# stelleg/caster-dta

Measured on AMD Instinct MI355X. Metric: graph-pairs/sec (Davis-shaped protein+drug), encoders fwd+bwd, higher is better.
Workload: dtype f32; 1 GPU; davis_b64; pairs_per_gpu=64, residues_per_gpu=19200, protein_edges_per_gpu=57484, atoms_per_gpu=2560, drug_edges_per_gpu=7986, encoder=CASTER-DTA(2,2), pass=fwdbwd, activation_storage=fp32, scope=encoders, torch_compile=False, tunable_gemms=False, two_lane_head=False, train_mode=True, csr_build_in_step=True, hip_graph=True, kernels=mfma

## Files before the change

caster-dta_amd/csrc/gvp_internal.h:

```cpp
#pragma once
#include <hip/hip_runtime.h>
#include <stdint.h>

#include "gvp_host.h"
#include "gvp_math.h"
#include "gvp_rng.h"

constexpr int POLICY_F32 = 0, POLICY_BF16 = 1, POLICY_GVPDEF = 2, POLICY_LINEAR = 3;

struct QuadOffsets {
  int emb, conv0, node0, layer_stride, head, total;
  int embT, convT0, nodeT0, layerT_stride, headT;
};

#ifndef CGVP_BWD_MAX_GRID
#define CGVP_BWD_MAX_GRID 240
#endif
constexpr int kBwdMaxGrid = CGVP_BWD_MAX_GRID;

#include <type_traits>

namespace gq { struct bf16s; struct f32_gvpdef; struct f32_linear; }
template <class T> struct Tag { using type = T; };
template <class ST> constexpr bool is_layer_kind = std::is_same_v<ST, gq::f32_gvpdef> || std::is_same_v<ST, gq::f32_linear>;
template <bool KINDS, class F>
int with_policy(int policy, F&& f) {
  if (policy == POLICY_F32) return f(Tag<float>{});
  if (policy == POLICY_BF16) return f(Tag<gq::bf16s>{});
  if constexpr (KINDS) {
    if (policy == POLICY_GVPDEF) return f(Tag<gq::f32_gvpdef>{});
    if (policy == POLICY_LINEAR) return f(Tag<gq::f32_linear>{});
  }
  return CGVP_ERR_UNSUPPORTED_DIMS;
}
template <class F>
int with_flag(bool b, F&& f) { return b ? f(std::true_type{}) : f(std::false_type{}); }

namespace quad {
int offsets(int nt_node, int nt_edge, int num_convs, QuadOffsets* o);
int prepare(const gvp::EncLayout& L, int num_convs, int packed_bf16, const float* params, float* image, hipStream_t st);
int node_embed(int nt_node, const float* img, const float* x_s, const float* x_v, const int64_t* ntypes,
               int64_t N, float* h, unsigned long long* rng_state, unsigned long long* rng_out, int policy, hipStream_t st);
int pass_begin(const gvp::EncLayout& L, int num_convs, int policy, const float* params, float* image, const float* x_s,
               const float* x_v, const int64_t* ntypes, int64_t N, float* h, unsigned long long* rng_state,
               unsigned long long* rng_out, const int64_t* edge_index, int64_t E, int32_t* counters, hipStream_t st);
int conv(int nt_edge, const float* img, const float* h, const float* e_s, const float* e_v,
         const int64_t* etypes, const int32_t* rowptr, const int32_t* eperm, const int32_t* esrc,
         const int32_t* edst, int64_t N, int64_t E, int mean, float* dh, int fuse, const float* img_node,
         const float* img_head, float* h_out, float* out, const float* mask0, const float* mask1, gvp::RngArgs rng,
         const float* e_in, float* e_out, int policy, hipStream_t st);
int node_update(const float* img_node, const float* img_head, const float* h, const float* dh, int64_t N,
                int with_head, float* h_out, float* out, const float* mask0, const float* mask1, gvp::RngArgs rng,
                int policy, hipStream_t st);

int node_update_bwd(const float* img_node, const float* imgT_node, const float* h, const float* dh,
                    const float* mask0, const float* mask1, gvp::RngArgs rng, const float* g_up0, const float* g_up1,
                    const float* g_up2, int64_t N, float* g_dh, float* g_h, float* zero_rows, float* slab, int* grid,
                    int policy, hipStream_t st);
int head_bwd(const float* img_head, const float* imgT_head, const float* h_out, const float* g_out, int64_t N,
             float* g_h_out, float* slab, int* grid, int policy, hipStream_t st);
int node_head_bwd(const float* img_head, const float* imgT_head, const float* h_out, const float* g_out, float* g_h_out,
                  float* head_slab, const float* img_node, const float* imgT_node, const float* h, const float* dh,
                  const float* mask0, const float* mask1, gvp::RngArgs rng, int64_t N, float* g_dh, float* g_h,
                  float* zero_rows, float* slab, int* grid, int policy, hipStream_t st);
int conv_bwd(int nt_edge, const float* img, const float* imgT, const float* h, const float* e_emb,
             const int32_t* rowptr, const int32_t* esrc, const int32_t* edst, int64_t N, int64_t E, int mean,
             const float* g_dh, float* g_src, float* g_dst, float* g_e, float* slab, int* grid, int policy, hipStream_t st,
             float* g_edge = nullptr, float* slot = nullptr);
int conv_bwd_max_waves();
int64_t src_index_work_ints(int64_t N, int64_t E);
int src_index(const int32_t* rowptr, const int32_t* esrc, int64_t N, int64_t E, int32_t* sptr, int32_t* spos,
              int32_t* work, hipStream_t st);
int src_sum(int width, const float* rows, const float* self, const int32_t* sptr, const int32_t* spos,
            const int32_t* rowptr, const float* slot, int64_t waves, int64_t N, float* out, hipStream_t st);
struct DetBufs { const int32_t* sptr; const int32_t* spos; float* rows; float* slot; };
int conv_bwd_entry(const cgvp_dims* dims, const cgvp_layout* layout, const float* image, int32_t layer,
                   const float* h, const float* e_emb, const int32_t* rowptr, const int32_t* esrc,
                   const int32_t* edst, int64_t N, int64_t E, int32_t aggr_mean, const float* g_dh, float* g_src,
                   int32_t g_src_zeroed, float* g_dst, float* g_e, float* grad_params, float* workspace,
                   cgvp_segment* segs, int32_t* nsegs, void* stream, const DetBufs* det);
bool deterministic_env();
int edge_embed_bwd(int nt_edge, const float* img, const float* imgT, const float* e_s, const float* e_v,
                   const int64_t* etypes, const int32_t* eperm, int64_t E, const float* const* g_e, int n_g,
                   float* g_e_s, float* g_e_v, float* slab, int* grid, int policy, hipStream_t st);
constexpr int kEdgeRow = 36;
int node_embed_bwd(int nt_node, const float* img, const float* imgT, const float* x_s, const float* x_v,
                   const int64_t* ntypes, int64_t N, const float* g_up0, const float* g_up1, const float* g_up2,
                   float* g_x_s, float* g_x_v, float* slab, int* grid, int policy, hipStream_t st);
constexpr int kGineBwdMaxGrid = 256;
constexpr int kGineBwdDefaultGrid = 16;
int gine_bwd(int cin, int chid, int cout, int nt, int net, int ed, const float* x, const int64_t* ntypes,
             const float* eattr, const int64_t* etypes, const int32_t* rowptr, const int32_t* eperm,
             const int32_t* esrc, const int32_t* edst, int64_t N, const cgvp_gine_w* w, float slope,
             const float* mask, gvp::RngArgs rng, const float* g_out, float* g_x, float* slab, int max_workgroups, int* rows,
             int* row_len, hipStream_t st, const float* agg_in = nullptr, const uint16_t* pos_in = nullptr,
             float* g_edge = nullptr, float* g_self = nullptr,
             float* g_eattr = nullptr, int eattr_accum = 0);
int gine_fwd(int cin, int chid, int cout, int nt, int net, int ed, const float* x, const int64_t* ntypes,
             const float* eattr, const int64_t* etypes, const int32_t* rowptr, const int32_t* eperm,
             const int32_t* esrc, const int32_t* edst, int64_t N, const cgvp_gine_w* w, float slope,
             const float* mask, gvp::RngArgs rng, float* out, float* agg_out, uint16_t* pos_out, hipStream_t st);
int reduce_slab(const float* slab, int rows, int stride, int col0, int len, float* dst, hipStream_t st);
int reduce_segments(const cgvp_segment* segs, int nsegs, float* grad_params, hipStream_t st, int overwrite = 0,
                    bool store_only = false);
struct BwdBlocks { int emb, conv_edge, conv_total, node, head; };
int bwd_block_sizes(int nt_node, int nt_edge, BwdBlocks* b);
void zero_words(void* p, size_t words, hipStream_t s);
int csr_build(const int64_t* edge_index, int64_t N, int64_t E, int32_t* rowptr, int32_t* eperm, int32_t* esrc,
              int32_t* edst, int32_t* work, int work_is_zero, int32_t* ids_scratch, unsigned long long* rng_state,
              unsigned long long* rng_out, hipStream_t stream);
}
```

caster-dta_amd/csrc/gvp_kernels.hip:

```cpp
#include <hip/hip_runtime.h>
#include <stdlib.h>
#include <stdint.h>

#include "gvp_internal.h"

using namespace gvp;

namespace {

constexpr int WAVE = 64;

inline int check_dims(const cgvp_dims* d) {
  if (!d) return CGVP_ERR_BAD_ARG;
  if (d->node_in_s != NODE_IN_S || d->node_in_v != NODE_IN_V || d->edge_in_s != EDGE_IN_S ||
      d->edge_in_v != EDGE_IN_V || d->hidden_s != NS || d->hidden_v != NV ||
      d->edge_hidden_s != ES || d->edge_hidden_v != EV || d->out_s != OUT)
    return CGVP_ERR_UNSUPPORTED_DIMS;
  if (d->storage != CGVP_F32 && d->storage != CGVP_BF16) return CGVP_ERR_UNSUPPORTED_DIMS;
  if (d->layer_kind < CGVP_LAYER_GATED || d->layer_kind > CGVP_LAYER_LINEAR) return CGVP_ERR_UNSUPPORTED_DIMS;
  if (d->layer_kind != CGVP_LAYER_GATED && d->storage != CGVP_F32) return CGVP_ERR_UNSUPPORTED_DIMS;
  return 0;
}
inline int check_dims_gated(const cgvp_dims* d) {
  if (int rc = check_dims(d)) return rc;
// ... 602 lines not shown
int cgvp_abi_version(void) { return CGVP_ABI_VERSION; }
const char* cgvp_build_info(void) { return "libcaster_gvp gfx950 (HIP, wave64), built " __DATE__ " " __TIME__; }

int cgvp_csr_from_coo(const int64_t* edge_index, int64_t N, int64_t E, int32_t* rowptr,
                      int32_t* eperm, int32_t* esrc, int32_t* edst, int32_t* work, int32_t work_is_zero,
                      int32_t* ids_scratch, void* stream) {
  return quad::csr_build(edge_index, N, E, rowptr, eperm, esrc, edst, work, work_is_zero, ids_scratch, nullptr, nullptr,
                         (hipStream_t)stream);
}
}

namespace quad {
void zero_words(void* p, size_t words, hipStream_t s) { ::zero_words(p, words, s); }

int csr_build(const int64_t* edge_index, int64_t N, int64_t E, int32_t* rowptr, int32_t* eperm, int32_t* esrc,
              int32_t* edst, int32_t* work, int work_is_zero, int32_t* ids_scratch, unsigned long long* rng_state,
              unsigned long long* rng_out, hipStream_t stream) {
  if (N < 0 || E < 0 || !rowptr || !work || (E > 0 && (!edge_index || !eperm || !esrc || !edst || !ids_scratch)))
    return CGVP_ERR_BAD_ARG;
  if (N >= (int64_t)1 << 31 || E >= (int64_t)1 << 31) return CGVP_ERR_BAD_ARG;
  if ((uintptr_t)work & 15) return CGVP_ERR_BAD_ARG;
  hipStream_t s = stream;
  const int64_t counters = (N + 1 + 63) / 64 * 64;
  if (work_is_zero == 0) {
    zero_words(work, (size_t)counters, s);
  }
  int32_t* tmp = ids_scratch;
  const int B = 256;
  if (E > 0 && work_is_zero != 2)
    launch<csr_count_kernel>(dim3((unsigned)((E + B - 1) / B)), dim3(B), 0, s, edge_index, N, E, work, rng_state, rng_out);
  else if (rng_state)
    launch<rng_next_kernel>(dim3(1), dim3(1), 0, s, rng_state, rng_out);
  if (N < SCAN_MULTI_MAX) {
    launch<csr_scan_multi_kernel>(dim3((unsigned)((N + 1 + SCAN_MULTI_CHUNK - 1) / SCAN_MULTI_CHUNK)),
                                  dim3(SCAN_MULTI_T), 0, s, work, (int32_t)N, (int32_t)counters, rowptr);
  } else {
    const int64_t tile = N < SCAN_LDS ? (N + 3) / 4 * 4 : SCAN_LDS;
    if (int rc = launch<csr_scan_kernel>(dim3(1), dim3(1024), (size_t)(tile + 1024 + 32) * sizeof(int32_t), s, work, N, rowptr)) return rc;
  }
  if (E > 0) launch<csr_fill_kernel>(dim3((unsigned)((E + B - 1) / B)), dim3(B), 0, s, edge_index, N, E, rowptr, work, tmp, edst);
  const int64_t span = E > counters ? E : counters;
  launch<csr_rank_kernel>(dim3((unsigned)((span + B - 1) / B)), dim3(B), 0, s, edge_index, N, E, counters, rowptr, tmp,
                          edst, eperm, esrc, work);
  return launch_status();
}

bool deterministic_env() {
  static const bool v = [] { const char* e = getenv("CGVP_DETERMINISTIC"); return e && e[0] == '1'; }();
  return v;
}

int64_t src_index_work_ints(int64_t N, int64_t E) { return (N + 1 + 63) / 64 * 64 + (E > 0 ? E : 1); }

int src_index(const int32_t* rowptr, const int32_t* esrc, int64_t N, int64_t E, int32_t* sptr, int32_t* spos,
              int32_t* work, hipStream_t s) {
  if (N < 0 || E < 0 || !rowptr || !sptr || !work || (E > 0 && (!esrc || !spos))) return CGVP_ERR_BAD_ARG;
  if (N >= (int64_t)1 << 31 || E >= (int64_t)1 << 31 || ((uintptr_t)work & 15)) return CGVP_ERR_BAD_ARG;
  const int64_t counters = (N + 1 + 63) / 64 * 64;
  int32_t* cnt = work;
  int32_t* tmp = work + counters;
  zero_words(cnt, (size_t)counters, s);
  const int B = 256;
  const unsigned eb = (unsigned)((E + B - 1) / B);
  if (E > 0) launch<src_count_kernel>(dim3(eb), dim3(B), 0, s, esrc, rowptr, N, cnt);
  if (N < SCAN_MULTI_MAX) {
    launch<csr_scan_multi_kernel>(dim3((unsigned)((N + 1 + SCAN_MULTI_CHUNK - 1) / SCAN_MULTI_CHUNK)),
                                  dim3(SCAN_MULTI_T), 0, s, cnt, (int32_t)N, (int32_t)counters, sptr);
  } else {
    const int64_t tile = N < SCAN_LDS ? (N + 3) / 4 * 4 : SCAN_LDS;
    if (int rc = launch<csr_scan_kernel>(dim3(1), dim3(1024), (size_t)(tile + 1024 + 32) * sizeof(int32_t), s, cnt, N, sptr)) return rc;
  }
  if (E > 0) {
    launch<src_fill_kernel>(dim3(eb), dim3(B), 0, s, esrc, rowptr, N, sptr, cnt, tmp);
    launch<src_rank_kernel>(dim3(eb), dim3(B), 0, s, esrc, rowptr, N, sptr, tmp, spos);
  }
  return launch_status();
}
}

extern "C" {

int cgvp_deterministic_forced(void) { return quad::deterministic_env() ? 1 : 0; }

int cgvp_csr_collate(const int32_t* st_rowptr, const int32_t* st_eperm, const int32_t* st_esrc,
                     const int32_t* st_edst, const int64_t* st_node_off, const int64_t* st_edge_off,
                     const int64_t* sel, const int64_t* b_node_off, const int64_t* b_edge_off, int64_t B,
                     int32_t table_mode, int32_t* rowptr, int32_t* eperm, int32_t* esrc, int32_t* edst, void* stream) {
  if (B < 0 || !rowptr) return CGVP_ERR_BAD_ARG;
  if (B == 0) return 0;
  if (!st_rowptr || !st_node_off || !st_edge_off || !sel || !b_node_off || !b_edge_off) return CGVP_ERR_BAD_ARG;
  CsrCollateArgs a{st_rowptr, st_eperm, st_esrc, st_edst, st_node_off, st_edge_off, sel, b_node_off, b_edge_off, B,
                   rowptr, eperm, esrc, edst, table_mode ? 1 : 0};
  launch<csr_collate_kernel>(dim3((unsigned)B), dim3(256), 0, (hipStream_t)stream, a);
  return launch_status();
}

int cgvp_lba_layout(const cgvp_dims* dims, int32_t num_ntypes, int32_t num_etypes, int32_t num_convs,
                    cgvp_layout* out) {
  if (int rc = check_dims(dims)) return rc;
  if (!out || num_ntypes < 0 || num_etypes < 0 || num_convs < 0) return CGVP_ERR_BAD_ARG;
  const EncLayout L = make_layout(num_ntypes, num_etypes, num_convs);
  out->nt_node = L.nt_node; out->nt_edge = L.nt_edge; out->node_gvp = L.node_gvp; out->node_ln = L.node_ln;
  out->edge_gvp = L.edge_gvp; out->edge_ln = L.edge_ln; out->conv0 = L.conv0;
  out->conv_stride = L.conv_stride; out->ln_out = L.ln_out; out->head = L.head; out->total = L.total;
  return 0;
}

int64_t cgvp_lba_image_floats(const cgvp_dims* dims, const cgvp_layout* layout) {
  if (int rc = check_dims(dims)) return rc;
  if (!layout) return CGVP_ERR_BAD_ARG;
  QuadOffsets o;
  if (int rc = quad::offsets(layout->nt_node, layout->nt_edge, num_convs_of(*layout), &o)) return rc;
  return o.total;
}

int cgvp_lba_prepare(const cgvp_dims* dims, const cgvp_layout* layout, const float* params, float* image,
                     void* stream) {
  if (int rc = check_dims(dims)) return rc;
  if (!layout || !params || !image) return CGVP_ERR_BAD_ARG;
  if (int rc = quad::prepare(cvt(*layout), num_convs_of(*layout), policy_of(dims) == POLICY_BF16 ? 1 : 0, params, image, (hipStream_t)stream)) return rc;
  return launch_status();
}

int cgvp_lba_pass_begin(const cgvp_dims* dims, const cgvp_layout* layout, const float* params, float* image,
                        const float* x_s, const float* x_v, const int64_t* ntypes, int64_t N, float* h,
                        uint64_t* rng_state, uint64_t* rng_out, const int64_t* edge_index, int64_t E,
                        int32_t* csr_counters, void* stream) {
  if (int rc = check_dims_gated(dims)) return rc;
  if (N < 0 || E < 0 || !layout || !params || !image || (layout->nt_node > 0 && N > 0 && !ntypes)) return CGVP_ERR_BAD_ARG;
  if ((rng_state != nullptr) != (rng_out != nullptr)) return CGVP_ERR_BAD_ARG;
  if (((uintptr_t)rng_state & 7) || ((uintptr_t)rng_out & 7) || ((uintptr_t)h & 15) || ((uintptr_t)image & 15)) return CGVP_ERR_BAD_ARG;
  if ((edge_index != nullptr) != (csr_counters != nullptr)) return CGVP_ERR_BAD_ARG;
  if (N > 0 && (!x_s || !x_v || !h)) return CGVP_ERR_BAD_ARG;
  if (N >= (int64_t)1 << 31 || E >= (int64_t)1 << 31) return CGVP_ERR_BAD_ARG;
  if (N == 0 && rng_state)
    if (int rc = cgvp_rng_next(rng_state, rng_out, stream)) return rc;
  if (int rc = quad::pass_begin(cvt(*layout), num_convs_of(*layout), policy_of(dims), params, image, x_s, x_v, ntypes, N, h,
                                reinterpret_cast<unsigned long long*>(rng_state), reinterpret_cast<unsigned long long*>(rng_out),
                                edge_index, E, csr_counters, (hipStream_t)stream)) return rc;
  return launch_status();
}


int cgvp_node_embed_fwd(const cgvp_dims* dims, const cgvp_layout* layout, const float* params,
                        const float* image, const float* x_s, const float* x_v, const int64_t* ntypes,
                        int64_t N, float* h, uint64_t* rng_state, uint64_t* rng_out, void* stream) {
  if (int rc = check_dims_gated(dims)) return rc;
  if (N < 0 || !layout || !params || (layout->nt_node > 0 && N > 0 && !ntypes)) return CGVP_ERR_BAD_ARG;
  if ((rng_state != nullptr) != (rng_out != nullptr) || (rng_state && !image)) return CGVP_ERR_BAD_ARG;
  if (((uintptr_t)rng_state & 7) || ((uintptr_t)rng_out & 7)) return CGVP_ERR_BAD_ARG;
  if (N == 0) return rng_state ? cgvp_rng_next(rng_state, rng_out, stream) : 0;
  if (!x_s || !x_v || !h) return CGVP_ERR_BAD_ARG;
  if (image) {
    if ((uintptr_t)h & 15) return CGVP_ERR_BAD_ARG;
    QuadOffsets o;
    if (int rc = quad::offsets(layout->nt_node, layout->nt_edge, num_convs_of(*layout), &o)) return rc;
    if (int rc = quad::node_embed(layout->nt_node, image + o.emb, x_s, x_v, ntypes, N, h,
                                  reinterpret_cast<unsigned long long*>(rng_state),
                                  reinterpret_cast<unsigned long long*>(rng_out), policy_of(dims), (hipStream_t)stream)) return rc;
    return launch_status();
  }
  if (policy_of(dims)) return CGVP_ERR_UNSUPPORTED_DIMS;
  NodeEmbedArgs a{params, cvt(*layout), x_s, x_v, ntypes, N, h};
  const dim3 grid((unsigned)((N + WAVE - 1) / WAVE));
  hipStream_t st = (hipStream_t)stream;
  switch (layout->nt_node) {
    case 0: launch<node_embed_kernel<0>>(grid, dim3(WAVE), 0, st, a); break;
    case 20: launch<node_embed_kernel<20>>(grid, dim3(WAVE), 0, st, a); break;
    case 21: launch<node_embed_kernel<21>>(grid, dim3(WAVE), 0, st, a); break;
    default: return CGVP_ERR_UNSUPPORTED_DIMS;
  }
  return launch_status();
}

int cgvp_conv_fwd(const cgvp_dims* dims, const cgvp_layout* layout, const float* params,
                  const float* image, int32_t layer,
                  const float* h, const float* e_s, const float* e_v, const int64_t* etypes,
                  const int32_t* rowptr, const int32_t* eperm, const int32_t* esrc,
                  const int32_t* edst, int64_t N, int64_t E, int32_t aggr_mean, const float* e_in,
                  float* e_out, float* dh, void* stream) {
  if (int rc = check_dims(dims)) return rc;
  if (N < 0 || E < 0 || !layout || !params) return CGVP_ERR_BAD_ARG;
  if (layer < 0 || layer >= num_convs_of(*layout)) return CGVP_ERR_BAD_ARG;
  if (N == 0) return 0;
  if (!h || !dh || !rowptr) return CGVP_ERR_BAD_ARG;
  if (!image && (e_in || e_out)) return CGVP_ERR_BAD_ARG;
  if (E > 0 && (!esrc || !edst)) return CGVP_ERR_BAD_ARG;
  if (E > 0 && !e_in && (!e_s || !e_v || !eperm || (layout->nt_edge > 0 && !etypes))) return CGVP_ERR_BAD_ARG;
  if (((uintptr_t)h & 15) || ((uintptr_t)e_s & 15) || ((uintptr_t)e_in & 15) || ((uintptr_t)e_out & 15)) return CGVP_ERR_BAD_ARG;
  if (image) {
    QuadOffsets o;
    if (int rc = quad::offsets(layout->nt_node, layout->nt_edge, num_convs_of(*layout), &o)) return rc;
    if (int rc = quad::conv(layout->nt_edge, image + o.conv0 + layer * o.layer_stride, h, e_s, e_v, etypes, rowptr,
                            eperm, esrc, edst, N, E, aggr_mean ? 1 : 0, dh, 0, nullptr, nullptr, nullptr, nullptr, nullptr,
                            nullptr, gvp::RngArgs{nullptr, 0.f, 0}, e_in, e_in ? nullptr : e_out, policy_of(dims),
                            (hipStream_t)stream)) return rc;
    return launch_status();
  }
  if (policy_of(dims)) return CGVP_ERR_UNSUPPORTED_DIMS;
  int64_t deg = (E + N - 1) / N;
  if (deg < 1) deg = 1;
  int npw = (int)(48 / deg);
  npw = npw < 1 ? 1 : (npw > WAVE ? WAVE : npw);
  ConvArgs a{params, cvt(*layout), layer, h, e_s, e_v, etypes, rowptr, eperm, esrc, edst, N, npw,
             aggr_mean ? 1 : 0, dh};
  const dim3 grid((unsigned)((N + npw - 1) / npw));
  hipStream_t st = (hipStream_t)stream;
  switch (layout->nt_edge) {
    case 0: launch<conv_fwd_kernel<0>>(grid, dim3(WAVE), 0, st, a); break;
    case 1: launch<conv_fwd_kernel<1>>(grid, dim3(WAVE), 0, st, a); break;
    default: return CGVP_ERR_UNSUPPORTED_DIMS;
  }
  return launch_status();
}

int cgvp_conv_layer_fwd(const cgvp_dims* dims, const cgvp_layout* layout, const float* image, int32_t layer,
                        const float* h, const float* e_s, const float* e_v, const int64_t* etypes,
                        const int32_t* rowptr, const int32_t* eperm, const int32_t* esrc, const int32_t* edst,
                        int64_t N, int64_t E, int32_t aggr_mean, const float* mask0, const float* mask1,
                        const cgvp_rng* rng, int32_t with_head, const float* e_in, float* e_out, float* dh,
                        float* h_out, float* out, void* stream) {
  if (int rc = check_dims_gated(dims)) return rc;
  if (int rc = check_rng(rng)) return rc;
  if (N < 0 || E < 0 || !layout || !image) return CGVP_ERR_BAD_ARG;
  if (layer < 0 || layer >= num_convs_of(*layout)) return CGVP_ERR_BAD_ARG;
  if (N == 0) return 0;
  if (!h || !rowptr || (with_head ? !out : !h_out)) return CGVP_ERR_BAD_ARG;
  if (E > 0 && (!esrc || !edst)) return CGVP_ERR_BAD_ARG;
  if (E > 0 && !e_in && (!e_s || !e_v || !eperm || (layout->nt_edge > 0 && !etypes))) return CGVP_ERR_BAD_ARG;
  const void* al[] = {h, e_s, dh, h_out, out, mask0, mask1, e_in, e_out};
  for (const void* q : al) if ((uintptr_t)q & 15) return CGVP_ERR_BAD_ARG;
  QuadOffsets o;
  if (int rc = quad::offsets(layout->nt_node, layout->nt_edge, num_convs_of(*layout), &o)) return rc;
  if (int rc = quad::conv(layout->nt_edge, image + o.conv0 + layer * o.layer_stride, h, e_s, e_v, etypes, rowptr, eperm,
                          esrc, edst, N, E, aggr_mean ? 1 : 0, dh, with_head ? 2 : 1,
                          image + o.node0 + layer * o.layer_stride, image + o.head, h_out, out, mask0, mask1,
                          rng_args(rng, 2 * layer), e_in, e_in ? nullptr : e_out, policy_of(dims), (hipStream_t)stream)) return rc;
  return launch_status();
}

int cgvp_node_update_fwd(const cgvp_dims* dims, const cgvp_layout* layout, const float* params,
                         const float* image, int32_t layer, const float* h, const float* dh, int64_t N,
                         int32_t with_head, float* h_out, float* out, void* stream) {
  if (int rc = check_dims(dims)) return rc;
  if (N < 0 || !layout || !params) return CGVP_ERR_BAD_ARG;
  if (layer < 0 || layer >= num_convs_of(*layout)) return CGVP_ERR_BAD_ARG;
  if (N == 0) return 0;
  if (!h || !dh || (with_head ? !out : !h_out)) return CGVP_ERR_BAD_ARG;
  if (((uintptr_t)h & 15) || ((uintptr_t)dh & 15)) return CGVP_ERR_BAD_ARG;
  if (image) {
    if (((uintptr_t)h_out & 15) || ((uintptr_t)out & 15)) return CGVP_ERR_BAD_ARG;
    QuadOffsets o;
    if (int rc = quad::offsets(layout->nt_node, layout->nt_edge, num_convs_of(*layout), &o)) return rc;
    if (int rc = quad::node_update(image + o.node0 + layer * o.layer_stride, image + o.head, h, dh, N,
                                   with_head ? 1 : 0, h_out, out, nullptr, nullptr, gvp::RngArgs{nullptr, 0.f, 0},
                                   policy_of(dims), (hipStream_t)stream)) return rc;
    return launch_status();
  }
  if (policy_of(dims)) return CGVP_ERR_UNSUPPORTED_DIMS;
  NodeUpdateArgs a{params, cvt(*layout), layer, h, dh, N, h_out, out};
  dim3 grid((unsigned)((N + WAVE - 1) / WAVE));
  if (with_head) launch<node_update_kernel<true>>(grid, dim3(WAVE), 0, (hipStream_t)stream, a);
  else launch<node_update_kernel<false>>(grid, dim3(WAVE), 0, (hipStream_t)stream, a);
  return launch_status();
}

int cgvp_node_update_fwd_train(const cgvp_dims* dims, const cgvp_layout* layout, const float* image,
                               int32_t layer, const float* h, const float* dh, const float* mask0,
                               const float* mask1, const cgvp_rng* rng, int64_t N, int32_t with_head, float* h_out,
                               float* out, void* stream) {
  if (int rc = check_dims(dims)) return rc;
  if (int rc = check_rng(rng)) return rc;
  if (N < 0 || !layout || !image) return CGVP_ERR_BAD_ARG;
  if (layer < 0 || layer >= num_convs_of(*layout)) return CGVP_ERR_BAD_ARG;
  if (N == 0) return 0;
  if (!h || !dh || (with_head ? !out : !h_out)) return CGVP_ERR_BAD_ARG;
  if (((uintptr_t)h & 15) || ((uintptr_t)dh & 15) || ((uintptr_t)h_out & 15) || ((uintptr_t)out & 15) ||
      ((uintptr_t)mask0 & 15) || ((uintptr_t)mask1 & 15)) return CGVP_ERR_BAD_ARG;
  QuadOffsets o;
  if (int rc = quad::offsets(layout->nt_node, layout->nt_edge, num_convs_of(*layout), &o)) return rc;
  if (int rc = quad::node_update(image + o.node0 + layer * o.layer_stride, image + o.head, h, dh, N,
                                 with_head ? 1 : 0, h_out, out, mask0, mask1, rng_args(rng, 2 * layer),
                                 policy_of(dims), (hipStream_t)stream)) return rc;
  return launch_status();
}

int64_t cgvp_bwd_workspace_floats(const cgvp_dims* dims, const cgvp_layout* layout) {
  if (int rc = check_dims(dims)) return rc;
  if (!layout) return CGVP_ERR_BAD_ARG;
  quad::BwdBlocks b;
  if (int rc = quad::bwd_block_sizes(layout->nt_node, layout->nt_edge, &b)) return rc;
  int mx = b.emb > b.conv_total ? b.emb : b.conv_total;
  mx = mx > b.node + b.head ? mx : b.node + b.head;
  mx = mx > 2 * b.conv_edge ? mx : 2 * b.conv_edge;
  return (int64_t)kBwdMaxGrid * mx;
}

int cgvp_node_update_bwd(const cgvp_dims* dims, const cgvp_layout* layout, const float* image, int32_t layer,
                         const float* h, const float* dh, const float* mask0, const float* mask1,
                         const cgvp_rng* rng, const float* h_out, const float* g_out, const float* g_up0, const float* g_up1,
                         const float* g_up2, int64_t N, int32_t with_head, float* g_dh, float* g_h,
                         float* zero_out, float* grad_params, float* workspace, cgvp_segment* segs, int32_t* nsegs,
                         void* stream) {
  if (int rc = check_dims(dims)) return rc;
  if (int rc = check_rng(rng)) return rc;
  if (N < 0 || !layout || !image || !grad_params || !workspace) return CGVP_ERR_BAD_ARG;
  const int nc = num_convs_of(*layout);
  if (layer < 0 || layer >= nc) return CGVP_ERR_BAD_ARG;
  if (N == 0) return 0;
  if (!h || !dh || !g_dh || (with_head && (!g_out || !h_out))) return CGVP_ERR_BAD_ARG;
  if (with_head && dims->layer_kind != CGVP_LAYER_GATED) return CGVP_ERR_UNSUPPORTED_DIMS;
  const void* al[] = {h, dh, mask0, mask1, h_out, g_out, g_up0, g_up1, g_up2, g_dh, g_h, zero_out};
  for (const void* q : al) if ((uintptr_t)q & 15) return CGVP_ERR_BAD_ARG;
  BwdLookup o;
  if (int rc = bwd_lookup(*layout, &o)) return rc;
  int grid = 0, hgrid = 0;
  hipStream_t st = (hipStream_t)stream;
  float* head_slab = workspace + (size_t)kBwdMaxGrid * o.blk.node;
  static const bool split_head = [] { const char* e = getenv("CGVP_SPLIT_HEAD_BWD"); return e && e[0] == '1'; }();
  if (with_head && !split_head) {
    if (int rc = quad::node_head_bwd(image + o.head, image + o.headT, h_out, g_out, g_dh, head_slab,
                                     image + o.node0 + layer * o.layer_stride, image + o.nodeT0 + layer * o.layerT_stride,
                                     h, dh, mask0, mask1, rng_args(rng, 2 * layer), N, g_dh, g_h, zero_out, workspace, &grid,
                                     policy_of(dims), st)) return rc;
    hgrid = grid;
  } else {
  if (with_head) {
    if (int rc = quad::head_bwd(image + o.head, image + o.headT, h_out, g_out, N, g_dh, head_slab, &hgrid, policy_of(dims), st)) return rc;
    g_up0 = g_dh; g_up1 = nullptr; g_up2 = nullptr;
  }
  if (int rc = quad::node_update_bwd(image + o.node0 + layer * o.layer_stride, image + o.nodeT0 + layer * o.layerT_stride,
                                     h, dh, mask0, mask1, rng_args(rng, 2 * layer), g_up0, g_up1, g_up2, N, g_dh, g_h, zero_out,
                                     workspace, &grid, policy_of(dims), st)) return rc;
  }
  const int node_len = conv_ff1() + LFf1::size(0) - conv_ln0();
  cgvp_segment sg[2] = {{workspace, grid, o.blk.node, 0, node_len, layout->conv0 + layer * layout->conv_stride + conv_ln0()},
                        {head_slab, hgrid, o.blk.head, 0, layout->total - layout->ln_out, layout->ln_out}};
  return emit_segments(sg, with_head ? 2 : 1, segs, nsegs, grad_params, st);
}

int cgvp_conv_bwd(const cgvp_dims* dims, const cgvp_layout* layout, const float* image, int32_t layer,
                  const float* h, const float* e_emb, const int32_t* rowptr, const int32_t* esrc,
                  const int32_t* edst, int64_t N, int64_t E, int32_t aggr_mean, const float* g_dh, float* g_src,
                  int32_t g_src_zeroed, float* g_dst, float* g_e, float* grad_params, float* workspace,
                  cgvp_segment* segs, int32_t* nsegs, void* stream) {
  if (quad::deterministic_env()) return CGVP_ERR_NONDETERMINISTIC;
  return quad::conv_bwd_entry(dims, layout, image, layer, h, e_emb, rowptr, esrc, edst, N, E, aggr_mean, g_dh, g_src,
                              g_src_zeroed, g_dst, g_e, grad_params, workspace, segs, nsegs, stream, nullptr);
}
}

int quad::conv_bwd_entry(const cgvp_dims* dims, const cgvp_layout* layout, const float* image, int32_t layer,
                         const float* h, const float* e_emb, const int32_t* rowptr, const int32_t* esrc,
                         const int32_t* edst, int64_t N, int64_t E, int32_t aggr_mean, const float* g_dh, float* g_src,
                         int32_t g_src_zeroed, float* g_dst, float* g_e, float* grad_params, float* workspace,
                         cgvp_segment* segs, int32_t* nsegs, void* stream, const quad::DetBufs* det) {
  if (int rc = check_dims(dims)) return rc;
  if (N < 0 || E < 0 || !layout || !image || !grad_params || !workspace) return CGVP_ERR_BAD_ARG;
  const int nc = num_convs_of(*layout);
  if (layer < 0 || layer >= nc) return CGVP_ERR_BAD_ARG;
  if (N == 0) return 0;
  if (!h || !g_dh || !g_src || !g_dst || !rowptr) return CGVP_ERR_BAD_ARG;
  if (E > 0 && (!e_emb || !g_e || !esrc || !edst)) return CGVP_ERR_BAD_ARG;
  const void* al[] = {h, e_emb, g_dh, g_src, g_dst, g_e};
  for (const void* q : al) if ((uintptr_t)q & 15) return CGVP_ERR_BAD_ARG;
  BwdLookup o;
  if (int rc = bwd_lookup(*layout, &o)) return rc;
  int grid = 0;
  hipStream_t st = (hipStream_t)stream;
  if (!g_src_zeroed && !det) {
    zero_words(g_src, (size_t)N * ROW, st);
  }
  if (int rc = quad::conv_bwd(layout->nt_edge, image + o.conv0 + layer * o.layer_stride,
                              image + o.convT0 + layer * o.layerT_stride, h, e_emb, rowptr, esrc, edst, N, E,
                              aggr_mean ? 1 : 0, g_dh, g_src, g_dst, g_e, workspace, &grid, policy_of(dims), st,
                              det ? det->rows : nullptr, det ? det->slot : nullptr)) return rc;
  if (det)
    if (int rc = quad::src_sum(ROW, det->rows, nullptr, det->sptr, det->spos, rowptr, det->slot, (int64_t)grid * 8, N, g_src, st))
      return rc;
  const cgvp_segment sg{workspace, grid, o.blk.conv_total, 0, conv_ln0(), layout->conv0 + layer * layout->conv_stride};
  return emit_segments(&sg, 1, segs, nsegs, grad_params, st, det ? 1 : 0, det != nullptr);
}

extern "C" {

int64_t cgvp_src_index_work_ints(int64_t num_nodes, int64_t num_edges) {
  if (num_nodes < 0 || num_edges < 0) return CGVP_ERR_BAD_ARG;
  return quad::src_index_work_ints(num_nodes, num_edges);
}

int cgvp_src_index(const int32_t* rowptr, const int32_t* esrc, int64_t num_nodes, int64_t num_edges, int32_t* sptr,
                   int32_t* spos, int32_t* work, void* stream) {
  return quad::src_index(rowptr, esrc, num_nodes, num_edges, sptr, spos, work, (hipStream_t)stream);
}

int64_t cgvp_conv_bwd_det_floats(int64_t num_nodes, int64_t num_edges) {
  if (num_nodes < 0 || num_edges < 0) return CGVP_ERR_BAD_ARG;
  return (num_edges > 0 ? num_edges : 1) * ROW + (int64_t)quad::conv_bwd_max_waves() * ROW;
}

int cgvp_conv_bwd_ex(const cgvp_dims* dims, const cgvp_layout* layout, const float* image, int32_t layer,
                     const float* h, const float* e_emb, const int32_t* rowptr, const int32_t* esrc,
                     const int32_t* edst, int64_t N, int64_t E, int32_t aggr_mean, const float* g_dh, float* g_src,
                     int32_t g_src_zeroed, float* g_dst, float* g_e, float* grad_params, float* workspace,
                     cgvp_segment* segs, int32_t* nsegs, const int32_t* sptr, const int32_t* spos, float* det_scratch,
                     int32_t flags, void* stream) {
  if (!((flags & CGVP_BWD_DETERMINISTIC) || quad::deterministic_env()))
    return quad::conv_bwd_entry(dims, layout, image, layer, h, e_emb, rowptr, esrc, edst, N, E, aggr_mean, g_dh, g_src,
                                g_src_zeroed, g_dst, g_e, grad_params, workspace, segs, nsegs, stream, nullptr);
  if (!sptr || !det_scratch || (E > 0 && !spos) || ((uintptr_t)det_scratch & 15)) return CGVP_ERR_BAD_ARG;
  const quad::DetBufs db{sptr, spos, det_scratch, det_scratch + (E > 0 ? E : 1) * ROW};
  return quad::conv_bwd_entry(dims, layout, image, layer, h, e_emb, rowptr, esrc, edst, N, E, aggr_mean, g_dh, g_src,
                              g_src_zeroed, g_dst, g_e, grad_params, workspace, segs, nsegs, stream, &db);
}

}

extern "C" {

int cgvp_edge_embed_bwd(const cgvp_dims* dims, const cgvp_layout* layout, const float* image, const float* e_s,
                        const float* e_v, const int64_t* etypes, const int32_t* eperm, int64_t E,
                        const float* const* g_e, int32_t num_g, float* g_e_s, float* g_e_v, float* grad_params,
                        float* workspace, cgvp_segment* segs, int32_t* nsegs, void* stream) {
  if (int rc = check_dims_gated(dims)) return rc;
  if (E < 0 || !layout || !image || !grad_params || !workspace || !g_e || num_g < 1) return CGVP_ERR_BAD_ARG;
  if ((g_e_s == nullptr) != (g_e_v == nullptr) || ((uintptr_t)g_e_s & 15)) return CGVP_ERR_BAD_ARG;
  if (segs && nsegs) *nsegs = 0;
  if (E == 0) return 0;
  if (!e_s || !e_v || !eperm || (layout->nt_edge > 0 && !etypes)) return CGVP_ERR_BAD_ARG;
  if ((uintptr_t)e_s & 15) return CGVP_ERR_BAD_ARG;
  for (int l = 0; l < num_g; ++l) if (!g_e[l] || ((uintptr_t)g_e[l] & 15)) return CGVP_ERR_BAD_ARG;
  BwdLookup o;
  if (int rc = bwd_lookup(*layout, &o)) return rc;
  int grid = 0;
  hipStream_t st = (hipStream_t)stream;
  if (g_e_s) {
    quad::zero_words(g_e_s, (size_t)E * EDGE_IN_S, st);
    quad::zero_words(g_e_v, (size_t)E * EDGE_IN_V * 3, st);
  }
  if (int rc = quad::edge_embed_bwd(layout->nt_edge, image + o.conv0, image + o.convT0, e_s, e_v, etypes, eperm, E, g_e,
                                    num_g, g_e_s, g_e_v, workspace, &grid, policy_of(dims), st)) return rc;
  const cgvp_segment sg{workspace, grid, o.blk.conv_edge, 0, layout->conv0 - layout->edge_gvp, layout->edge_gvp};
  return emit_segments(&sg, 1, segs, nsegs, grad_params, st);
}

int cgvp_node_embed_bwd(const cgvp_dims* dims, const cgvp_layout* layout, const float* image, const float* x_s,
                        const float* x_v, const int64_t* ntypes, int64_t N, const float* g_up0,
                        const float* g_up1, const float* g_up2, float* g_x_s, float* g_x_v, float* grad_params,
                        float* workspace, cgvp_segment* segs, int32_t* nsegs, void* stream) {
  if (int rc = check_dims_gated(dims)) return rc;
  if (N < 0 || !layout || !image || !grad_params || !workspace) return CGVP_ERR_BAD_ARG;
  if (N == 0) return 0;
  if (!x_s || !x_v || (layout->nt_node > 0 && !ntypes) || ((g_x_s == nullptr) != (g_x_v == nullptr))) return CGVP_ERR_BAD_ARG;
  const void* al[] = {g_up0, g_up1, g_up2};
  for (const void* q : al) if ((uintptr_t)q & 15) return CGVP_ERR_BAD_ARG;
  BwdLookup o;
  if (int rc = bwd_lookup(*layout, &o)) return rc;
  int grid = 0;
  hipStream_t st = (hipStream_t)stream;
  if (int rc = quad::node_embed_bwd(layout->nt_node, image + o.emb, image + o.embT, x_s, x_v, ntypes, N, g_up0, g_up1,
                                    g_up2, g_x_s, g_x_v, workspace, &grid, policy_of(dims), st)) return rc;
  const cgvp_segment sg{workspace, grid, o.blk.emb, 0, layout->edge_gvp - layout->node_gvp, layout->node_gvp};
  return emit_segments(&sg, 1, segs, nsegs, grad_params, st);
}

int cgvp_gine_conv_fwd(const float* x, const int64_t* ntypes, int32_t num_ntypes, const float* eattr,
                       const int64_t* etypes, int32_t num_etypes, int32_t edge_dim,
                       const int32_t* rowptr, const int32_t* eperm, const int32_t* esrc, const int32_t* edst,
                       int64_t N, int64_t E, int32_t cin, int32_t chid, int32_t cout, const cgvp_gine_w* w,
                       float act_slope, const float* mask, const cgvp_rng* rng, int32_t variant, float* out,
                       void* stream) {
  if (N < 0 || E < 0 || !w) return CGVP_ERR_BAD_ARG;
  if (int rc = check_rng(rng)) return rc;
  const gvp::RngArgs ra = rng_args(rng, 0);
  if (num_ntypes < 0 || num_etypes < 0 || edge_dim < 0 || cin <= num_ntypes) return CGVP_ERR_BAD_ARG;
  if (cin > WAVE || chid > WAVE || cout > WAVE || chid < 1 || cout < 1 || num_etypes + edge_dim > GINE_MAXKE)
    return CGVP_ERR_UNSUPPORTED_DIMS;
  if (N == 0) return 0;
  if (!x || !out || !rowptr || (num_ntypes > 0 && !ntypes)) return CGVP_ERR_BAD_ARG;
  if (E > 0 && (!eperm || !esrc || (edge_dim > 0 && !eattr) || (num_etypes > 0 && !etypes))) return CGVP_ERR_BAD_ARG;
  if (variant == 0 && edst && !((uintptr_t)out & 15) && !((uintptr_t)mask & 15)) {
    const int rc = quad::gine_fwd(cin, chid, cout, num_ntypes, num_etypes, edge_dim, x, ntypes, eattr, etypes, rowptr,
                                  eperm, esrc, edst, N, w, act_slope, mask, ra, out, nullptr, nullptr, (hipStream_t)stream);
    if (rc <= 0) return rc < 0 ? rc : launch_status();
  }
  GineArgs a{x, ntypes, num_ntypes, eattr, etypes, num_etypes, edge_dim, rowptr, eperm, esrc, N, cin,
             chid, cout, w->eps, w->we, w->be, w->w0, w->b0, w->w1, w->b1, act_slope, out, mask, ra};
  const size_t lds = (size_t)(chid * (cin + 1) + cout * (chid + 1) + 2 * GINE_APB * WAVE) * sizeof(float);
  launch<gine_conv_kernel>(dim3((unsigned)((N + GINE_APB - 1) / GINE_APB)),
                           dim3(WAVE * GINE_APB), lds, (hipStream_t)stream, a);
  return launch_status();
}

int cgvp_rng_next(uint64_t* state, uint64_t* out, void* stream) {
  if (!state || !out || ((uintptr_t)state & 7) || ((uintptr_t)out & 7)) return CGVP_ERR_BAD_ARG;
  launch<rng_next_kernel>(dim3(1), dim3(1), 0, (hipStream_t)stream,
                          reinterpret_cast<unsigned long long*>(state), reinterpret_cast<unsigned long long*>(out));
  return launch_status();
}

int cgvp_dropout_masks(const cgvp_rng* rng, int32_t num_masks, int64_t N, int32_t width, float* out, void* stream) {
  if (!rng || !rng->seed || !out || num_masks < 1 || N < 0 || width < 4 || (width & 3)) return CGVP_ERR_BAD_ARG;
  if (int rc = check_rng(rng)) return rc;
  if (N == 0) return 0;
  MaskArgs a{rng_args(rng, 0), num_masks, N, width, out};
  const int64_t total = (int64_t)num_masks * N * (width / 4);
  launch<dropout_masks_kernel>(dim3((unsigned)((total + 255) / 256 > 4096 ? 4096 : (total + 255) / 256)), dim3(256), 0,
                               (hipStream_t)stream, a);
  return launch_status();
}

int cgvp_bwd_reduce(const cgvp_segment* segs, int32_t nsegs, float* grad_params, int32_t overwrite, void* stream) {
  if (!segs || nsegs < 0 || nsegs > CGVP_MAX_SEGS || !grad_params) return CGVP_ERR_BAD_ARG;
  quad::reduce_segments(segs, nsegs, grad_params, (hipStream_t)stream, overwrite ? 1 : 0);
  return launch_status();
}

int64_t cgvp_gine_bwd_workspace_floats(void) { return (int64_t)quad::kGineBwdMaxGrid * gine_layer_floats(16, 64, 64, 14); }

int cgvp_gine_conv_bwd(const float* x, const int64_t* ntypes, int32_t num_ntypes, const float* eattr,
                       const int64_t* etypes, int32_t num_etypes, int32_t edge_dim, const int32_t* rowptr,
                       const int32_t* eperm, const int32_t* esrc, const int32_t* edst, int64_t N, int64_t E,
                       int32_t cin, int32_t chid, int32_t cout, const cgvp_gine_w* w, float act_slope,
                       const float* mask, const cgvp_rng* rng, const float* g_out, float* g_x, float* grad_layer,
                       float* workspace, int32_t max_workgroups, void* stream) {
  if (N < 0 || E < 0 || !w || !grad_layer || !workspace) return CGVP_ERR_BAD_ARG;
  if (int rc = check_rng(rng)) return rc;
  if (quad::deterministic_env() && g_x) return CGVP_ERR_NONDETERMINISTIC;
  if (N == 0) return 0;
  if (!x || !g_out || !rowptr || (num_ntypes > 0 && !ntypes)) return CGVP_ERR_BAD_ARG;
  if (E > 0 && (!eperm || !esrc || !edst || (edge_dim > 0 && !eattr) || (num_etypes > 0 && !etypes))) return CGVP_ERR_BAD_ARG;
  if (((uintptr_t)g_out & 15) || ((uintptr_t)mask & 15)) return CGVP_ERR_BAD_ARG;
  hipStream_t st = (hipStream_t)stream;
  if (g_x) {
    zero_words(g_x, (size_t)N * (cin - num_ntypes), st);
  }
  int rows = 0, row_len = 0;
  if (int rc = quad::gine_bwd(cin, chid, cout, num_ntypes, num_etypes, edge_dim, x, ntypes, eattr, etypes, rowptr, eperm,
                              esrc, edst, N, w, act_slope, mask, rng_args(rng, 0), g_out, g_x, workspace, max_workgroups, &rows, &row_len, st)) return rc;
  quad::reduce_slab(workspace, rows, row_len, 0, row_len, grad_layer, st);
  return launch_status();
}

}
```

caster-dta_amd/csrc/gvp_quad_bwd_kernels.hip:

```cpp
#include <hip/hip_runtime.h>
#include <stdint.h>
#include <stdlib.h>

#include <type_traits>

#include "gvp_internal.h"
#include "gvp_quad.h"

using namespace gq;

#ifdef CGVP_STAMPS
__device__ unsigned long long* g_stamp_buf_bwd = nullptr;
extern "C" int cgvp_debug_set_stamp_buffer_bwd(unsigned long long* buf) {
  return (int)hipMemcpyToSymbol(HIP_SYMBOL(g_stamp_buf_bwd), &buf, sizeof(buf));
}
#endif

namespace {

constexpr int WAVE = 64;
constexpr int TILE = 16;

#ifdef CGVP_STAMPS
#define STAMP(slot)                                                                          \
  do {                                                                                       \
    __builtin_amdgcn_sched_barrier(0);                                                       \
    unsigned long long t_;                                                                   \
    asm volatile("s_waitcnt vmcnt(0) lgkmcnt(0)\n\ts_memtime %0\n\ts_waitcnt lgkmcnt(0)" : "=s"(t_)::"memory"); \
    __builtin_amdgcn_sched_barrier(0);                                                       \
    if (g_stamp_buf_bwd && (threadIdx.x & 63) == 0)                                          \
      g_stamp_buf_bwd[((size_t)blockIdx.x * (blockDim.x >> 6) + (threadIdx.x >> 6)) * 16 + (slot)] = t_;    \
  } while (0)
struct WallStamp {
  int kind;
  __device__ __forceinline__ explicit WallStamp(int k) : kind(k) { put(0); }
  __device__ __forceinline__ ~WallStamp() { put(1); }
  __device__ __forceinline__ void put(int which) const {
    unsigned long long t_;
    asm volatile("s_waitcnt vmcnt(0) lgkmcnt(0)\n\ts_memrealtime %0\n\ts_waitcnt lgkmcnt(0)" : "=s"(t_)::"memory");
    const size_t wave = (size_t)blockIdx.x * (blockDim.x >> 6) + (threadIdx.x >> 6);
    if (g_stamp_buf_bwd && (threadIdx.x & 63) == 0 && wave < 4096)
      g_stamp_buf_bwd[4096 * 16 + ((size_t)kind * 4096 + wave) * 2 + which] = t_;
  }
};
#define WALL_STAMP(kind) WallStamp wall_stamp_(kind)
#else
#define STAMP(slot) do {} while (0)
#define WALL_STAMP(kind) do {} while (0)
#endif
constexpr int BW_WPB = 8, BW_TPB = WAVE * BW_WPB, BW_MAX_GRID = kBwdMaxGrid;
static_assert(BW_MAX_GRID <= 256, "at most one workgroup per CU");

__device__ __forceinline__ int opaque_lane(int lane) {
  asm volatile("" : "+v"(lane));
  return lane;
}

template <int BLK>
__device__ __forceinline__ void zero_block(float* gblk, int lane) {
  static_assert(BLK % 4 == 0, "blocks are whole float4s");
  for (int k = lane; k < BLK / 4; k += WAVE) reinterpret_cast<f4*>(gblk)[k] = f4{0.f, 0.f, 0.f, 0.f};
}
template <int BLK, int PW, int WPB_ = 8>
__device__ __forceinline__ void write_slab_row(float* slab, const float* blocks, int row = blockIdx.x) {
  __syncthreads();
  float* out = slab + (size_t)row * BLK;
  for (int k = threadIdx.x; k < BLK; k += WAVE * WPB_) {
    float t = 0.f;
#pragma unroll
    for (int ww = 0; ww < WPB_; ++ww) t += blocks[ww * PW + k];
    out[k] = t;
  }
}

template <int NFLOATS, int NTHR>
__device__ __forceinline__ void stage_slice(float* lds, const float* __restrict__ src, int tid) {
  static_assert(NFLOATS % 4 == 0, "image slices are whole float4s");
  constexpr int NF4 = NFLOATS / 4, IT = (NF4 + NTHR - 1) / NTHR;
  const f4* s = reinterpret_cast<const f4*>(src);
  f4* d = reinterpret_cast<f4*>(lds);
  f4 v[IT];
#pragma unroll
  for (int k = 0; k < IT; ++k) { const int idx = tid + k * NTHR; if (idx < NF4) v[k] = s[idx]; }
#pragma unroll
  for (int k = 0; k < IT; ++k) { const int idx = tid + k * NTHR; if (idx < NF4) d[idx] = v[k]; }
}

constexpr int cmax(int a, int b) { return a > b ? a : b; }
template <bool ONE> using AccFor = typename std::conditional<ONE, AccStoreOnce, AccPriv>::type;
constexpr int pad4(int x) { return (x + 3) / 4 * 4; }

template <class Acc, int S>
__device__ __forceinline__ void ln_param_grads(float* blk, bool first, int lane, bool active,
                                               const f4 (&dgamma)[S / 16], const f4 (&dbeta)[S / 16]) {
  const int i = lane & 15, g = lane >> 4;
#pragma unroll
  for (int t = 0; t < S / 16; ++t) {
    float tot[8];
    float* q[8];
    bool on[8];
#pragma unroll
    for (int r = 0; r < 4; ++r) {
      tot[r] = row_total(active ? dgamma[t][r] : 0.f);
      tot[4 + r] = row_total(active ? dbeta[t][r] : 0.f);
      q[r] = blk + 16 * t + 4 * g + r;
      q[4 + r] = blk + S + 16 * t + 4 * g + r;
      on[r] = on[4 + r] = i == 15;
    }
    add_where<Acc, 8>(q, on, tot);
  }
}

constexpr int NB_LN0 = 0, NB_LN1 = 2 * NS, NB_FF0 = 4 * NS, NB_FF1 = NB_FF0 + LFf0::size(0),
              NODE_BLK = NB_FF1 + LFf1::size(0);
constexpr int HB_LN = 0, HB_GVP = 2 * NS, HEAD_BLK = HB_GVP + LHead::size(0);
constexpr int NODE_GB = pad4(NODE_BLK), HEAD_GB = pad4(HEAD_BLK);

constexpr int MROW = NS + NV;
__device__ __forceinline__ void node_dropout(const float* mask, const gvp::RngArgs& rng, int which, int64_t n, int g,
                                             f4& ms, float& mv) {
  if (mask) {
    ms = *reinterpret_cast<const f4*>(mask + n * MROW + 4 * g);
    mv = mask[n * MROW + NS + g];
  } else if (rng.seed) {
    const unsigned long long seed = rng.seed[0], off = rng.seed[1];
    float fs[4];
    gvp::dropout_row20(seed, off, rng.stream + which, n, g, rng.p, fs, mv);
    ms = f4{fs[0], fs[1], fs[2], fs[3]};
  }
}
struct NodeBArgs {
  const float* img_node; const float* imgT_node;
  const float* h; const float* dh; const float* mask0; const float* mask1; gvp::RngArgs rng;
  const float* g_up0; const float* g_up1; const float* g_up2;
  int64_t N; float* g_dh; float* g_h; float* zero_rows; float* slab;
};
constexpr int node_bwd_lds_floats() { return BW_TPB + Image<0, 0>::ND_SIZE + Image<0, 0>::TN_SIZE + BW_WPB * (NODE_GB + TSCR_FLOATS); }
static_assert(node_bwd_lds_floats() * 4 <= 160 * 1024, "node backward LDS plan exceeds the CU");

template <typename ST, bool ONE = false>
__device__ __forceinline__ void node_bwd_body(const NodeBArgs& a, float* lds) {
  typedef Image<0, 0> IM;
  typedef AccFor<ONE> Acc;
  float* f_node = lds + BW_TPB;
  float* t_node = f_node + IM::ND_SIZE;
  float* blocks = t_node + IM::TN_SIZE;
  const int lane0 = threadIdx.x & 63, w = threadIdx.x >> 6;
  float* gblk = blocks + w * NODE_GB;
  float* tscr = blocks + BW_WPB * NODE_GB + w * TSCR_FLOATS;
  stage_slice<IM::ND_SIZE, BW_TPB>(f_node, a.img_node, threadIdx.x);
  stage_slice<IM::TN_SIZE, BW_TPB>(t_node, a.imgT_node, threadIdx.x);
  zero_block<NODE_GB>(gblk, lane0);
  STAMP(0);
  __syncthreads();
  STAMP(1);

  const f4 zero = {0.f, 0.f, 0.f, 0.f};
  const int zt[1] = {0};
  const bool first = false;
  const int64_t ntiles = (a.N + TILE - 1) / TILE;
  for (int64_t tile = (int64_t)w * gridDim.x + blockIdx.x; tile < ntiles; tile += (int64_t)gridDim.x * BW_WPB) {
    const int lane = opaque_lane(lane0), i = lane & 15, g = lane >> 4;
    const int64_t n = tile * TILE + i;
    const bool active = n < a.N;
    f4 x0[1] = {zero};
    float xv0[3][1] = {{0.f}, {0.f}, {0.f}};
    f4 m0s = {1.f, 1.f, 1.f, 1.f}, m1s = {1.f, 1.f, 1.f, 1.f};
    float m0v = 1.f, m1v = 1.f;
    f4 gs[1] = {zero};
    float gv[3][1] = {{0.f}, {0.f}, {0.f}};
    if (active) {
      const int64_t hr = n * ROW;
      node_dropout(a.mask0, a.rng, 0, n, g, m0s, m0v);
      node_dropout(a.mask1, a.rng, 1, n, g, m1s, m1v);
      x0[0] = Io<ST>::ld4(a.h, hr + 4 * g) + Io<ST>::ld4(a.dh, hr + 4 * g) * m0s;
#pragma unroll
      for (int p = 0; p < 3; ++p) xv0[p][0] = Io<ST>::ld(a.h, hr + NS + 3 * g + p) + Io<ST>::ld(a.dh, hr + NS + 3 * g + p) * m0v;
      const float* ups[3] = {a.g_up0, a.g_up1, a.g_up2};
#pragma unroll
      for (int u = 0; u < 3; ++u)
        if (ups[u]) {
          const float* r_ = ups[u] + n * ROW;
          gs[0] += *reinterpret_cast<const f4*>(r_ + 4 * g);
#pragma unroll
          for (int p = 0; p < 3; ++p) gv[p][0] += r_[NS + 3 * g + p];
        }
    }
    f4 y[1] = {x0[0]};
    float yv[3][1] = {{xv0[0][0]}, {xv0[1][0]}, {xv0[2][0]}};
    ln_quad<NS, NV>(f_node + IM::ND_LN0, lane, y, yv);
    f4 hs[1][4], s2[1][1];
    float hv[1][3][2], v2[1][3][1];
    float bs0[1][4], bv0[1][3][1], bs1[1][16], bv1[1][3][2];
    typename Ff0<ST>::Cache c0[1];
    typename Ff1<ST>::Cache c1[1];
#pragma unroll
    for (int r = 0; r < 4; ++r) bs0[0][r] = y[0][r];
#pragma unroll
    for (int p = 0; p < 3; ++p) bv0[0][p][0] = yv[p][0];
    Ff0<ST>::template forward<1, Io<ST>::BF>(f_node + IM::ND_FF0, lane, zt, bs0, bv0, hs, hv, c0);
#pragma unroll
    for (int t = 0; t < 4; ++t)
#pragma unroll
      for (int r = 0; r < 4; ++r) bs1[0][4 * t + r] = hs[0][t][r];
#pragma unroll
    for (int p = 0; p < 3; ++p) { bv1[0][p][0] = hv[0][p][0]; bv1[0][p][1] = hv[0][p][1]; }
    Ff1<ST>::template forward<1, Io<ST>::BF>(f_node + IM::ND_FF1, lane, zt, bs1, bv1, s2, v2, c1);
    f4 z[1] = {y[0] + s2[0][0] * m1s};
    float zv[3][1];
#pragma unroll
    for (int p = 0; p < 3; ++p) zv[p][0] = yv[p][0] + v2[0][p][0] * m1v;

    STAMP(2);
    STAMP(3);
    {
      f4 dga[1], dbe[1];
      ln_quad_bwd<NS, NV>(f_node + IM::ND_LN1, lane, z, zv, gs, gv, dga, dbe);
      ln_param_grads<Acc, NS>(gblk + NB_LN1, first, lane, active, dga, dbe);
    }
    float d_hs[16], d_hv[3][2];
    {
      f4 d_so[1] = {gs[0] * m1s};
      float d_vo[3][1] = {{gv[0][0] * m1v}, {gv[1][0] * m1v}, {gv[2][0] * m1v}};
      typename Ff1<ST>::Grads gr1;
      STAMP(4);
      Ff1<ST>::template backward<Io<ST>::BF>(t_node + IM::TN_FF1, lane, c1[0], d_so, d_vo, d_hs, d_hv, gr1);
      STAMP(5);
      Ff1<ST>::template weight_grads<Acc, Io<ST>::BF>(gblk + NB_FF1, first, lane, 0, active, bs1[0], bv1[0], c1[0], gr1, tscr);
    }
    {
      f4 d_so[4];
#pragma unroll
      for (int t = 0; t < 4; ++t) d_so[t] = f4{d_hs[4 * t], d_hs[4 * t + 1], d_hs[4 * t + 2], d_hs[4 * t + 3]};
      float d_ys[4], d_yv[3][1];
      typename Ff0<ST>::Grads gr0;
      STAMP(6);
      Ff0<ST>::template backward<Io<ST>::BF>(t_node + IM::TN_FF0, lane, c0[0], d_so, d_hv, d_ys, d_yv, gr0);
      STAMP(7);
      Ff0<ST>::template weight_grads<Acc, Io<ST>::BF>(gblk + NB_FF0, first, lane, 0, active, bs0[0], bv0[0], c0[0], gr0, tscr);
#pragma unroll
      for (int r = 0; r < 4; ++r) gs[0][r] += d_ys[r];
#pragma unroll
      for (int p = 0; p < 3; ++p) gv[p][0] += d_yv[p][0];
    }
    STAMP(8);
    {
      f4 dga[1], dbe[1];
      ln_quad_bwd<NS, NV>(f_node + IM::ND_LN0, lane, x0, xv0, gs, gv, dga, dbe);
      ln_param_grads<Acc, NS>(gblk + NB_LN0, first, lane, active, dga, dbe);
    }
    if (active) {
      if (a.g_h) {
        float* row = a.g_h + n * ROW;
        *reinterpret_cast<f4*>(row + 4 * g) = gs[0];
#pragma unroll
        for (int p = 0; p < 3; ++p) row[NS + 3 * g + p] = gv[p][0];
      }
      float* row = a.g_dh + n * ROW;
      *reinterpret_cast<f4*>(row + 4 * g) = gs[0] * m0s;
#pragma unroll
      for (int p = 0; p < 3; ++p) row[NS + 3 * g + p] = gv[p][0] * m0v;
      if (a.zero_rows) {
        float* z = a.zero_rows + n * ROW;
        *reinterpret_cast<f4*>(z + 4 * g) = zero;
#pragma unroll
        for (int p = 0; p < 3; ++p) z[NS + 3 * g + p] = 0.f;
      }
    }
  }
  STAMP(9);
  write_slab_row<NODE_GB, NODE_GB>(a.slab, blocks);
  STAMP(10);
}
template <typename ST, bool ONE = false>
__global__ __launch_bounds__(BW_TPB, 2) void node_bwd_kernel(NodeBArgs a) {
  WALL_STAMP(0);
  extern __shared__ __attribute__((aligned(16))) float lds[];
  node_bwd_body<ST, ONE>(a, lds);
}

struct HeadBArgs {
  const float* img_head; const float* imgT_head; const float* h_out; const float* g_out;
  int64_t N; float* g_h_out; float* slab;
};
constexpr int head_bwd_lds_floats() { return BW_TPB + Image<0, 0>::HD_SIZE + Image<0, 0>::TH_SIZE + BW_WPB * (HEAD_GB + TSCR_FLOATS); }

template <typename ST, bool ONE = false>
__device__ __forceinline__ void head_bwd_body(const HeadBArgs& a, float* lds) {
  typedef Image<0, 0> IM;
  typedef AccFor<ONE> Acc;
  float* f_head = lds + BW_TPB;
  float* t_head = f_head + IM::HD_SIZE;
  float* blocks = t_head + IM::TH_SIZE;
  const int lane = threadIdx.x & 63, w = threadIdx.x >> 6;
  float* gblk = blocks + w * HEAD_GB;
  float* tscr = blocks + BW_WPB * HEAD_GB + w * TSCR_FLOATS;
  stage_slice<IM::HD_SIZE, BW_TPB>(f_head, a.img_head, threadIdx.x);
  stage_slice<IM::TH_SIZE, BW_TPB>(t_head, a.imgT_head, threadIdx.x);
  zero_block<HEAD_GB>(gblk, lane);
  __syncthreads();

  const int i = lane & 15, g = lane >> 4;
  const f4 zero = {0.f, 0.f, 0.f, 0.f};
  const int zt[1] = {0};
  const bool first = false;
  const int64_t ntiles = (a.N + TILE - 1) / TILE;
  for (int64_t tile = (int64_t)w * gridDim.x + blockIdx.x; tile < ntiles; tile += (int64_t)gridDim.x * BW_WPB) {
    const int64_t n = tile * TILE + i;
    const bool active = n < a.N;
    f4 o1[1] = {zero};
    float ov1[3][1] = {{0.f}, {0.f}, {0.f}};
    f4 d_o[4] = {zero, zero, zero, zero};
    if (active) {
      const int64_t hr = n * ROW;
      o1[0] = Io<ST>::ld4(a.h_out, hr + 4 * g);
#pragma unroll
      for (int p = 0; p < 3; ++p) ov1[p][0] = Io<ST>::ld(a.h_out, hr + NS + 3 * g + p);
      const float* gr_ = a.g_out + n * OUT;
#pragma unroll
      for (int t = 0; t < 4; ++t) d_o[t] = *reinterpret_cast<const f4*>(gr_ + 16 * t + 4 * g);
    }
    f4 wsn[1] = {o1[0]};
    float wvn[3][1] = {{ov1[0][0]}, {ov1[1][0]}, {ov1[2][0]}};
    ln_quad<NS, NV>(f_head + IM::HD_LN, lane, wsn, wvn);
    float bsh[1][4], bvh[1][3][1], dummy[1][3][1];
#pragma unroll
    for (int r = 0; r < 4; ++r) bsh[0][r] = wsn[0][r];
#pragma unroll
    for (int p = 0; p < 3; ++p) bvh[0][p][0] = wvn[p][0];
    f4 o[1][4];
    QHead::Cache ch[1];
    QHead::template forward<1, Io<ST>::BF>(f_head + IM::HD_GVP, lane, zt, bsh, bvh, o, dummy, ch);
    float d_vo[3][1] = {{0.f}, {0.f}, {0.f}}, d_bs[4], d_bv[3][1];
    QHead::Grads grh;
    QHead::template backward<Io<ST>::BF>(t_head, lane, ch[0], d_o, d_vo, d_bs, d_bv, grh);
    QHead::template weight_grads<Acc, Io<ST>::BF>(gblk + HB_GVP, first, lane, 0, active, bsh[0], bvh[0], ch[0], grh, tscr);
    f4 dws[1] = {f4{d_bs[0], d_bs[1], d_bs[2], d_bs[3]}};
    float dwv[3][1] = {{d_bv[0][0]}, {d_bv[1][0]}, {d_bv[2][0]}};
    f4 dga[1], dbe[1];
    ln_quad_bwd<NS, NV>(f_head + IM::HD_LN, lane, o1, ov1, dws, dwv, dga, dbe);
    ln_param_grads<Acc, NS>(gblk + HB_LN, first, lane, active, dga, dbe);
    if (active) {
      float* row = a.g_h_out + n * ROW;
      *reinterpret_cast<f4*>(row + 4 * g) = dws[0];
#pragma unroll
      for (int p = 0; p < 3; ++p) row[NS + 3 * g + p] = dwv[p][0];
    }
  }
  write_slab_row<HEAD_GB, HEAD_GB>(a.slab, blocks);
}
template <typename ST>
__global__ __launch_bounds__(BW_TPB, 2) void head_bwd_kernel(HeadBArgs a) {
  WALL_STAMP(1);
  extern __shared__ __attribute__((aligned(16))) float lds[];
  head_bwd_body<ST>(a, lds);
}

template <typename ST, bool ONE = false>
__global__ __launch_bounds__(BW_TPB, 2) void node_head_bwd_kernel(HeadBArgs hd, NodeBArgs a) {
  WALL_STAMP(0);
  extern __shared__ __attribute__((aligned(16))) float lds[];
  head_bwd_body<ST, ONE>(hd, lds);
  __syncthreads();
  node_bwd_body<ST, ONE>(a, lds);
}

constexpr int EROW = quad::kEdgeRow;
template <int NTE>
struct ConvBlk {
  static constexpr int M0 = 0, M1 = M0 + LMsg0::size(0), M2 = M1 + LMsg::size(0), SIZE = pad4(M2 + LMsg::size(0));
};
#ifndef CGVP_CONV_BWD_WAVES
#define CGVP_CONV_BWD_WAVES 8
#endif
constexpr int CB_WPB = CGVP_CONV_BWD_WAVES, CB_TPB = WAVE * CB_WPB, CB_MAX_GRID = BW_MAX_GRID;
constexpr int CB_SCR = TSCR_FLOATS;
static_assert(CB_SCR >= (TILE / 2) * ROW + TILE, "g_src transpose fits the scratch");
template <int NTE>
struct ConvBImg {
  typedef Image<0, NTE> IM;
  static constexpr int F0 = IM::CV_M0, FSIZE = IM::CV_SIZE - IM::CV_M0;
  static constexpr int T0 = IM::TC_M0, TSIZE = IM::TC_SIZE - IM::TC_M0;
};
template <int NTE>
constexpr int conv_bwd_lds_floats() { return CB_TPB + ConvBImg<NTE>::FSIZE + ConvBImg<NTE>::TSIZE + CB_WPB * (ConvBlk<NTE>::SIZE + CB_SCR); }
static_assert(conv_bwd_lds_floats<1>() * 4 <= 160 * 1024 && conv_bwd_lds_floats<0>() * 4 <= 160 * 1024, "conv backward LDS plan exceeds the CU");

struct ConvBArgs {
  const float* img; const float* imgT;
  const float* h; const float* e_emb;
  const int32_t* rowptr; const int32_t* esrc; const int32_t* edst;
  int64_t N; int npw; int mean; const float* g_dh; float* g_src; float* g_dst; float* g_e; float* slab;
  float* g_edge; float* slot;
};

template <int NTE, typename ST>
__global__ __launch_bounds__(CB_TPB, CB_WPB / 4) void conv_bwd_kernel(ConvBArgs a) {
  WALL_STAMP(2);
  typedef Image<0, NTE> IM;
  typedef ConvBImg<NTE> BI;
  typedef ConvBlk<NTE> B;
  constexpr int PW = B::SIZE + CB_SCR;
  extern __shared__ __attribute__((aligned(16))) float lds[];
  float* img = lds + CB_TPB - BI::F0;
  float* imgT = lds + CB_TPB + BI::FSIZE - BI::T0;
  const int lane0 = threadIdx.x & 63, w = threadIdx.x >> 6;
  float* blocks = lds + CB_TPB + BI::FSIZE + BI::TSIZE;
  float* gblk = blocks + w * PW;
  float* scr = gblk + B::SIZE;
#ifdef CGVP_MFMA_TRANSPOSE
  float* const CB_TSCR = nullptr;
#else
  float* const CB_TSCR = scr;
#endif
  stage_slice<BI::FSIZE, CB_TPB>(lds + CB_TPB, a.img + BI::F0, threadIdx.x);
  stage_slice<BI::TSIZE, CB_TPB>(lds + CB_TPB + BI::FSIZE, a.imgT + BI::T0, threadIdx.x);
  for (int k = lane0; k < B::SIZE / 4; k += WAVE) reinterpret_cast<f4*>(gblk)[k] = f4{0.f, 0.f, 0.f, 0.f};
  STAMP(0);
  __syncthreads();
  STAMP(1);

  const f4 zero = {0.f, 0.f, 0.f, 0.f};
  const int zt[1] = {0};
  const int64_t ngroups = (a.N + a.npw - 1) / a.npw;
  const int64_t grp0 = (int64_t)blockIdx.x * CB_WPB + w;
  const bool first = false;
  float carry[7] = {0.f, 0.f, 0.f, 0.f, 0.f, 0.f, 0.f};
  int carry_dst = -1;
  for (int64_t grp = grp0; grp < ngroups; grp += (int64_t)gridDim.x * CB_WPB) {
    const int64_t n0 = grp * a.npw;
    const int nn = (int)((a.N - n0 < a.npw) ? (a.N - n0) : a.npw);
    const int32_t e0 = a.rowptr[n0], e1 = a.rowptr[n0 + nn];
    for (int k = lane0; k < nn * ROW; k += WAVE) {
      const int64_t nd = n0 + k / ROW;
      if (a.rowptr[nd + 1] == a.rowptr[nd]) a.g_dst[n0 * ROW + k] = 0.f;
    }
    for (int32_t base = e0; base < e1; base += TILE) {
      const int lane = opaque_lane(lane0), i = lane & 15, g = lane >> 4;
      const int32_t p = base + i;
      const bool active = p < e1;
      f4 es0 = zero, es1 = zero, sj = zero, si = zero, d_ms = zero;
      float ev[3] = {0.f, 0.f, 0.f}, vj[3] = {0.f, 0.f, 0.f}, vi[3] = {0.f, 0.f, 0.f}, d_mv[3] = {0.f, 0.f, 0.f};
      int32_t src = 0, dst = -1;
      if (active) {
        src = a.esrc[p];
        dst = a.edst[p];
        const int64_t er = (int64_t)p * EROW;
        es0 = Io<ST>::ld4(a.e_emb, er + 4 * g);
        es1 = Io<ST>::ld4(a.e_emb, er + 16 + 4 * g);
        if (g == 0) {
#pragma unroll
          for (int d = 0; d < 3; ++d) ev[d] = Io<ST>::ld(a.e_emb, er + ES + d);
        }
        const int64_t hj = (int64_t)src * ROW, hi = (int64_t)dst * ROW;
        const float* gd = a.g_dh + (int64_t)dst * ROW;
        sj = Io<ST>::ld4(a.h, hj + 4 * g);
        si = Io<ST>::ld4(a.h, hi + 4 * g);
        d_ms = *reinterpret_cast<const f4*>(gd + 4 * g);
#pragma unroll
        for (int d = 0; d < 3; ++d) { vj[d] = Io<ST>::ld(a.h, hj + NS + 3 * g + d); vi[d] = Io<ST>::ld(a.h, hi + NS + 3 * g + d); d_mv[d] = gd[NS + 3 * g + d]; }
        if (a.mean) {
          const int deg = a.rowptr[dst + 1] - a.rowptr[dst];
          const float sc = 1.0f / (float)(deg > 1 ? deg : 1);
          d_ms *= sc;
#pragma unroll
          for (int d = 0; d < 3; ++d) d_mv[d] *= sc;
        }
      }
      STAMP(2);
      float b0[1][16], bv0[1][3][3], b1[1][4], bv1[1][3][1], b2[1][4], bv2[1][3][1];
#pragma unroll
      for (int r = 0; r < 4; ++r) { b0[0][r] = sj[r]; b0[0][4 + r] = es0[r]; b0[0][8 + r] = es1[r]; b0[0][12 + r] = si[r]; }
#pragma unroll
      for (int d = 0; d < 3; ++d) { bv0[0][d][0] = vj[d]; bv0[0][d][1] = vi[d]; bv0[0][d][2] = ev[d]; }
      f4 s1[1][1], s2[1][1], s3[1][1];
      float v1[1][3][1], v2[1][3][1], v3[1][3][1];
      typename Msg0<ST>::Cache c0[1];
      typename Msg1<ST>::Cache c1[1];
      typename Msg2<ST>::Cache c2[1];
      Msg0<ST>::template forward<1, Io<ST>::BF>(img + IM::CV_M0, lane, zt, b0, bv0, s1, v1, c0);
#pragma unroll
      for (int r = 0; r < 4; ++r) b1[0][r] = s1[0][0][r];
#pragma unroll
      for (int d = 0; d < 3; ++d) bv1[0][d][0] = v1[0][d][0];
      Msg1<ST>::template forward<1, Io<ST>::BF>(img + IM::CV_M1, lane, zt, b1, bv1, s2, v2, c1);
#pragma unroll
      for (int r = 0; r < 4; ++r) b2[0][r] = s2[0][0][r];
#pragma unroll
      for (int d = 0; d < 3; ++d) bv2[0][d][0] = v2[0][d][0];
      Msg2<ST>::template forward<1, Io<ST>::BF>(img + IM::CV_M2, lane, zt, b2, bv2, s3, v3, c2);

      STAMP(3);
      constexpr bool kAllActive = true;
      float d_b[4], d_bv[3][1];
      {
        f4 d_so[1] = {d_ms};
        float d_vo[3][1] = {{d_mv[0]}, {d_mv[1]}, {d_mv[2]}};
        typename Msg2<ST>::Grads gr;
        Msg2<ST>::template backward<Io<ST>::BF>(imgT + IM::TC_M2, lane, c2[0], d_so, d_vo, d_b, d_bv, gr);
        STAMP(10);
        Msg2<ST>::template weight_grads<AccPriv, Io<ST>::BF>(gblk + B::M2, first, lane, 0, kAllActive, b2[0], bv2[0], c2[0], gr, CB_TSCR);
      }
      {
        f4 d_so[1] = {f4{d_b[0], d_b[1], d_b[2], d_b[3]}};
        float d_vo[3][1] = {{d_bv[0][0]}, {d_bv[1][0]}, {d_bv[2][0]}};
        typename Msg1<ST>::Grads gr;
        STAMP(11);
        Msg1<ST>::template backward<Io<ST>::BF>(imgT + IM::TC_M1, lane, c1[0], d_so, d_vo, d_b, d_bv, gr);
        STAMP(12);
        Msg1<ST>::template weight_grads<AccPriv, Io<ST>::BF>(gblk + B::M1, first, lane, 0, kAllActive, b1[0], bv1[0], c1[0], gr, CB_TSCR);
      }
      float d_b0[16], d_bv0[3][3];
      {
        f4 d_so[1] = {f4{d_b[0], d_b[1], d_b[2], d_b[3]}};
        float d_vo[3][1] = {{d_bv[0][0]}, {d_bv[1][0]}, {d_bv[2][0]}};
        typename Msg0<ST>::Grads gr;
        STAMP(13);
        Msg0<ST>::template backward<Io<ST>::BF>(imgT + IM::TC_M0, lane, c0[0], d_so, d_vo, d_b0, d_bv0, gr);
        STAMP(14);
        Msg0<ST>::template weight_grads<AccPriv, Io<ST>::BF>(gblk + B::M0, first, lane, 0, kAllActive, b0[0], bv0[0], c0[0], gr, CB_TSCR);
      }
      STAMP(4);
      if (active) {
        const int64_t gr_ = (int64_t)p * EROW;
        Io<ST>::st4(a.g_e, gr_ + 4 * g, f4{d_b0[4], d_b0[5], d_b0[6], d_b0[7]});
        Io<ST>::st4(a.g_e, gr_ + 16 + 4 * g, f4{d_b0[8], d_b0[9], d_b0[10], d_b0[11]});
        if (g == 0) {
#pragma unroll
          for (int d = 0; d < 3; ++d) Io<ST>::st(a.g_e, gr_ + ES + d, d_bv0[d][2]);
        }
      }
      STAMP(5);
      {
        float* trow = scr;
        int* tsrc = reinterpret_cast<int*>(scr + (TILE / 2) * ROW);
        if (g == 0) tsrc[i] = active ? src : -1;
        const int half = lane / ROW, col = lane - half * ROW;
#pragma unroll
        for (int hb = 0; hb < 2; ++hb) {
          if ((i >> 3) == hb) {
            float* tr = trow + (i & 7) * ROW;
            *reinterpret_cast<f4*>(tr + 4 * g) = f4{d_b0[0], d_b0[1], d_b0[2], d_b0[3]};
#pragma unroll
            for (int d = 0; d < 3; ++d) tr[NS + 3 * g + d] = d_bv0[d][0];
          }
          __builtin_amdgcn_fence(__ATOMIC_RELEASE, "workgroup");
          __builtin_amdgcn_wave_barrier();
          __builtin_amdgcn_fence(__ATOMIC_ACQUIRE, "workgroup");
          if (half < 2) {
#pragma unroll
            for (int k = 0; k < TILE / 4; ++k) {
              const int r = 2 * k + half;
              const int sr = tsrc[8 * hb + r];
              if (sr >= 0) atomicAdd(a.g_src + (int64_t)sr * ROW + col, trow[r * ROW + col]);
            }
          }
          __builtin_amdgcn_fence(__ATOMIC_RELEASE, "workgroup");
          __builtin_amdgcn_wave_barrier();
        }
      }
      STAMP(6);
      {
        float x[7] = {d_b0[12], d_b0[13], d_b0[14], d_b0[15], d_bv0[0][1], d_bv0[1][1], d_bv0[2][1]};
        if (i == 0 && active && dst == carry_dst) {
#pragma unroll
          for (int k = 0; k < 7; ++k) x[k] += carry[k];
        }
        seg_scan16<7>(dst, x);
        const int nxt = __builtin_amdgcn_update_dpp(-1, dst, 0x100 | 1, 0xf, 0xf, false);
        if (active && (i == TILE - 1 || nxt != dst)) {
          float* row = a.g_dst + (int64_t)dst * ROW;
          *reinterpret_cast<f4*>(row + 4 * g) = f4{x[0], x[1], x[2], x[3]};
#pragma unroll
          for (int d = 0; d < 3; ++d) row[NS + 3 * g + d] = x[4 + d];
        }
        carry_dst = __builtin_amdgcn_update_dpp(-1, dst, 0x100 | 15, 0xf, 0xf, false);
#pragma unroll
        for (int k = 0; k < 7; ++k)
          carry[k] = __builtin_bit_cast(float, __builtin_amdgcn_update_dpp(0, __builtin_bit_cast(int, x[k]), 0x100 | 15, 0xf, 0xf, false));
      }
    }
    STAMP(7);
  }
  STAMP(8);
  write_slab_row<B::SIZE, PW, CB_WPB>(a.slab, blocks);
  STAMP(9);
}

template <int TN, int WPB>
struct C2Shape {
  static constexpr int TPB = WAVE * WPB, GS_ROWS = TN * TILE;
  static constexpr int SCR = TN * TSCR_FLOATS + GS_ROWS * ROW + GS_ROWS;
  static_assert((TN * TSCR_FLOATS) % 4 == 0 && (GS_ROWS * ROW) % 4 == 0, "scratch regions stay 16-B aligned");
  template <int NTE>
  static constexpr int lds_floats() { return TPB + ConvBImg<NTE>::FSIZE + ConvBImg<NTE>::TSIZE + WPB * (ConvBlk<NTE>::SIZE + SCR); }
};
static_assert(C2Shape<2, 4>::lds_floats<1>() * 4 <= 160 * 1024 && C2Shape<1, 8>::lds_floats<1>() * 4 <= 160 * 1024, "conv backward v2 LDS plan exceeds the CU");

struct C2Rows {
  f4 es0, es1, sj, si, d_ms;
  float ev[3], vj[3], vi[3], d_mv[3];
};
template <typename ST>
__device__ __forceinline__ void c2_load_rows(const ConvBArgs& a, int32_t pc, int32_t src, int32_t dst, int g, C2Rows& r) {
  const int64_t er = (int64_t)pc * EROW;
  r.es0 = Io<ST>::ld4(a.e_emb, er + 4 * g);
  r.es1 = Io<ST>::ld4(a.e_emb, er + 16 + 4 * g);
#pragma unroll
  for (int d = 0; d < 3; ++d) r.ev[d] = Io<ST>::ld(a.e_emb, er + ES + d);
  const int64_t hj = (int64_t)src * ROW, hi = (int64_t)dst * ROW;
  const float* gd = a.g_dh + (int64_t)dst * ROW;
  r.sj = Io<ST>::ld4(a.h, hj + 4 * g);
  r.si = Io<ST>::ld4(a.h, hi + 4 * g);
  r.d_ms = *reinterpret_cast<const f4*>(gd + 4 * g);
#pragma unroll
  for (int d = 0; d < 3; ++d) {
    r.vj[d] = Io<ST>::ld(a.h, hj + NS + 3 * g + d);
    r.vi[d] = Io<ST>::ld(a.h, hi + NS + 3 * g + d);
    r.d_mv[d] = gd[NS + 3 * g + d];
  }
  if (a.mean) {
    const int deg = a.rowptr[dst + 1] - a.rowptr[dst];
    const float sc = 1.0f / (float)(deg > 1 ? deg : 1);
    r.d_ms *= sc;
#pragma unroll
    for (int d = 0; d < 3; ++d) r.d_mv[d] *= sc;
  }
}

template <int NTE, typename ST, int TN, int C2_WPB, bool STORE = false>
__global__ __launch_bounds__(WAVE * C2_WPB) __attribute__((amdgpu_waves_per_eu(C2_WPB / 4, C2_WPB / 4))) void conv_bwd2_kernel(ConvBArgs a) {
  WALL_STAMP(2);
  typedef Image<0, NTE> IM;
  typedef ConvBImg<NTE> BI;
  typedef ConvBlk<NTE> B;
  typedef C2Shape<TN, C2_WPB> SH;
  constexpr int C2_TPB = SH::TPB, C2_GS_ROWS = SH::GS_ROWS, C2_SCR = SH::SCR;
  constexpr int PW = B::SIZE + C2_SCR;
  constexpr bool BF = Io<ST>::BF;
  extern __shared__ __attribute__((aligned(16))) float lds[];
  float* img = lds + C2_TPB - BI::F0;
  float* imgT = lds + C2_TPB + BI::FSIZE - BI::T0;
  const int lane = threadIdx.x & 63, i = lane & 15, g = lane >> 4;
  const int w = __builtin_amdgcn_readfirstlane(threadIdx.x >> 6);
  float* blocks = lds + C2_TPB + BI::FSIZE + BI::TSIZE;
  float* gblk = blocks + w * PW;
  float* tscr = gblk + B::SIZE;
  float* trow = tscr + TN * TSCR_FLOATS;
  int* tsrc = reinterpret_cast<int*>(trow + C2_GS_ROWS * ROW);
  stage_slice<BI::FSIZE, C2_TPB>(lds + C2_TPB, a.img + BI::F0, threadIdx.x);
  stage_slice<BI::TSIZE, C2_TPB>(lds + C2_TPB + BI::FSIZE, a.imgT + BI::T0, threadIdx.x);
  for (int k = lane; k < B::SIZE / 4; k += WAVE) reinterpret_cast<f4*>(gblk)[k] = f4{0.f, 0.f, 0.f, 0.f};

  const f4 zero = {0.f, 0.f, 0.f, 0.f};
  const int64_t waves = (int64_t)gridDim.x * C2_WPB, wid = (int64_t)blockIdx.x * C2_WPB + w;
  {
    const int64_t npw = (a.N + waves - 1) / waves;
    const int64_t n0 = wid * npw;
    const int64_t nn = n0 >= a.N ? 0 : (a.N - n0 < npw ? a.N - n0 : npw);
    for (int64_t k = lane; k < nn * ROW; k += WAVE) {
      const int64_t nd = n0 + k / ROW;
      if (a.rowptr[nd + 1] == a.rowptr[nd]) a.g_dst[n0 * ROW + k] = 0.f;
    }
  }
  const int32_t E = a.rowptr[a.N];
  const int32_t iters = (E + TN * TILE - 1) / (TN * TILE);
  const int32_t ipw = (int32_t)((iters + waves - 1) / waves);
  const int64_t it0 = wid * ipw;
  const int32_t c_lo = (int32_t)(it0 < iters ? it0 : iters) * (TN * TILE);
  int32_t c_hi = (int32_t)(it0 + ipw < iters ? it0 + ipw : iters) * (TN * TILE);
  c_hi = c_hi < E ? c_hi : E;
  int32_t lead_dst = -1;
  if (c_lo > 0 && c_lo < c_hi) {
    const int32_t d0 = a.edst[c_lo], dm = a.edst[c_lo - 1];
    lead_dst = d0 == dm ? d0 : -1;
  }
  typename Msg0<ST>::WAcc w0;
  typename Msg1<ST>::WAcc w1;
  typename Msg2<ST>::WAcc w2;
  Msg0<ST>::wacc_zero(w0);
  Msg1<ST>::wacc_zero(w1);
  Msg2<ST>::wacc_zero(w2);
  float carry[7] = {0.f, 0.f, 0.f, 0.f, 0.f, 0.f, 0.f};
  int carry_dst = -1;
  const int32_t p_last = c_hi - 1;
  constexpr bool PREFETCH = C2_WPB == 4;
  int32_t csrc[TN], cdst[TN];
  C2Rows cur[TN];
  if (PREFETCH && c_lo < c_hi) {
#pragma unroll
    for (int j = 0; j < TN; ++j) {
      const int32_t p = c_lo + j * TILE + i, pc = p < p_last ? p : p_last;
      csrc[j] = a.esrc[pc];
      cdst[j] = a.edst[pc];
    }
#pragma unroll
    for (int j = 0; j < TN; ++j) {
      const int32_t p = c_lo + j * TILE + i, pc = p < p_last ? p : p_last;
      c2_load_rows<ST>(a, pc, csrc[j], cdst[j], g, cur[j]);
    }
  }
  STAMP(0);
  __syncthreads();
  STAMP(1);

  const int zt[TN] = {};
  for (int32_t base = c_lo; base < c_hi; base += TN * TILE) {
    STAMP(15);
    const int32_t nxt_base = base + TN * TILE;
    int32_t nsrc[TN], ndst[TN], npc[TN];
    if constexpr (PREFETCH) {
#pragma unroll
      for (int j = 0; j < TN; ++j) {
        const int32_t p = nxt_base + j * TILE + i;
        npc[j] = p < p_last ? p : p_last;
        nsrc[j] = a.esrc[npc[j]];
        ndst[j] = a.edst[npc[j]];
      }
    } else {
      int32_t pc[TN];
#pragma unroll
      for (int j = 0; j < TN; ++j) {
        const int32_t p = base + j * TILE + i;
        pc[j] = p < p_last ? p : p_last;
        csrc[j] = a.esrc[pc[j]];
        cdst[j] = a.edst[pc[j]];
      }
#pragma unroll
      for (int j = 0; j < TN; ++j) c2_load_rows<ST>(a, pc[j], csrc[j], cdst[j], g, cur[j]);
    }
    f4 es0[TN], es1[TN], sj[TN], si[TN], d_ms[TN];
    float ev[TN][3], vj[TN][3], vi[TN][3], d_mv[TN][3];
    int32_t src[TN], dst[TN];
    bool active[TN];
#pragma unroll
    for (int j = 0; j < TN; ++j) {
      active[j] = base + j * TILE + i < c_hi;
      src[j] = csrc[j];
      dst[j] = active[j] ? cdst[j] : -1;
      es0[j] = cur[j].es0; es1[j] = cur[j].es1; sj[j] = cur[j].sj; si[j] = cur[j].si;
      d_ms[j] = active[j] ? cur[j].d_ms : zero;
#pragma unroll
      for (int d = 0; d < 3; ++d) {
        ev[j][d] = g == 0 ? cur[j].ev[d] : 0.f;
        vj[j][d] = cur[j].vj[d];
        vi[j][d] = cur[j].vi[d];
        d_mv[j][d] = active[j] ? cur[j].d_mv[d] : 0.f;
      }
    }
    STAMP(2);
    float b0[TN][16], bv0[TN][3][3], b1[TN][4], bv1[TN][3][1], b2[TN][4], bv2[TN][3][1];
#pragma unroll
    for (int j = 0; j < TN; ++j) {
#pragma unroll
      for (int r = 0; r < 4; ++r) { b0[j][r] = sj[j][r]; b0[j][4 + r] = es0[j][r]; b0[j][8 + r] = es1[j][r]; b0[j][12 + r] = si[j][r]; }
#pragma unroll
      for (int d = 0; d < 3; ++d) { bv0[j][d][0] = vj[j][d]; bv0[j][d][1] = vi[j][d]; bv0[j][d][2] = ev[j][d]; }
    }
    f4 s1[TN][1], s2[TN][1], s3[TN][1];
    float v1[TN][3][1], v2[TN][3][1], v3[TN][3][1];
    typename Msg0<ST>::Cache c0[TN];
    typename Msg1<ST>::Cache c1[TN];
    typename Msg2<ST>::Cache c2[TN];
    Msg0<ST>::template forward<TN, BF>(img + IM::CV_M0, lane, zt, b0, bv0, s1, v1, c0);
#pragma unroll
    for (int j = 0; j < TN; ++j) {
#pragma unroll
      for (int r = 0; r < 4; ++r) b1[j][r] = s1[j][0][r];
#pragma unroll
      for (int d = 0; d < 3; ++d) bv1[j][d][0] = v1[j][d][0];
    }
    Msg1<ST>::template forward<TN, BF>(img + IM::CV_M1, lane, zt, b1, bv1, s2, v2, c1);
#pragma unroll
    for (int j = 0; j < TN; ++j) {
#pragma unroll
      for (int r = 0; r < 4; ++r) b2[j][r] = s2[j][0][r];
#pragma unroll
      for (int d = 0; d < 3; ++d) bv2[j][d][0] = v2[j][d][0];
    }
    Msg2<ST>::template forward<TN, BF>(img + IM::CV_M2, lane, zt, b2, bv2, s3, v3, c2);
    STAMP(3);
    float d_b[TN][4], d_bv[TN][3][1];
    {
      f4 d_so[TN][1];
      float d_vo[TN][3][1];
#pragma unroll
      for (int j = 0; j < TN; ++j) {
        d_so[j][0] = d_ms[j];
#pragma unroll
        for (int d = 0; d < 3; ++d) d_vo[j][d][0] = d_mv[j][d];
      }
      typename Msg2<ST>::Grads gr[TN];
      Msg2<ST>::template backward_tn<TN, BF>(imgT + IM::TC_M2, lane, c2, d_so, d_vo, d_b, d_bv, gr);
      STAMP(10);
      if constexpr (!PREFETCH) {
        float b2r[TN][4], bv2r[TN][3][1];
#pragma unroll
        for (int j = 0; j < TN; ++j) Msg1<ST>::outputs_from_cache(c1[j], b2r[j], bv2r[j]);
        Msg2<ST>::template wacc_accumulate<TN, BF>(w2, lane, zt, b2r, bv2r, c2, gr, tscr);
      } else {
        Msg2<ST>::template wacc_accumulate<TN, BF>(w2, lane, zt, b2, bv2, c2, gr, tscr);
      }
    }
    {
      f4 d_so[TN][1];
      float d_vo[TN][3][1];
#pragma unroll
      for (int j = 0; j < TN; ++j) {
        d_so[j][0] = f4{d_b[j][0], d_b[j][1], d_b[j][2], d_b[j][3]};
#pragma unroll
        for (int d = 0; d < 3; ++d) d_vo[j][d][0] = d_bv[j][d][0];
      }
      typename Msg1<ST>::Grads gr[TN];
      STAMP(11);
      Msg1<ST>::template backward_tn<TN, BF>(imgT + IM::TC_M1, lane, c1, d_so, d_vo, d_b, d_bv, gr);
      STAMP(12);
      if constexpr (!PREFETCH) {
        float b1r[TN][4], bv1r[TN][3][1];
#pragma unroll
        for (int j = 0; j < TN; ++j) Msg0<ST>::outputs_from_cache(c0[j], b1r[j], bv1r[j]);
        Msg1<ST>::template wacc_accumulate<TN, BF>(w1, lane, zt, b1r, bv1r, c1, gr, tscr);
      } else {
        Msg1<ST>::template wacc_accumulate<TN, BF>(w1, lane, zt, b1, bv1, c1, gr, tscr);
      }
    }
    float d_b0[TN][16], d_bv0[TN][3][3];
    {
      f4 d_so[TN][1];
      float d_vo[TN][3][1];
#pragma unroll
      for (int j = 0; j < TN; ++j) {
        d_so[j][0] = f4{d_b[j][0], d_b[j][1], d_b[j][2], d_b[j][3]};
#pragma unroll
        for (int d = 0; d < 3; ++d) d_vo[j][d][0] = d_bv[j][d][0];
      }
      typename Msg0<ST>::Grads gr[TN];
      STAMP(13);
      Msg0<ST>::template backward_tn<TN, BF>(imgT + IM::TC_M0, lane, c0, d_so, d_vo, d_b0, d_bv0, gr);
      STAMP(14);
      if constexpr (PREFETCH) {
#pragma unroll
        for (int j = 0; j < TN; ++j) c2_load_rows<ST>(a, npc[j], nsrc[j], ndst[j], g, cur[j]);
      }
      Msg0<ST>::template wacc_accumulate<TN, BF>(w0, lane, zt, b0, bv0, c0, gr, tscr);
    }
    int32_t next_first = -1;
    if (nxt_base < c_hi) next_first = PREFETCH ? __builtin_amdgcn_readfirstlane(ndst[0]) : a.edst[nxt_base];
    STAMP(4);
#pragma unroll
    for (int j = 0; j < TN; ++j)
      if (active[j]) {
        const int64_t gr_ = (int64_t)(base + j * TILE + i) * EROW;
        Io<ST>::st4(a.g_e, gr_ + 4 * g, f4{d_b0[j][4], d_b0[j][5], d_b0[j][6], d_b0[j][7]});
        Io<ST>::st4(a.g_e, gr_ + 16 + 4 * g, f4{d_b0[j][8], d_b0[j][9], d_b0[j][10], d_b0[j][11]});
        if (g == 0) {
#pragma unroll
          for (int d = 0; d < 3; ++d) Io<ST>::st(a.g_e, gr_ + ES + d, d_bv0[j][d][2]);
        }
      }
    STAMP(5);
    bool self[TN];
    if constexpr (STORE) {
#pragma unroll
      for (int j = 0; j < TN; ++j) {
        self[j] = active[j] && src[j] == dst[j];
        if (active[j]) {
          float* row = a.g_edge + (int64_t)(base + j * TILE + i) * ROW;
          const bool z = self[j];
          *reinterpret_cast<f4*>(row + 4 * g) = z ? zero : f4{d_b0[j][0], d_b0[j][1], d_b0[j][2], d_b0[j][3]};
#pragma unroll
          for (int d = 0; d < 3; ++d) row[NS + 3 * g + d] = z ? 0.f : d_bv0[j][d][0];
        }
      }
    } else {
#pragma unroll
      for (int j = 0; j < TN; ++j) {
        self[j] = active[j] && src[j] == dst[j];
        float* tr = trow + (j * TILE + i) * ROW;
        *reinterpret_cast<f4*>(tr + 4 * g) = f4{d_b0[j][0], d_b0[j][1], d_b0[j][2], d_b0[j][3]};
#pragma unroll
        for (int d = 0; d < 3; ++d) tr[NS + 3 * g + d] = d_bv0[j][d][0];
        if (g == 0) tsrc[j * TILE + i] = (active[j] && !self[j]) ? src[j] : -1;
      }
      __builtin_amdgcn_wave_barrier();
      {
        const int half = lane / ROW, col = lane - half * ROW;
        const int hr = half & 1;
        int sr[C2_GS_ROWS / 2];
        float val[C2_GS_ROWS / 2];
#pragma unroll
        for (int k = 0; k < C2_GS_ROWS / 2; ++k) {
          sr[k] = tsrc[2 * k + hr];
          val[k] = trow[(2 * k + hr) * ROW + (half < 2 ? col : 0)];
        }
#pragma unroll
        for (int k = 0; k < C2_GS_ROWS / 2; ++k)
          if (half < 2 && sr[k] >= 0) atomicAdd(a.g_src + (int64_t)sr[k] * ROW + col, val[k]);
      }
      __builtin_amdgcn_wave_barrier();
    }
    STAMP(6);
#pragma unroll
    for (int j = 0; j < TN; ++j) {
      float x[7] = {d_b0[j][12], d_b0[j][13], d_b0[j][14], d_b0[j][15], d_bv0[j][0][1], d_bv0[j][1][1], d_bv0[j][2][1]};
      if (self[j]) {
#pragma unroll
        for (int k = 0; k < 4; ++k) x[k] += d_b0[j][k];
#pragma unroll
        for (int d = 0; d < 3; ++d) x[4 + d] += d_bv0[j][d][0];
      }
      if (i == 0 && active[j] && dst[j] == carry_dst) {
#pragma unroll
        for (int k = 0; k < 7; ++k) x[k] += carry[k];
      }
      seg_scan16<7>(dst[j], x);
      int nxt = __builtin_amdgcn_update_dpp(-1, dst[j], 0x100 | 1, 0xf, 0xf, false);
      if (i == TILE - 1) nxt = next_first;
      if (j + 1 < TN) {
        const int nf = __builtin_amdgcn_update_dpp(-1, dst[j + 1 < TN ? j + 1 : j], 0x110 | 15, 0xf, 0xf, false);
        if (i == TILE - 1) nxt = nf;
      }
      if (active[j] && nxt != dst[j]) {
        if (dst[j] != lead_dst) {
          float* row = a.g_dst + (int64_t)dst[j] * ROW;
          *reinterpret_cast<f4*>(row + 4 * g) = f4{x[0], x[1], x[2], x[3]};
#pragma unroll
          for (int d = 0; d < 3; ++d) row[NS + 3 * g + d] = x[4 + d];
        } else if constexpr (STORE) {
          float* row = a.slot + wid * ROW;
          *reinterpret_cast<f4*>(row + 4 * g) = f4{x[0], x[1], x[2], x[3]};
#pragma unroll
          for (int d = 0; d < 3; ++d) row[NS + 3 * g + d] = x[4 + d];
        } else {
          float* row = a.g_src + (int64_t)dst[j] * ROW;
#pragma unroll
          for (int k = 0; k < 4; ++k) atomicAdd(row + 4 * g + k, x[k]);
#pragma unroll
          for (int d = 0; d < 3; ++d) atomicAdd(row + NS + 3 * g + d, x[4 + d]);
        }
      }
      carry_dst = __builtin_amdgcn_update_dpp(-1, dst[j], 0x100 | 15, 0xf, 0xf, false);
#pragma unroll
      for (int k = 0; k < 7; ++k)
        carry[k] = __builtin_bit_cast(float, __builtin_amdgcn_update_dpp(0, __builtin_bit_cast(int, x[k]), 0x100 | 15, 0xf, 0xf, false));
    }
    if constexpr (PREFETCH) {
#pragma unroll
      for (int j = 0; j < TN; ++j) { csrc[j] = nsrc[j]; cdst[j] = ndst[j]; }
    }
    STAMP(7);
  }
  STAMP(8);
  Msg0<ST>::template wacc_flush<AccStoreOnce>(w0, gblk + B::M0, lane);
  Msg1<ST>::template wacc_flush<AccStoreOnce>(w1, gblk + B::M1, lane);
  Msg2<ST>::template wacc_flush<AccStoreOnce>(w2, gblk + B::M2, lane);
  write_slab_row<B::SIZE, PW, C2_WPB>(a.slab, blocks);
  STAMP(9);
}

template <int NTE>
struct EdgeBlk {
  static constexpr int GVP = 0, LN = LEdgeGvp::size(NTE), SIZE = pad4(LN + 2 * ES);
};
constexpr int EB_MAX_LAYERS = 8;
struct EdgeBArgs {
  const float* img; const float* imgT;
  const float* e_s; const float* e_v; const int64_t* etypes; const int32_t* eperm; int64_t E;
  const float* g_e[EB_MAX_LAYERS]; int n_g; float* slab;
  float* g_e_s; float* g_e_v;
};
template <int NTE>
constexpr int edge_bwd_lds_floats() { return BW_TPB + Image<0, NTE>::CV_M0 + Image<0, NTE>::TC_M0 + BW_WPB * (EdgeBlk<NTE>::SIZE + TSCR_FLOATS); }

template <int NTE, typename ST, bool DX>
__device__ __forceinline__ void edge_bwd_body(const EdgeBArgs& a, float* lds, int bid, int nblk) {
  typedef Image<0, NTE> IM;
  typedef EdgeBlk<NTE> B;
  constexpr int PW = B::SIZE + TSCR_FLOATS;
  float* img = lds + BW_TPB;
  float* imgT = img + IM::CV_M0;
  const int lane0 = threadIdx.x & 63, w = threadIdx.x >> 6;
  float* blocks = imgT + IM::TC_M0;
  float* gblk = blocks + w * PW;
  float* tscr = gblk + B::SIZE;
  stage_slice<IM::CV_M0, BW_TPB>(img, a.img, threadIdx.x);
  stage_slice<IM::TC_M0, BW_TPB>(imgT, a.imgT, threadIdx.x);
  for (int k = lane0; k < B::SIZE / 4; k += WAVE) reinterpret_cast<f4*>(gblk)[k] = f4{0.f, 0.f, 0.f, 0.f};
  __syncthreads();
  const f4 zero = {0.f, 0.f, 0.f, 0.f};
  const bool first = false;
  const int64_t tiles = (a.E + TILE - 1) / TILE;
  typename QEdge<NTE>::WAcc wacc;
  QEdge<NTE>::wacc_zero(wacc);
  for (int64_t t = (int64_t)w * nblk + bid; t < tiles; t += (int64_t)nblk * BW_WPB) {
    const int lane = opaque_lane(lane0), i = lane & 15, g = lane >> 4;
    const int64_t p = t * TILE + i;
    const int32_t eid = p < a.E ? a.eperm[p] : -1;
    const bool active = eid >= 0;
    f4 es0 = zero, es1 = zero;
    float ev[3] = {0.f, 0.f, 0.f};
    int et[1] = {0};
    f4 d_es[2] = {zero, zero};
    float d_ev[3][1] = {{0.f}, {0.f}, {0.f}};
    if (active) {
      const int64_t er = (int64_t)eid * EDGE_IN_S;
      es0 = Io<ST>::ld4(a.e_s, er + 4 * g);
      es1 = Io<ST>::ld4(a.e_s, er + 16 + 4 * g);
      if (g == 0) {
#pragma unroll
        for (int d = 0; d < 3; ++d) ev[d] = Io<ST>::ld(a.e_v, (int64_t)eid * 3 + d);
      }
      if (NTE > 0) {
        et[0] = (int)a.etypes[eid];
        et[0] = et[0] < 0 ? 0 : (et[0] >= NTE ? NTE - 1 : et[0]);
      }
      for (int l = 0; l < a.n_g; ++l) {
        const int64_t gr_ = p * EROW;
        d_es[0] += Io<ST>::ld4(a.g_e[l], gr_ + 4 * g);
        d_es[1] += Io<ST>::ld4(a.g_e[l], gr_ + 16 + 4 * g);
        if (g == 0) {
#pragma unroll
          for (int d = 0; d < 3; ++d) d_ev[d][0] += Io<ST>::ld(a.g_e[l], gr_ + ES + d);
        }
      }
    }
    float bse[1][8], bve[1][3][1];
#pragma unroll
    for (int r = 0; r < 4; ++r) { bse[0][r] = es0[r]; bse[0][4 + r] = es1[r]; }
#pragma unroll
    for (int d = 0; d < 3; ++d) bve[0][d][0] = ev[d];
    f4 e_pre[1][2];
    float ev_pre[1][3][1];
    typename QEdge<NTE>::Cache ce[1];
    QEdge<NTE>::template forward<1, Io<ST>::BF>(img + IM::CV_EDGE, lane, et, bse, bve, e_pre, ev_pre, ce);
    f4 dga[2], dbe[2];
    ln_quad_bwd<ES, EV>(img + IM::CV_ELN, lane, e_pre[0], ev_pre[0], d_es, d_ev, dga, dbe);
    ln_param_grads<AccPriv, ES>(gblk + B::LN, first, lane, active, dga, dbe);
    float d_in[8], d_inv[3][1];
    typename QEdge<NTE>::Grads gr[1];
    QEdge<NTE>::template backward<Io<ST>::BF>(imgT + IM::TC_EDGE, lane, ce[0], d_es, d_ev, d_in, d_inv, gr[0]);
    if (DX && active) {
      const int64_t er = (int64_t)eid * EDGE_IN_S;
      *reinterpret_cast<f4*>(a.g_e_s + er + 4 * g) = f4{d_in[0], d_in[1], d_in[2], d_in[3]};
      *reinterpret_cast<f4*>(a.g_e_s + er + 16 + 4 * g) = f4{d_in[4], d_in[5], d_in[6], d_in[7]};
      if (g == 0) {
#pragma unroll
        for (int d = 0; d < 3; ++d) a.g_e_v[(int64_t)eid * 3 + d] = d_inv[d][0];
      }
    }
    QEdge<NTE>::template wacc_accumulate<1, Io<ST>::BF>(wacc, lane, et, bse, bve, ce, gr, tscr);
  }
  QEdge<NTE>::template wacc_flush<AccStoreOnce>(wacc, gblk + B::GVP, lane0);
  write_slab_row<B::SIZE, PW>(a.slab, blocks, bid);
}
template <int NTE, typename ST, bool DX = false>
__global__ __launch_bounds__(BW_TPB) __attribute__((amdgpu_waves_per_eu(4, 4))) void edge_bwd_kernel(EdgeBArgs a) {
  WALL_STAMP(3);
  extern __shared__ __attribute__((aligned(16))) float lds[];
  edge_bwd_body<NTE, ST, DX>(a, lds, blockIdx.x, gridDim.x);
}

template <int NTN>
struct EmbBlk {
  static constexpr int GVP = 0, LN = LNodeGvp::size(NTN), SIZE = pad4(LN + 2 * NS);
};

struct EmbBArgs {
  const float* img; const float* imgT; const float* x_s; const float* x_v; const int64_t* ntypes; int64_t N;
  const float* g_up0; const float* g_up1; const float* g_up2; float* g_x_s; float* g_x_v; float* slab;
};

template <int NTN>
constexpr int embed_bwd_lds_floats() { return BW_TPB + Image<NTN, 0>::EMB_SIZE + Image<NTN, 0>::TE_SIZE + BW_WPB * (EmbBlk<NTN>::SIZE + TSCR_FLOATS); }

template <int NTN, typename ST, bool ONE = false>
__device__ __forceinline__ void embed_bwd_body(const EmbBArgs& a, float* lds, int bid, int nblk) {
  typedef Image<NTN, 0> IM;
  typedef AccFor<ONE> Acc;
  typedef QNode<NTN> Q;
  typedef EmbBlk<NTN> B;
  float* img = lds + BW_TPB;
  float* imgT = img + IM::EMB_SIZE;
  float* blocks = imgT + IM::TE_SIZE;
  const int lane = threadIdx.x & 63, w = threadIdx.x >> 6;
  float* gblk = blocks + w * B::SIZE;
  float* tscr = blocks + BW_WPB * B::SIZE + w * TSCR_FLOATS;
  stage_slice<IM::EMB_SIZE, BW_TPB>(img, a.img, threadIdx.x);
  stage_slice<IM::TE_SIZE, BW_TPB>(imgT, a.imgT, threadIdx.x);
  zero_block<B::SIZE>(gblk, lane);
  __syncthreads();
  const int i = lane & 15, g = lane >> 4;
  const f4 zero = {0.f, 0.f, 0.f, 0.f};
  const int64_t ntiles = (a.N + TILE - 1) / TILE;
  const bool first = false;
  for (int64_t tile = (int64_t)w * nblk + bid; tile < ntiles; tile += (int64_t)nblk * BW_WPB) {
    const int64_t n = tile * TILE + i;
    const bool active = n < a.N;
    float bs[1][Q::SSTEPS], bv[1][3][1];
    int type[1] = {0};
#pragma unroll
    for (int s = 0; s < Q::SSTEPS; ++s) {
      const int c = 4 * s + g;
      bs[0][s] = (active && c < NODE_IN_S) ? Io<ST>::ld(a.x_s, n * NODE_IN_S + c) : 0.f;
    }
#pragma unroll
    for (int p = 0; p < 3; ++p) bv[0][p][0] = (active && g < NODE_IN_V) ? Io<ST>::ld(a.x_v, n * 3 * NODE_IN_V + 3 * g + p) : 0.f;
    if (NTN > 0 && active) {
      type[0] = (int)a.ntypes[n];
      type[0] = type[0] < 0 ? 0 : (type[0] >= NTN ? NTN - 1 : type[0]);
    }
    f4 s_pre[1][1];
    float v_pre[1][3][1];
    typename Q::Cache c[1];
    Q::template forward<1, Io<ST>::BF>(img + IM::EMB_GVP, lane, type, bs, bv, s_pre, v_pre, c);
    f4 gs[1] = {zero};
    float gv[3][1] = {{0.f}, {0.f}, {0.f}};
    if (active) {
      const float* ups[3] = {a.g_up0, a.g_up1, a.g_up2};
#pragma unroll
      for (int u = 0; u < 3; ++u)
        if (ups[u]) {
          const float* r_ = ups[u] + n * ROW;
          gs[0] += *reinterpret_cast<const f4*>(r_ + 4 * g);
#pragma unroll
          for (int p = 0; p < 3; ++p) gv[p][0] += r_[NS + 3 * g + p];
        }
    }
    f4 dga[1], dbe[1];
    ln_quad_bwd<NS, NV>(img + IM::EMB_LN, lane, s_pre[0], v_pre[0], gs, gv, dga, dbe);
    ln_param_grads<Acc, NS>(gblk + B::LN, first, lane, active, dga, dbe);
    float d_bs[Q::SSTEPS], d_bv[3][1];
    typename Q::Grads gr;
    Q::template backward<Io<ST>::BF>(imgT, lane, c[0], gs, gv, d_bs, d_bv, gr);
    Q::template weight_grads<Acc, Io<ST>::BF>(gblk + B::GVP, first, lane, type[0], active, bs[0], bv[0], c[0], gr, tscr);
    if (active && a.g_x_s) {
#pragma unroll
      for (int s = 0; s < Q::SSTEPS; ++s) {
        const int cc = 4 * s + g;
        if (cc < NODE_IN_S) a.g_x_s[n * NODE_IN_S + cc] = d_bs[s];
      }
      if (g < NODE_IN_V) {
#pragma unroll
        for (int p = 0; p < 3; ++p) a.g_x_v[n * 3 * NODE_IN_V + 3 * g + p] = d_bv[p][0];
      }
    }
  }
  write_slab_row<B::SIZE, B::SIZE>(a.slab, blocks, bid);
}
template <int NTN, typename ST, bool ONE = false>
__global__ __launch_bounds__(BW_TPB, 2) void embed_bwd_kernel(EmbBArgs a) {
  WALL_STAMP(4);
  extern __shared__ __attribute__((aligned(16))) float lds[];
  embed_bwd_body<NTN, ST, ONE>(a, lds, blockIdx.x, gridDim.x);
}

constexpr int RED_COLS = 64, RED_RG = 16;
__global__ __launch_bounds__(RED_COLS * RED_RG) void reduce_slab_kernel(const float* __restrict__ slab, int rows,
                                                                        int stride, int col0, int len,
                                                                        float* __restrict__ dst) {
  __shared__ float part[RED_RG][RED_COLS];
  const int c = threadIdx.x & (RED_COLS - 1), rg = threadIdx.x / RED_COLS;
  const int j = blockIdx.x * RED_COLS + c;
  float s = 0.f;
  if (j < len)
    for (int r = rg; r < rows; r += RED_RG) s += slab[(size_t)r * stride + col0 + j];
  part[rg][c] = s;
  __syncthreads();
  if (rg == 0 && j < len) {
    float t = 0.f;
#pragma unroll
    for (int k = 0; k < RED_RG; ++k) t += part[k][c];
    dst[j] += t;
  }
}

__global__ __launch_bounds__(256) void reduce_rows_kernel(const float* __restrict__ slab, int rows, int stride, int col0,
                                                          int len, float* __restrict__ dst) {
  const int j = blockIdx.x * 256 + threadIdx.x;
  if (j >= len) return;
  float s = 0.f;
  for (int r = 0; r < rows; ++r) s += slab[(size_t)r * stride + col0 + j];
  dst[j] += s;
}

struct SegTable { cgvp_segment s[CGVP_MAX_SEGS]; };
template <bool ADD = true>
__global__ __launch_bounds__(RED_COLS * RED_RG) void reduce_segments_kernel(SegTable t, float* __restrict__ grad, int overwrite) {
  __shared__ float part[RED_RG][RED_COLS];
  const cgvp_segment sg = t.s[blockIdx.y];
  const int c = threadIdx.x & (RED_COLS - 1), rg = threadIdx.x / RED_COLS;
  const int j = blockIdx.x * RED_COLS + c;
  if (blockIdx.x * RED_COLS >= sg.len) return;
  float s = 0.f;
  if (j < sg.len) {
    const float* col = sg.slab + sg.col0 + j;
    float s0 = 0.f, s1 = 0.f, s2 = 0.f, s3 = 0.f;
    int r = rg;
    for (; r + 3 * RED_RG < sg.rows; r += 4 * RED_RG) {
      s0 += col[(size_t)r * sg.stride];
      s1 += col[(size_t)(r + RED_RG) * sg.stride];
      s2 += col[(size_t)(r + 2 * RED_RG) * sg.stride];
      s3 += col[(size_t)(r + 3 * RED_RG) * sg.stride];
    }
    for (; r < sg.rows; r += RED_RG) s0 += col[(size_t)r * sg.stride];
    s = (s0 + s1) + (s2 + s3);
  }
  part[rg][c] = s;
  __syncthreads();
  if (rg == 0 && j < sg.len) {
    float tt = 0.f;
#pragma unroll
    for (int k = 0; k < RED_RG; ++k) tt += part[k][c];
    if (!ADD || overwrite) grad[sg.dst + j] = tt;
    else atomicAdd(grad + sg.dst + j, tt);
  }
}

template <bool ADD = true>
__global__ __launch_bounds__(256) void reduce_segments_rows_kernel(SegTable t, float* __restrict__ grad, int overwrite) {
  const cgvp_segment sg = t.s[blockIdx.y];
  const int j = blockIdx.x * 256 + threadIdx.x;
  if (j >= sg.len) return;
  const float* col = sg.slab + sg.col0 + j;
  float s = 0.f;
  for (int r = 0; r < sg.rows; ++r) s += col[(size_t)r * sg.stride];
  if (!ADD || overwrite) grad[sg.dst + j] = s;
  else atomicAdd(grad + sg.dst + j, s);
}

struct SrcSumArgs {
  const float* rows; const float* self; const int32_t* sptr; const int32_t* spos;
  const int32_t* rowptr; const float* slot; int64_t waves; int64_t N; float* out;
};
template <int W>
__global__ __launch_bounds__(256) void src_sum_kernel(SrcSumArgs a) {
  const int64_t t = (int64_t)blockIdx.x * 256 + threadIdx.x;
  if (t >= a.N * W) return;
  const int64_t n = t / W;
  const int c = (int)(t - n * W);
  float s = a.self ? a.self[t] : 0.f;
  const int32_t k0 = a.sptr[n], k1 = a.sptr[n + 1];
#pragma unroll 4
  for (int32_t k = k0; k < k1; ++k) s += a.rows[(int64_t)a.spos[k] * W + c];
  if (a.slot) {
    const int64_t ev = a.rowptr[a.N];
    const int64_t iters = (ev + TILE - 1) / TILE, chunk = (iters + a.waves - 1) / a.waves * TILE;
    const int64_t r0 = a.rowptr[n], r1 = a.rowptr[n + 1];
    if (chunk > 0)
      for (int64_t w = r0 / chunk + 1; w * chunk < r1; ++w) s += a.slot[w * W + c];
  }
  a.out[t] = s;
}

inline int bwd_grid_cap(int64_t units) {
  static const int forced = [] {
    const char* e = getenv("CGVP_BWD_GRID");
    const int v = e ? atoi(e) : 0;
    return (v >= 1 && v <= BW_MAX_GRID) ? v : 0;
  }();
  if (forced) return forced;
  constexpr int SMALL = BW_MAX_GRID - 8;
  return units <= (int64_t)SMALL * BW_WPB ? SMALL : BW_MAX_GRID;
}
inline bool one_tile_per_wave(int64_t tiles, int grid) {
  static const bool on = [] { const char* e = getenv("CGVP_BWD_STORE_ONCE"); return !(e && e[0] == '0'); }();
  return on && tiles <= (int64_t)grid * BW_WPB;
}
inline int grid_for(int64_t tiles) {
  const int cap = bwd_grid_cap(tiles);
  return (int)(tiles < 1 ? 1 : (tiles > cap ? cap : tiles));
}

}

namespace quad {

int bwd_block_sizes(int nt_node, int nt_edge, BwdBlocks* b) {
  if (nt_node == 0) b->emb = EmbBlk<0>::SIZE; else if (nt_node == 20) b->emb = EmbBlk<20>::SIZE;
  else if (nt_node == 21) b->emb = EmbBlk<21>::SIZE; else return CGVP_ERR_UNSUPPORTED_DIMS;
  if (nt_edge == 0) { b->conv_edge = EdgeBlk<0>::SIZE; b->conv_total = ConvBlk<0>::SIZE; }
  else if (nt_edge == 1) { b->conv_edge = EdgeBlk<1>::SIZE; b->conv_total = ConvBlk<1>::SIZE; }
  else return CGVP_ERR_UNSUPPORTED_DIMS;
  b->node = NODE_GB;
  b->head = HEAD_GB;
  return 0;
}

template <bool ADD>
void launch_reduce_segments(const SegTable& t, int nsegs, int maxlen, int maxrows, float* grad_params, hipStream_t st,
                            int overwrite) {
  if (maxrows <= 32) {
    launch<reduce_segments_rows_kernel<ADD>>(dim3((maxlen + 255) / 256, nsegs), dim3(256), 0, st, t, grad_params, overwrite);
    return;
  }
  launch<reduce_segments_kernel<ADD>>(dim3((maxlen + RED_COLS - 1) / RED_COLS, nsegs), dim3(RED_COLS * RED_RG), 0,
                                      st, t, grad_params, overwrite);
}

int reduce_segments(const cgvp_segment* segs, int nsegs, float* grad_params, hipStream_t st, int overwrite, bool store_only) {
  if (nsegs <= 0) return 0;
  SegTable t;
  int maxlen = 0;
  int maxrows = 0;
  for (int i = 0; i < nsegs; ++i) {
    t.s[i] = segs[i];
    maxlen = segs[i].len > maxlen ? segs[i].len : maxlen;
    maxrows = segs[i].rows > maxrows ? segs[i].rows : maxrows;
  }
  if (store_only) launch_reduce_segments<false>(t, nsegs, maxlen, maxrows, grad_params, st, 1);
  else launch_reduce_segments<true>(t, nsegs, maxlen, maxrows, grad_params, st, overwrite);
  return 0;
}

int src_sum(int width, const float* rows, const float* self, const int32_t* sptr, const int32_t* spos,
            const int32_t* rowptr, const float* slot, int64_t waves, int64_t N, float* out, hipStream_t st) {
  if (N <= 0) return 0;
  SrcSumArgs a{rows, self, sptr, spos, rowptr, slot, waves, N, out};
  const unsigned blocks = (unsigned)((N * width + 255) / 256);
  switch (width) {
    case 16: return launch<src_sum_kernel<16>>(dim3(blocks), dim3(256), 0, st, a);
    case ROW: return launch<src_sum_kernel<ROW>>(dim3(blocks), dim3(256), 0, st, a);
    case 41: return launch<src_sum_kernel<41>>(dim3(blocks), dim3(256), 0, st, a);
    case 52: return launch<src_sum_kernel<52>>(dim3(blocks), dim3(256), 0, st, a);
    default: return CGVP_ERR_UNSUPPORTED_DIMS;
  }
}

int conv_bwd_max_waves() { return BW_MAX_GRID * 8; }

int reduce_slab(const float* slab, int rows, int stride, int col0, int len, float* dst, hipStream_t st) {
  if (rows <= 32) {
    launch<reduce_rows_kernel>(dim3((len + 255) / 256), dim3(256), 0, st, slab, rows, stride, col0, len, dst);
    return 0;
  }
  launch<reduce_slab_kernel>(dim3((len + RED_COLS - 1) / RED_COLS), dim3(RED_COLS * RED_RG), 0, st, slab, rows, stride, col0, len, dst);
  return 0;
}

int node_update_bwd(const float* img_node, const float* imgT_node, const float* h, const float* dh,
                    const float* mask0, const float* mask1, gvp::RngArgs rng, const float* g_up0, const float* g_up1,
                    const float* g_up2, int64_t N, float* g_dh, float* g_h, float* zero_rows, float* slab, int* grid,
                    int policy, hipStream_t st) {
  NodeBArgs a{img_node, imgT_node, h, dh, mask0, mask1, rng, g_up0, g_up1, g_up2, N, g_dh, g_h, zero_rows, slab};
  const int64_t tiles = (N + TILE - 1) / TILE;
  const int G = grid_for(tiles);
  *grid = G;
  const size_t lds = (size_t)node_bwd_lds_floats() * sizeof(float);
  return with_policy<true>(policy, [&](auto tag) {
    using ST = typename decltype(tag)::type;
    return with_flag(one_tile_per_wave(tiles, G), [&](auto one) {
      return launch<node_bwd_kernel<ST, one.value>>(dim3(G), dim3(BW_TPB), lds, st, a);
    });
  });
}

int node_head_bwd(const float* img_head, const float* imgT_head, const float* h_out, const float* g_out, float* g_h_out,
                  float* head_slab, const float* img_node, const float* imgT_node, const float* h, const float* dh,
                  const float* mask0, const float* mask1, gvp::RngArgs rng, int64_t N, float* g_dh, float* g_h,
                  float* zero_rows, float* slab, int* grid, int policy, hipStream_t st) {
  HeadBArgs hd{img_head, imgT_head, h_out, g_out, N, g_h_out, head_slab};
  NodeBArgs a{img_node, imgT_node, h, dh, mask0, mask1, rng, g_h_out, nullptr, nullptr, N, g_dh, g_h, zero_rows, slab};
  const int64_t tiles = (N + TILE - 1) / TILE;
  const int G = grid_for(tiles);
  *grid = G;
  const int f = node_bwd_lds_floats() > head_bwd_lds_floats() ? node_bwd_lds_floats() : head_bwd_lds_floats();
  const size_t lds = (size_t)f * sizeof(float);
  return with_policy<false>(policy, [&](auto tag) {
    using ST = typename decltype(tag)::type;
    return with_flag(one_tile_per_wave(tiles, G), [&](auto one) {
      return launch<node_head_bwd_kernel<ST, one.value>>(dim3(G), dim3(BW_TPB), lds, st, hd, a);
    });
  });
}

int head_bwd(const float* img_head, const float* imgT_head, const float* h_out, const float* g_out, int64_t N,
             float* g_h_out, float* slab, int* grid, int policy, hipStream_t st) {
  HeadBArgs a{img_head, imgT_head, h_out, g_out, N, g_h_out, slab};
  const int G = grid_for((N + TILE - 1) / TILE);
  *grid = G;
  const size_t lds = (size_t)head_bwd_lds_floats() * sizeof(float);
  return with_policy<false>(policy, [&](auto tag) {
    return launch<head_bwd_kernel<typename decltype(tag)::type>>(dim3(G), dim3(BW_TPB), lds, st, a);
  });
}

int conv_bwd_version() {
  static const int v = [] {
    const char* e = getenv("CGVP_CONV_BWD");
    return (e && e[0] == '1') ? 1 : ((e && e[0] == '2') ? 2 : 3);
  }();
  return v;
}

template <int NTE, int TN, int WPB_, bool STORE>
int conv_bwd2_impl(ConvBArgs& a, int64_t E, int* grid, int policy, hipStream_t st) {
  typedef C2Shape<TN, WPB_> SH;
  const int64_t iters = (E + TN * TILE - 1) / (TN * TILE);
  const int64_t wgs = (iters + WPB_ - 1) / WPB_;
  const int cap = bwd_grid_cap(((E + TILE - 1) / TILE + 1) / 2);
  const int G = (int)(wgs < 1 ? 1 : (wgs > cap ? cap : wgs));
  *grid = G;
  const size_t lds = (size_t)SH::template lds_floats<NTE>() * sizeof(float);
  return with_policy<NTE == 0>(policy, [&](auto tag) {
    return launch<conv_bwd2_kernel<NTE, typename decltype(tag)::type, TN, WPB_, STORE>>(dim3(G), dim3(SH::TPB), lds, st, a);
  });
}

template <int NTE>
int conv_bwd_impl(ConvBArgs& a, int* grid, int policy, hipStream_t st) {
  const int64_t ngroups = (a.N + a.npw - 1) / a.npw;
  const int64_t wgs = (ngroups + CB_WPB - 1) / CB_WPB;
  const int cap = bwd_grid_cap(ngroups);
  const int G = (int)(wgs < 1 ? 1 : (wgs > cap ? cap : wgs));
  *grid = G;
  const size_t lds = (size_t)conv_bwd_lds_floats<NTE>() * sizeof(float);
  return with_policy<NTE == 0>(policy, [&](auto tag) {
    return launch<conv_bwd_kernel<NTE, typename decltype(tag)::type>>(dim3(G), dim3(CB_TPB), lds, st, a);
  });
}

template <int NTE>
int conv_bwd_version_impl(ConvBArgs& a, int64_t E, int* grid, int policy, hipStream_t st) {
  if (a.g_edge) return conv_bwd2_impl<NTE, 1, 8, true>(a, E, grid, policy, st);
  if (conv_bwd_version() == 2) return conv_bwd2_impl<NTE, 2, 4, false>(a, E, grid, policy, st);
  if (conv_bwd_version() == 3) return conv_bwd2_impl<NTE, 1, 8, false>(a, E, grid, policy, st);
  return conv_bwd_impl<NTE>(a, grid, policy, st);
}

int conv_bwd(int nt_edge, const float* img, const float* imgT, const float* h, const float* e_emb,
             const int32_t* rowptr, const int32_t* esrc, const int32_t* edst, int64_t N, int64_t E, int mean,
             const float* g_dh, float* g_src, float* g_dst, float* g_e, float* slab, int* grid, int policy, hipStream_t st,
             float* g_edge, float* slot) {
  int64_t deg = N > 0 ? (E + N - 1) / N : 1;
  if (deg < 1) deg = 1;
  int npw = (int)((2 * TILE - 2) / deg);
  npw = npw < 1 ? 1 : (npw > WAVE ? WAVE : npw);
  ConvBArgs a{img, imgT, h, e_emb, rowptr, esrc, edst, N, npw, mean, g_dh, g_src, g_dst, g_e, slab, g_edge, slot};
  if (g_edge && (conv_bwd_version() != 3 || !slot)) return CGVP_ERR_NONDETERMINISTIC;
  if (nt_edge == 0) return conv_bwd_version_impl<0>(a, E, grid, policy, st);
  if (nt_edge == 1) return conv_bwd_version_impl<1>(a, E, grid, policy, st);
  return CGVP_ERR_UNSUPPORTED_DIMS;
}

template <int NTE>
int edge_bwd_impl(EdgeBArgs& a, int* grid, int policy, hipStream_t st) {
  const int64_t tiles = (a.E + TILE - 1) / TILE;
  const int G = (int)(tiles < 1 ? 1 : (tiles > 2 * bwd_grid_cap((tiles + 1) / 2) ? 2 * bwd_grid_cap((tiles + 1) / 2) : tiles));
  *grid = G;
  const size_t lds = (size_t)edge_bwd_lds_floats<NTE>() * sizeof(float);
  return with_policy<false>(policy, [&](auto tag) {
    using ST = typename decltype(tag)::type;
    return with_flag(a.g_e_s != nullptr, [&](auto dx) {
      return launch<edge_bwd_kernel<NTE, ST, dx.value>>(dim3(G), dim3(BW_TPB), lds, st, a);
    });
  });
}

int edge_embed_bwd(int nt_edge, const float* img, const float* imgT, const float* e_s, const float* e_v,
                   const int64_t* etypes, const int32_t* eperm, int64_t E, const float* const* g_e, int n_g,
                   float* g_e_s, float* g_e_v, float* slab, int* grid, int policy, hipStream_t st) {
  if (n_g < 1 || n_g > EB_MAX_LAYERS) return CGVP_ERR_BAD_ARG;
  if ((g_e_s == nullptr) != (g_e_v == nullptr)) return CGVP_ERR_BAD_ARG;
  EdgeBArgs a{img, imgT, e_s, e_v, etypes, eperm, E, {}, n_g, slab, g_e_s, g_e_v};
  for (int l = 0; l < n_g; ++l) a.g_e[l] = g_e[l];
  if (nt_edge == 0) return edge_bwd_impl<0>(a, grid, policy, st);
  if (nt_edge == 1) return edge_bwd_impl<1>(a, grid, policy, st);
  return CGVP_ERR_UNSUPPORTED_DIMS;
}

template <int NTN>
int embed_bwd_impl(EmbBArgs& a, int* grid, int policy, hipStream_t st) {
  const int64_t tiles = (a.N + TILE - 1) / TILE;
  const int G = grid_for(tiles);
  *grid = G;
  const size_t lds = (size_t)embed_bwd_lds_floats<NTN>() * sizeof(float);
  return with_policy<false>(policy, [&](auto tag) {
    using ST = typename decltype(tag)::type;
    return with_flag(one_tile_per_wave(tiles, G), [&](auto one) {
      return launch<embed_bwd_kernel<NTN, ST, one.value>>(dim3(G), dim3(BW_TPB), lds, st, a);
    });
  });
}

int node_embed_bwd(int nt_node, const float* img, const float* imgT, const float* x_s, const float* x_v,
                   const int64_t* ntypes, int64_t N, const float* g_up0, const float* g_up1, const float* g_up2,
                   float* g_x_s, float* g_x_v, float* slab, int* grid, int policy, hipStream_t st) {
  EmbBArgs a{img, imgT, x_s, x_v, ntypes, N, g_up0, g_up1, g_up2, g_x_s, g_x_v, slab};
  if (nt_node == 0) return embed_bwd_impl<0>(a, grid, policy, st);
  if (nt_node == 20) return embed_bwd_impl<20>(a, grid, policy, st);
  if (nt_node == 21) return embed_bwd_impl<21>(a, grid, policy, st);
  return CGVP_ERR_UNSUPPORTED_DIMS;
}

}
```

caster-dta_amd/csrc/pass_api.hip:

```cpp
#include <hip/hip_runtime.h>
#include <stdint.h>
#include <stdlib.h>

#include <atomic>
#include <mutex>
#include <vector>

#include "gvp_internal.h"

namespace {

struct TimedLaunch { hipEvent_t a, b; int kind; };
std::atomic<bool> g_timing{false};
std::mutex g_timed_mutex;
std::vector<TimedLaunch> g_timed;
struct Timed {
  hipStream_t st; bool on; TimedLaunch t;
  Timed(int kind, void* stream) : st((hipStream_t)stream), on(g_timing.load(std::memory_order_relaxed)) {
    if (!on) return;
    t.kind = kind;
    if (hipEventCreate(&t.a) != hipSuccess || hipEventCreate(&t.b) != hipSuccess) { on = false; return; }
    (void)hipEventRecord(t.a, st);
  }
  ~Timed() {
// ... 35 lines not shown
  d->work = b.take(quad::src_index_work_ints(N, E) * 4);
  d->rows = b.take((E > 0 ? E : 1) * width * 4);
  d->extra = b.take(extra_floats * 4);
}
inline bool det_mode(int32_t flags) { return (flags & CGVP_BWD_DETERMINISTIC) || quad::deterministic_env(); }

struct LbaBwdWs {
  int64_t slabs, g_e, rows, total;
  int64_t slab_floats, g_e_stride, row_floats;
  int det; DetWs det_ws;
};
int lba_bwd_layout(const cgvp_dims* dims, const cgvp_layout* layout, int64_t N, int64_t E, LbaBwdWs* w, bool det = false) {
  const int64_t wsz = cgvp_bwd_workspace_floats(dims, layout);
  if (wsz < 0) return (int)wsz;
  const int nc = num_convs_of(*layout);
  Bump b;
  w->slab_floats = wsz;
  w->slabs = b.take((int64_t)(2 * nc + 2) * wsz * 4);
  w->g_e_stride = up((E + 1) * EROW * 4, 256) / 4;
  w->g_e = b.take((int64_t)nc * w->g_e_stride * 4);
  w->row_floats = up(N * ROW * 4, 256) / 4;
  w->rows = b.take(8 * w->row_floats * 4);
  w->total = b.off;
  w->det = 0;
  if (det) take_det(b, N, E, ROW, ROW * (int64_t)quad::conv_bwd_max_waves(), &w->det_ws);
  if (det) { w->det = 1; w->total = b.off; }
  return 0;
}

inline int gine_layer_floats(int cin, int chid, int cout, int ke) {
  return 1 + chid * cin + chid + cout * chid + cout + cin * ke + cin;
}
int check_gine_cfg(const cgvp_gine_cfg* c) {
  if (!c || c->num_layers < 1 || c->num_layers > CGVP_GINE_MAX_LAYERS) return CGVP_ERR_BAD_ARG;
  if (c->num_ntypes < 0 || c->num_etypes < 0 || c->edge_dim < 0) return CGVP_ERR_BAD_ARG;
  for (int l = 0; l <= c->num_layers; ++l)
    if (c->widths[l] < 1 || c->widths[l] > 64) return CGVP_ERR_UNSUPPORTED_DIMS;
  if (c->widths[0] <= c->num_ntypes) return CGVP_ERR_BAD_ARG;
  return 0;
}
struct GineBwdWs { int64_t slabs, gx, total, slab_floats, gx_floats; int det; DetWs det_ws; };
void gine_bwd_layout(const cgvp_gine_cfg* c, int64_t N, GineBwdWs* w, int64_t E = 0, bool det = false) {
  Bump b;
  w->slab_floats = cgvp_gine_bwd_workspace_floats();
  w->slabs = b.take((int64_t)c->num_layers * w->slab_floats * 4);
  int maxw = 0;
  for (int l = 1; l < c->num_layers; ++l) maxw = c->widths[l] > maxw ? c->widths[l] : maxw;
  w->gx_floats = up(N * maxw * 4, 256) / 4;
  w->gx = b.take((int64_t)(c->num_layers - 1) * w->gx_floats * 4);
  w->total = b.off;
  w->det = 0;
  if (det) {
    int maxx = 0;
    for (int l = 0; l < c->num_layers; ++l) {
      const int xw = c->widths[l] - (l == 0 ? c->num_ntypes : 0);
      maxx = xw > maxx ? xw : maxx;
    }
    take_det(b, N, E, maxx, N * maxx, &w->det_ws);
    w->det = 1;
    w->total = b.off;
  }
}

struct StageTable { cgvp_stage_item it[CGVP_MAX_STAGE]; };
__global__ __launch_bounds__(256) void stage_kernel(StageTable t) {
  const cgvp_stage_item it = t.it[blockIdx.y];
  const int64_t words = it.capacity_bytes >> 2, copy = it.copy_bytes >> 2;
  uint32_t* __restrict__ d = static_cast<uint32_t*>(it.dst);
  const uint32_t* __restrict__ s = static_cast<const uint32_t*>(it.src);
  const bool vec = !(((uintptr_t)d | (uintptr_t)s) & 15);
  if (vec) {
    const int64_t c4 = copy >> 2, w4 = words >> 2;
    for (int64_t i = (int64_t)blockIdx.x * 256 + threadIdx.x; i < w4; i += (int64_t)gridDim.x * 256) {
      uint4 v = make_uint4(it.fill_word, it.fill_word, it.fill_word, it.fill_word);
      if (i < c4) v = reinterpret_cast<const uint4*>(s)[i];
      else if (i == c4 && (copy & 3)) {
        const int64_t b = i << 2;
        v.x = b < copy ? s[b] : it.fill_word; v.y = b + 1 < copy ? s[b + 1] : it.fill_word;
        v.z = b + 2 < copy ? s[b + 2] : it.fill_word; v.w = it.fill_word;
      }
      reinterpret_cast<uint4*>(d)[i] = v;
    }
    for (int64_t i = (w4 << 2) + (int64_t)blockIdx.x * 256 + threadIdx.x; i < words; i += (int64_t)gridDim.x * 256)
      d[i] = i < copy ? s[i] : it.fill_word;
    return;
  }
  for (int64_t i = (int64_t)blockIdx.x * 256 + threadIdx.x; i < words; i += (int64_t)gridDim.x * 256)
    d[i] = i < copy ? s[i] : it.fill_word;
}

}

extern "C" {

int cgvp_stage_buffers(const cgvp_stage_item* items, int32_t n, void* stream) {
  if (n < 0 || n > CGVP_MAX_STAGE || (n > 0 && !items)) return CGVP_ERR_BAD_ARG;
  if (n == 0) return 0;
  StageTable t;
  int64_t most = 0;
  for (int i = 0; i < n; ++i) {
    const cgvp_stage_item& it = items[i];
    if (it.copy_bytes < 0 || it.capacity_bytes < it.copy_bytes || (it.copy_bytes & 3) || (it.capacity_bytes & 3)) return CGVP_ERR_BAD_ARG;
    if ((it.capacity_bytes > 0 && !it.dst) || (it.copy_bytes > 0 && !it.src)) return CGVP_ERR_BAD_ARG;
    if (((uintptr_t)it.dst & 3) || ((uintptr_t)it.src & 3)) return CGVP_ERR_BAD_ARG;
    t.it[i] = it;
    most = it.capacity_bytes > most ? it.capacity_bytes : most;
  }
  int64_t blocks = (most / 16 + 255) / 256;
  blocks = blocks < 1 ? 1 : (blocks > 2048 ? 2048 : blocks);
  launch<stage_kernel>(dim3((unsigned)blocks, (unsigned)n), dim3(256), 0, (hipStream_t)stream, t);
  return launch_status();
}

int cgvp_lba_fwd_workspace(const cgvp_dims* dims, const cgvp_layout* layout, int64_t N, int64_t E, int32_t save_state,
                           cgvp_lba_fwd_ws* out) {
  if (!dims || !layout || !out || N < 0 || E < 0) return CGVP_ERR_BAD_ARG;
  if (dims->layer_kind != CGVP_LAYER_GATED) return CGVP_ERR_UNSUPPORTED_DIMS;
  const int64_t img = cgvp_lba_image_floats(dims, layout);
  if (img < 0) return (int)img;
  const int nc = num_convs_of(*layout);
  Bump b;
  out->seed = b.take(16);
  out->image = b.take(img * 4);
  out->state_rows = save_state ? 2 * nc + 1 : 3;
  out->node_stride = N + (N & 1);
  out->state = b.take(out->state_rows * out->node_stride * ROW * esize(dims));
  out->e_emb = b.take((E + 1) * EROW * esize(dims) > E * 4 ? (E + 1) * EROW * esize(dims) : E * 4);
  out->ids_scratch = out->e_emb;
  out->rowptr = b.take((N + 1) * 4);
  out->eperm = b.take((E > 0 ? E : 1) * 4);
  out->esrc = b.take((E > 0 ? E : 1) * 4);
  out->edst = b.take((E > 0 ? E : 1) * 4);
  out->total = b.off;
  return 0;
}

int cgvp_lba_forward_plan(int64_t N, int64_t E, int32_t num_convs, int32_t prebuilt_csr, int32_t flags, int32_t* fused_layers) {
  if (N < 0 || E < 0 || num_convs < 1) return CGVP_ERR_BAD_ARG;
  const int fuse = !(flags & CGVP_PASS_UNFUSED) && E <= 4 * N;
  if (fused_layers) *fused_layers = fuse;
  int launches = 1 + (prebuilt_csr ? 0 : (E > 0 ? 3 : 2));
  if (N > 0) launches += num_convs * (fuse ? 1 : 2);
  return launches;
}

int cgvp_lba_forward_pass(const cgvp_dims* dims, const cgvp_layout* layout, const float* params,
                          const cgvp_lba_batch* batch, int32_t aggr_mean, float dropout_p, uint64_t* rng_state,
                          const float* masks, int32_t* csr_counters, void* workspace, int32_t save_state,
                          int32_t flags, float* out, void* stream) {
  if (!dims || !layout || !params || !batch || !workspace) return CGVP_ERR_BAD_ARG;
  if ((uintptr_t)workspace & 255) return CGVP_ERR_BAD_ARG;
  const int64_t N = batch->num_nodes, E = batch->num_edges;
  cgvp_lba_fwd_ws ws;
  if (int rc = cgvp_lba_fwd_workspace(dims, layout, N, E, save_state, &ws)) return rc;
  const int nc = num_convs_of(*layout);
  if (nc < 1) return CGVP_ERR_UNSUPPORTED_DIMS;
  if (!(dropout_p >= 0.f && dropout_p < 1.f)) return CGVP_ERR_BAD_ARG;
  const bool drop = dropout_p > 0.f && save_state;
  const bool draw = drop && !masks;
  if (draw && !rng_state) return CGVP_ERR_BAD_ARG;
  const bool tables = has_tables(batch);
  if (tables && (E > 0 && (!batch->eperm || !batch->esrc || !batch->edst))) return CGVP_ERR_BAD_ARG;
  if (!tables && E > 0 && (!batch->edge_index || !csr_counters)) return CGVP_ERR_BAD_ARG;
  if (N > 0 && !out) return CGVP_ERR_BAD_ARG;
  const int es = esize(dims);
  float* image = at<float>(workspace, ws.image);
  uint64_t* seed = at<uint64_t>(workspace, ws.seed);
  char* state = at<char>(workspace, ws.state);
  const int64_t srow = ws.node_stride * ROW * es;
  auto row = [&](int64_t r) { return reinterpret_cast<float*>(state + r * srow); };
  float* e_emb = at<float>(workspace, ws.e_emb);
  int32_t* rowptr = tables ? const_cast<int32_t*>(batch->rowptr) : at<int32_t>(workspace, ws.rowptr);
  int32_t* eperm = tables ? const_cast<int32_t*>(batch->eperm) : at<int32_t>(workspace, ws.eperm);
  int32_t* esrc = tables ? const_cast<int32_t*>(batch->esrc) : at<int32_t>(workspace, ws.esrc);
  int32_t* edst = tables ? const_cast<int32_t*>(batch->edst) : at<int32_t>(workspace, ws.edst);
  const bool count_here = !tables && E > 0;
  if (int rc = cgvp_lba_pass_begin(dims, layout, params, image, batch->x_s, batch->x_v, batch->ntypes, N, row(0),
                                   draw ? rng_state : nullptr, draw ? seed : nullptr,
                                   count_here ? batch->edge_index : nullptr, E, count_here ? csr_counters : nullptr, stream))
    return rc;
  if (!tables) {
    if (!csr_counters) return CGVP_ERR_BAD_ARG;
    if (int rc = cgvp_csr_from_coo(batch->edge_index, N, E, rowptr, eperm, esrc, edst, csr_counters, count_here ? 2 : 1,
                                   at<int32_t>(workspace, ws.ids_scratch), stream))
      return rc;
  }
  if (N == 0) return 0;
  int32_t fuse_i = 0;
  (void)cgvp_lba_forward_plan(N, E, nc, tables ? 1 : 0, flags, &fuse_i);
  const bool fuse = fuse_i != 0;
  const int64_t mstride = N * MROW;
  for (int l = 0; l < nc; ++l) {
    const bool last = l == nc - 1;
    cgvp_rng rng{draw ? seed : nullptr, dropout_p, 2 * l};
    const cgvp_rng* rp = draw ? &rng : nullptr;
    const float* m0 = (drop && masks) ? masks + (int64_t)(2 * l) * mstride : nullptr;
    const float* m1 = (drop && masks) ? masks + (int64_t)(2 * l + 1) * mstride : nullptr;
    float *h, *dh, *h_out;
    if (save_state) { h = row(l); dh = row(nc + l); h_out = last ? row(2 * nc) : row(l + 1); }
    else { h = row(l & 1); dh = fuse ? nullptr : row(2); h_out = last ? nullptr : row((l + 1) & 1); }
    const float* e_in = l > 0 ? e_emb : nullptr;
    float* e_out = l == 0 ? e_emb : nullptr;
    if (fuse) {
      Timed timed(0, stream);
      if (int rc = cgvp_conv_layer_fwd(dims, layout, image, l, h, batch->e_s, batch->e_v, batch->etypes, rowptr, eperm, esrc,
                                       edst, N, E, aggr_mean, m0, m1, rp, last ? 1 : 0, e_in, e_out, dh, h_out, out, stream))
        return rc;
    } else {
      {
        Timed timed(0, stream);
        if (int rc = cgvp_conv_fwd(dims, layout, params, image, l, h, batch->e_s, batch->e_v, batch->etypes, rowptr, eperm,
                                   esrc, edst, N, E, aggr_mean, e_in, e_out, dh, stream))
          return rc;
      }
      if (!save_state && last) h_out = row((l + 1) & 1);
      if (int rc = cgvp_node_update_fwd_train(dims, layout, image, l, h, dh, m0, m1, rp, N, last ? 1 : 0, h_out, out, stream))
        return rc;
    }
  }
  return launch_status();
}

int64_t cgvp_lba_bwd_workspace_bytes_ex(const cgvp_dims* dims, const cgvp_layout* layout, int64_t N, int64_t E,
                                        int32_t flags) {
  if (!dims || !layout || N < 0 || E < 0) return CGVP_ERR_BAD_ARG;
  if (dims->layer_kind != CGVP_LAYER_GATED) return CGVP_ERR_UNSUPPORTED_DIMS;
  LbaBwdWs w;
  if (int rc = lba_bwd_layout(dims, layout, N, E, &w, det_mode(flags))) return rc;
  return w.total;
}

int64_t cgvp_lba_bwd_workspace_bytes(const cgvp_dims* dims, const cgvp_layout* layout, int64_t N, int64_t E) {
  if (!dims || !layout || N < 0 || E < 0) return CGVP_ERR_BAD_ARG;
  if (dims->layer_kind != CGVP_LAYER_GATED) return CGVP_ERR_UNSUPPORTED_DIMS;
  LbaBwdWs w;
  if (int rc = lba_bwd_layout(dims, layout, N, E, &w)) return rc;
  return w.total;
}

int cgvp_lba_backward_pass(const cgvp_dims* dims, const cgvp_layout* layout, const cgvp_lba_batch* batch,
                           int32_t aggr_mean, float dropout_p, const float* masks, const void* fwd_workspace,
                           const float* g_out, void* bwd_workspace, float* grad_params, float* g_x_s, float* g_x_v,
                           float* g_e_s, float* g_e_v, void* stream) {
  if (quad::deterministic_env()) return CGVP_ERR_NONDETERMINISTIC;
  return cgvp_lba_backward_pass_ex(dims, layout, batch, aggr_mean, dropout_p, masks, fwd_workspace, g_out, bwd_workspace,
                                   grad_params, g_x_s, g_x_v, g_e_s, g_e_v, 0, stream);
}

int cgvp_lba_backward_pass_ex(const cgvp_dims* dims, const cgvp_layout* layout, const cgvp_lba_batch* batch,
                              int32_t aggr_mean, float dropout_p, const float* masks, const void* fwd_workspace,
                              const float* g_out, void* bwd_workspace, float* grad_params, float* g_x_s, float* g_x_v,
                              float* g_e_s, float* g_e_v, int32_t flags, void* stream) {
  const bool det = det_mode(flags);
  if (!dims || !layout || !batch || !fwd_workspace || !bwd_workspace || !grad_params) return CGVP_ERR_BAD_ARG;
  if (((uintptr_t)fwd_workspace & 255) || ((uintptr_t)bwd_workspace & 255)) return CGVP_ERR_BAD_ARG;
  if ((g_x_s == nullptr) != (g_x_v == nullptr) || (g_e_s == nullptr) != (g_e_v == nullptr)) return CGVP_ERR_BAD_ARG;
  const int64_t N = batch->num_nodes, E = batch->num_edges;
  cgvp_lba_fwd_ws ws;
  if (int rc = cgvp_lba_fwd_workspace(dims, layout, N, E, 1, &ws)) return rc;
  LbaBwdWs bw;
  if (int rc = lba_bwd_layout(dims, layout, N, E, &bw, det)) return rc;
  const int nc = num_convs_of(*layout);
  if (nc < 1) return CGVP_ERR_UNSUPPORTED_DIMS;
  hipStream_t st = (hipStream_t)stream;
  if (N == 0) {
    quad::zero_words(grad_params, (size_t)layout->total, st);
    return launch_status();
  }
  if (!g_out) return CGVP_ERR_BAD_ARG;
  const bool drop = dropout_p > 0.f;
  const bool draw = drop && !masks;
  const int es = esize(dims);
  const float* image = at<float>(fwd_workspace, ws.image);
  const uint64_t* seed = at<uint64_t>(fwd_workspace, ws.seed);
  const char* state = at<char>(fwd_workspace, ws.state);
  const int64_t srow = ws.node_stride * ROW * es;
  auto row = [&](int64_t r) { return reinterpret_cast<const float*>(state + r * srow); };
  const float* e_emb = at<float>(fwd_workspace, ws.e_emb);
  const bool tables = has_tables(batch);
  const int32_t* rowptr = tables ? batch->rowptr : at<int32_t>(fwd_workspace, ws.rowptr);
  const int32_t* eperm = tables ? batch->eperm : at<int32_t>(fwd_workspace, ws.eperm);
  const int32_t* esrc = tables ? batch->esrc : at<int32_t>(fwd_workspace, ws.esrc);
  const int32_t* edst = tables ? batch->edst : at<int32_t>(fwd_workspace, ws.edst);
  float* slabs = at<float>(bwd_workspace, bw.slabs);
  float* g_e = at<float>(bwd_workspace, bw.g_e);
  float* rows = at<float>(bwd_workspace, bw.rows);
  auto buf = [&](int l, int k) { return rows + (int64_t)((l & 1) * 4 + k) * bw.row_floats; };
  cgvp_segment segs[CGVP_MAX_SEGS];
  int nseg = 0, stage = 0;
  int32_t cnt = 0;
  auto region = [&]() { return slabs + (int64_t)(stage++) * bw.slab_floats; };
  if (2 * nc + 2 + 1 > CGVP_MAX_SEGS) return CGVP_ERR_UNSUPPORTED_DIMS;
  const int64_t mstride = N * MROW;
  quad::DetBufs db{};
  if (det) {
    const DetWs& d = bw.det_ws;
    db = quad::DetBufs{at<int32_t>(bwd_workspace, d.sptr), at<int32_t>(bwd_workspace, d.spos),
                       at<float>(bwd_workspace, d.rows), at<float>(bwd_workspace, d.extra)};
    if (int rc = quad::src_index(rowptr, esrc, N, E, at<int32_t>(bwd_workspace, d.sptr), at<int32_t>(bwd_workspace, d.spos),
                                 at<int32_t>(bwd_workspace, d.work), st))
      return rc;
  }
  const float *up0 = nullptr, *up1 = nullptr, *up2 = nullptr;
  for (int l = nc - 1; l >= 0; --l) {
    const bool last = l == nc - 1;
    float* g_dh = buf(l, 0);
    float* g_h = drop ? buf(l, 1) : nullptr;
    float* g_src = buf(l, 2);
    float* g_dst = buf(l, 3);
    cgvp_rng rng{draw ? seed : nullptr, dropout_p, 2 * l};
    const float* m0 = (drop && masks) ? masks + (int64_t)(2 * l) * mstride : nullptr;
    const float* m1 = (drop && masks) ? masks + (int64_t)(2 * l + 1) * mstride : nullptr;
    if (int rc = cgvp_node_update_bwd(dims, layout, image, l, row(l), row(nc + l), m0, m1, draw ? &rng : nullptr,
                                      last ? row(2 * nc) : nullptr, last ? g_out : nullptr, up0, up1, up2, N, last ? 1 : 0,
                                      g_dh, g_h, g_src, grad_params, region(), segs + nseg, &cnt, stream))
      return rc;
    nseg += cnt;
    {
      Timed timed(1, stream);
      if (int rc = quad::conv_bwd_entry(dims, layout, image, l, row(l), e_emb, rowptr, esrc, edst, N, E, aggr_mean, g_dh, g_src,
                                        1, g_dst, g_e + (int64_t)l * bw.g_e_stride, grad_params, region(), segs + nseg, &cnt,
                                        stream, det ? &db : nullptr))
        return rc;
    }
    nseg += cnt;
    up0 = g_h ? g_h : g_dh; up1 = g_src; up2 = g_dst;
  }
  if (int rc = cgvp_node_embed_bwd(dims, layout, image, batch->x_s, batch->x_v, batch->ntypes, N, up0, up1, up2, g_x_s, g_x_v,
                                   grad_params, region(), segs + nseg, &cnt, stream))
    return rc;
  nseg += cnt;
  if (E > 0) {
    const float* ge[16];
    if (nc > 16) return CGVP_ERR_UNSUPPORTED_DIMS;
    for (int l = 0; l < nc; ++l) ge[l] = g_e + (int64_t)l * bw.g_e_stride;
    if (int rc = cgvp_edge_embed_bwd(dims, layout, image, batch->e_s, batch->e_v, batch->etypes, eperm, E, ge, nc,
                                     g_e_s, g_e_v, grad_params, region(), segs + nseg, &cnt, stream))
      return rc;
    nseg += cnt;
  } else {
    quad::zero_words(grad_params + layout->edge_gvp, (size_t)(layout->conv0 - layout->edge_gvp), st);
  }
  if (det) quad::reduce_segments(segs, nseg, grad_params, st, 1, true);
  else if (int rc = cgvp_bwd_reduce(segs, nseg, grad_params, 1, stream)) return rc;
  return launch_status();
}

int cgvp_gine_fwd_workspace(const cgvp_gine_cfg* cfg, int64_t N, int64_t E, int32_t save_state, cgvp_gine_fwd_ws* out) {
  if (int rc = check_gine_cfg(cfg)) return rc;
  if (!out || N < 0 || E < 0) return CGVP_ERR_BAD_ARG;
  const int L = cfg->num_layers;
  Bump b;
  out->seed = b.take(16);
  for (int l = 0; l < CGVP_GINE_MAX_LAYERS; ++l) out->hidden[l] = out->agg[l] = out->pos[l] = 0;
  if (save_state) {
    for (int l = 0; l < L - 1; ++l) out->hidden[l] = b.take(N * cfg->widths[l + 1] * 4);
    for (int l = 0; l < L; ++l) {
      out->agg[l] = b.take(N * ((cfg->widths[l] + 15) / 16 * 16) * 4);
      out->pos[l] = b.take((E > 0 ? E : 1) * 8);
    }
  } else {
    int maxw = 1;
    for (int l = 1; l < L; ++l) maxw = cfg->widths[l] > maxw ? cfg->widths[l] : maxw;
    const int64_t a = b.take(N * maxw * 4), c = b.take(N * maxw * 4);
    for (int l = 0; l < L - 1; ++l) out->hidden[l] = (l & 1) ? c : a;
  }
  out->rowptr = b.take((N + 1) * 4);
  out->eperm = b.take((E > 0 ? E : 1) * 4);
  out->esrc = b.take((E > 0 ? E : 1) * 4);
  out->edst = b.take((E > 0 ? E : 1) * 4);
  out->saved = b.off;
  out->ids_scratch = b.take((E > 0 ? E : 1) * 4);
  out->total = b.off;
  return 0;
}

int cgvp_gine_forward_pass(const cgvp_gine_cfg* cfg, const cgvp_gine_w* w, const cgvp_gine_batch* batch, float dropout_p,
                           uint64_t* rng_state, const float* const* masks, int32_t* csr_counters, void* workspace,
                           int32_t save_state, int32_t variant, float* out, void* stream) {
  if (!cfg || !w || !batch || !workspace || ((uintptr_t)workspace & 255)) return CGVP_ERR_BAD_ARG;
  const int64_t N = batch->num_nodes, E = batch->num_edges;
  cgvp_gine_fwd_ws ws;
  if (int rc = cgvp_gine_fwd_workspace(cfg, N, E, save_state, &ws)) return rc;
  if (!(dropout_p >= 0.f && dropout_p < 1.f)) return CGVP_ERR_BAD_ARG;
  const int L = cfg->num_layers;
  const bool drop = dropout_p > 0.f && save_state && L > 1;
  const bool draw = drop && !masks;
  if (draw && !rng_state) return CGVP_ERR_BAD_ARG;
  const bool tables = has_tables(batch);
  if (!tables && (!csr_counters || (E > 0 && !batch->edge_index))) return CGVP_ERR_BAD_ARG;
  if (N > 0 && !out) return CGVP_ERR_BAD_ARG;
  hipStream_t st = (hipStream_t)stream;
  uint64_t* seed = at<uint64_t>(workspace, ws.seed);
  const int32_t* rowptr = tables ? batch->rowptr : at<int32_t>(workspace, ws.rowptr);
  const int32_t* eperm = tables ? batch->eperm : at<int32_t>(workspace, ws.eperm);
  const int32_t* esrc = tables ? batch->esrc : at<int32_t>(workspace, ws.esrc);
  const int32_t* edst = tables ? batch->edst : at<int32_t>(workspace, ws.edst);
  if (!tables) {
    if (int rc = quad::csr_build(batch->edge_index, N, E, at<int32_t>(workspace, ws.rowptr), at<int32_t>(workspace, ws.eperm),
                                 at<int32_t>(workspace, ws.esrc), at<int32_t>(workspace, ws.edst), csr_counters, 1,
                                 at<int32_t>(workspace, ws.ids_scratch),
                                 draw ? reinterpret_cast<unsigned long long*>(rng_state) : nullptr,
                                 draw ? reinterpret_cast<unsigned long long*>(seed) : nullptr, st))
      return rc;
  } else if (draw) {
    if (int rc = cgvp_rng_next(rng_state, seed, stream)) return rc;
  }
  if (N == 0) return 0;
  const float* x = batch->x;
  for (int l = 0; l < L; ++l) {
    const bool first = l == 0, lastl = l == L - 1;
    float* y = lastl ? out : at<float>(workspace, ws.hidden[l]);
    cgvp_rng rng{draw ? seed : nullptr, dropout_p, l};
    const bool dl = drop && !lastl;
    bool done = false;
    if (save_state) {
      if (((uintptr_t)x & 15) || ((uintptr_t)y & 15)) return CGVP_ERR_BAD_ARG;
      gvp::RngArgs ra{(dl && draw) ? reinterpret_cast<const unsigned long long*>(seed) : nullptr, dropout_p, l};
      if (!(dl && draw)) ra = gvp::RngArgs{nullptr, 0.f, 0};
      const int rc = quad::gine_fwd(cfg->widths[l], cfg->widths[l + 1], cfg->widths[l + 1], first ? cfg->num_ntypes : 0,
                                    cfg->num_etypes, cfg->edge_dim, x, first ? batch->ntypes : nullptr, batch->eattr,
                                    batch->etypes, rowptr, eperm, esrc, edst, N, w + l, cfg->act_slope,
                                    (dl && masks) ? masks[l] : nullptr, ra, y,
                                    gine_recompute() ? nullptr : at<float>(workspace, ws.agg[l]),
                                    gine_recompute() ? nullptr : at<uint16_t>(workspace, ws.pos[l]), st);
      if (rc < 0 || rc > 1) return rc;
      done = rc == 0;
    }
    if (!done)
      if (int rc = cgvp_gine_conv_fwd(x, first ? batch->ntypes : nullptr, first ? cfg->num_ntypes : 0, batch->eattr, batch->etypes,
                                      cfg->num_etypes, cfg->edge_dim, rowptr, eperm, esrc, edst, N, E, cfg->widths[l],
                                      cfg->widths[l + 1], cfg->widths[l + 1], w + l, cfg->act_slope,
                                      (dl && masks) ? masks[l] : nullptr, (dl && draw) ? &rng : nullptr, variant, y, stream))
        return rc;
    x = y;
  }
  return launch_status();
}

int64_t cgvp_gine_bwd_workspace_bytes(const cgvp_gine_cfg* cfg, int64_t N, int64_t E) {
  if (int rc = check_gine_cfg(cfg)) return rc;
  if (N < 0 || E < 0) return CGVP_ERR_BAD_ARG;
  GineBwdWs w;
  gine_bwd_layout(cfg, N, &w);
  return w.total;
}

int64_t cgvp_gine_bwd_workspace_bytes_ex(const cgvp_gine_cfg* cfg, int64_t N, int64_t E, int32_t flags) {
  if (int rc = check_gine_cfg(cfg)) return rc;
  if (N < 0 || E < 0) return CGVP_ERR_BAD_ARG;
  GineBwdWs w;
  gine_bwd_layout(cfg, N, &w, E, det_mode(flags));
  return w.total;
}

int cgvp_gine_backward_pass(const cgvp_gine_cfg* cfg, const cgvp_gine_w* w, const cgvp_gine_batch* batch, float dropout_p,
                            const float* const* masks, const void* fwd_workspace, const float* g_out, void* bwd_workspace,
                            float* grad_flat, float* g_x, int32_t max_workgroups, void* stream) {
  if (quad::deterministic_env()) return CGVP_ERR_NONDETERMINISTIC;
  return cgvp_gine_backward_pass_eattr(cfg, w, batch, dropout_p, masks, fwd_workspace, g_out, bwd_workspace, grad_flat, g_x,
                                       nullptr, max_workgroups, 0, stream);
}

int cgvp_gine_backward_pass_ex(const cgvp_gine_cfg* cfg, const cgvp_gine_w* w, const cgvp_gine_batch* batch, float dropout_p,
                               const float* const* masks, const void* fwd_workspace, const float* g_out, void* bwd_workspace,
                               float* grad_flat, float* g_x, int32_t max_workgroups, int32_t flags, void* stream) {
  return cgvp_gine_backward_pass_eattr(cfg, w, batch, dropout_p, masks, fwd_workspace, g_out, bwd_workspace, grad_flat, g_x,
                                       nullptr, max_workgroups, flags, stream);
}

int cgvp_gine_backward_pass_eattr(const cgvp_gine_cfg* cfg, const cgvp_gine_w* w, const cgvp_gine_batch* batch, float dropout_p,
                                  const float* const* masks, const void* fwd_workspace, const float* g_out, void* bwd_workspace,
                                  float* grad_flat, float* g_x, float* g_eattr, int32_t max_workgroups, int32_t flags,
                                  void* stream) {
  const bool det = det_mode(flags);
  if (det && gine_recompute()) return CGVP_ERR_NONDETERMINISTIC;
  if (!cfg || !w || !batch || !fwd_workspace || !bwd_workspace || !grad_flat) return CGVP_ERR_BAD_ARG;
  if (((uintptr_t)fwd_workspace & 255) || ((uintptr_t)bwd_workspace & 255)) return CGVP_ERR_BAD_ARG;
  const int64_t N = batch->num_nodes, E = batch->num_edges;
  cgvp_gine_fwd_ws ws;
  if (int rc = cgvp_gine_fwd_workspace(cfg, N, E, 1, &ws)) return rc;
  GineBwdWs bw;
  gine_bwd_layout(cfg, N, &bw, E, det);
  const int L = cfg->num_layers;
  const int ke = cfg->num_etypes + cfg->edge_dim;
  hipStream_t st = (hipStream_t)stream;
  int64_t total = 0;
  int loff[CGVP_GINE_MAX_LAYERS];
  for (int l = 0; l < L; ++l) { loff[l] = (int)total; total += gine_layer_floats(cfg->widths[l], cfg->widths[l + 1], cfg->widths[l + 1], ke); }
  if (N == 0) {
    quad::zero_words(grad_flat, (size_t)total, st);
    return launch_status();
  }
  if (!g_out) return CGVP_ERR_BAD_ARG;
  const bool drop = dropout_p > 0.f && L > 1;
  const bool draw = drop && !masks;
  const uint64_t* seed = at<uint64_t>(fwd_workspace, ws.seed);
  const bool tables = has_tables(batch);
  const int32_t* rowptr = tables ? batch->rowptr : at<int32_t>(fwd_workspace, ws.rowptr);
  const int32_t* eperm = tables ? batch->eperm : at<int32_t>(fwd_workspace, ws.eperm);
  const int32_t* esrc = tables ? batch->esrc : at<int32_t>(fwd_workspace, ws.esrc);
  const int32_t* edst = tables ? batch->edst : at<int32_t>(fwd_workspace, ws.edst);
  float* slabs = at<float>(bwd_workspace, bw.slabs);
  float* gx = at<float>(bwd_workspace, bw.gx);
  const DetWs& dw = bw.det_ws;
  if (det) {
    if (int rc = quad::src_index(rowptr, esrc, N, E, at<int32_t>(bwd_workspace, dw.sptr), at<int32_t>(bwd_workspace, dw.spos),
                                 at<int32_t>(bwd_workspace, dw.work), st))
      return rc;
  } else {
    if (L > 1) quad::zero_words(gx, (size_t)(L - 1) * bw.gx_floats, st);
    if (g_x) quad::zero_words(g_x, (size_t)N * (cfg->widths[0] - cfg->num_ntypes), st);
  }
  cgvp_segment segs[CGVP_GINE_MAX_LAYERS];
  const float* g = g_out;
  for (int l = L - 1; l >= 0; --l) {
    const bool first = l == 0;
    const float* x = first ? batch->x : at<float>(fwd_workspace, ws.hidden[l - 1]);
    float* gxl = first ? g_x : gx + (int64_t)(l - 1) * bw.gx_floats;
    const bool dl = drop && l < L - 1;
    gvp::RngArgs ra{(dl && draw) ? reinterpret_cast<const unsigned long long*>(seed) : nullptr, dropout_p, l};
    if (!(dl && draw)) ra = gvp::RngArgs{nullptr, 0.f, 0};
    const float* mask = (dl && masks) ? masks[l] : nullptr;
    if (((uintptr_t)g & 15) || ((uintptr_t)mask & 15)) return CGVP_ERR_BAD_ARG;
    int rows = 0, row_len = 0;
    float* slab = slabs + (int64_t)l * bw.slab_floats;
    if (int rc = quad::gine_bwd(cfg->widths[l], cfg->widths[l + 1], cfg->widths[l + 1], first ? cfg->num_ntypes : 0,
                                cfg->num_etypes, cfg->edge_dim, x, first ? batch->ntypes : nullptr, batch->eattr, batch->etypes,
                                rowptr, eperm, esrc, edst, N, w + l, cfg->act_slope, mask, ra, g, gxl, slab, max_workgroups,
                                &rows, &row_len, st, gine_recompute() ? nullptr : at<float>(fwd_workspace, ws.agg[l]),
                                gine_recompute() ? nullptr : at<uint16_t>(fwd_workspace, ws.pos[l]),
                                det ? at<float>(bwd_workspace, dw.rows) : nullptr,
                                (det && gxl) ? at<float>(bwd_workspace, dw.extra) : nullptr,
                                g_eattr, l < L - 1))
      return rc;
    if (det && gxl)
      if (int rc = quad::src_sum(cfg->widths[l] - (first ? cfg->num_ntypes : 0), at<float>(bwd_workspace, dw.rows),
                                 at<float>(bwd_workspace, dw.extra), at<int32_t>(bwd_workspace, dw.sptr),
                                 at<int32_t>(bwd_workspace, dw.spos), rowptr, nullptr, 0, N, gxl, st))
        return rc;
    segs[l] = cgvp_segment{slab, rows, row_len, 0,
                           gine_layer_floats(cfg->widths[l], cfg->widths[l + 1], cfg->widths[l + 1], ke), loff[l]};
    g = gxl;
  }
  if (det) quad::reduce_segments(segs, L, grad_flat, st, 1, true);
  else quad::reduce_segments(segs, L, grad_flat, st, 1);
  return launch_status();
}

int cgvp_debug_kernel_timing(int32_t enable) {
  g_timing.store(enable != 0, std::memory_order_relaxed);
  return 0;
}

int cgvp_debug_kernel_times(float* ms, int32_t* kinds, int32_t capacity) {
  int n = 0;
  std::vector<TimedLaunch> taken;
  {
    std::lock_guard<std::mutex> lock(g_timed_mutex);
    taken.swap(g_timed);
  }
  for (const TimedLaunch& t : taken) {
    float v = 0.f;
    (void)hipEventSynchronize(t.b);
    (void)hipEventElapsedTime(&v, t.a, t.b);
    if (n < capacity && ms && kinds) { ms[n] = v; kinds[n] = t.kind; }
    ++n;
    (void)hipEventDestroy(t.a);
    (void)hipEventDestroy(t.b);
  }
  return n;
}

}
```

Measured before the change: 279,400 graph-pairs/sec.

## Fuse node-update and conv backward into one kernel for inner GVP layers

Adds a fused node_conv_bwd kernel that runs the node-update backward and the edge-conv backward for non-last layers in a single launch. Each workgroup owns a dst-sorted edge range (found with a boundary search) and the node tiles for that range, so the conv pass can consume g_dh without a separate kernel boundary. The layer-below g_src buffer is now zeroed inside the previous node kernel instead of separately. The fused path is enabled heuristically only for f32 when grid capacity covers the node tiles, and it adds LDS pressure and range-partition complexity.

```diff
diff --git a/caster-dta_amd/csrc/gvp_internal.h b/caster-dta_amd/csrc/gvp_internal.h
--- a/caster-dta_amd/csrc/gvp_internal.h
+++ b/caster-dta_amd/csrc/gvp_internal.h
@@ -56,13 +56,33 @@
 int node_update_bwd(const float* img_node, const float* imgT_node, const float* h, const float* dh,
                     const float* mask0, const float* mask1, gvp::RngArgs rng, const float* g_up0, const float* g_up1,
                     const float* g_up2, int64_t N, float* g_dh, float* g_h, float* zero_rows, float* slab, int* grid,
-                    int policy, hipStream_t st);
+                    int policy, hipStream_t st, float* zero_rows2 = nullptr);
 int head_bwd(const float* img_head, const float* imgT_head, const float* h_out, const float* g_out, int64_t N,
              float* g_h_out, float* slab, int* grid, int policy, hipStream_t st);
 int node_head_bwd(const float* img_head, const float* imgT_head, const float* h_out, const float* g_out, float* g_h_out,
                   float* head_slab, const float* img_node, const float* imgT_node, const float* h, const float* dh,
                   const float* mask0, const float* mask1, gvp::RngArgs rng, int64_t N, float* g_dh, float* g_h,
-                  float* zero_rows, float* slab, int* grid, int policy, hipStream_t st);
+                  float* zero_rows, float* slab, int* grid, int policy, hipStream_t st, float* zero_rows2 = nullptr);
+bool fuse_node_conv(int policy, int64_t N, int64_t E);
+int node_conv_bwd(int nt_edge, const float* img_node, const float* imgT_node, const float* h, const float* dh,
+                  const float* mask0, const float* mask1, gvp::RngArgs rng, const float* g_up0, const float* g_up1,
+                  const float* g_up2, float* g_dh, float* g_h, float* zero_rows, float* node_slab, const float* img,
+                  const float* imgT, const float* e_emb, const int32_t* rowptr, const int32_t* esrc, const int32_t* edst,
+                  int64_t N, int64_t E, int mean, float* g_src, float* g_dst, float* g_e, float* conv_slab, int* grid,
+                  hipStream_t st);
+int node_bwd_entry(const cgvp_dims* dims, const cgvp_layout* layout, const float* image, int32_t layer, const float* h,
+                   const float* dh, const float* mask0, const float* mask1, const cgvp_rng* rng, const float* h_out,
+                   const float* g_out, const float* g_up0, const float* g_up1, const float* g_up2, int64_t N,
+                   int32_t with_head, float* g_dh, float* g_h, float* zero_out, float* zero_out2, float* grad_params,
+                   float* workspace, cgvp_segment* segs, int32_t* nsegs, void* stream);
+int node_conv_bwd_entry(const cgvp_dims* dims, const cgvp_layout* layout, const float* image, int32_t layer,
+                        const float* h, const float* dh, const float* mask0, const float* mask1, const cgvp_rng* rng,
+                        const float* g_up0, const float* g_up1, const float* g_up2, const float* e_emb,
+                        const int32_t* rowptr, const int32_t* esrc, const int32_t* edst, int64_t N, int64_t E,
+                        int32_t aggr_mean, float* g_dh, float* g_h, float* zero_out, float* g_src, float* g_dst,
+                        float* g_e, float* node_workspace, float* conv_workspace, cgvp_segment* segs, int32_t* nsegs,
+                        void* stream);
+int policy_index(const cgvp_dims* dims);
 int conv_bwd(int nt_edge, const float* img, const float* imgT, const float* h, const float* e_emb,
              const int32_t* rowptr, const int32_t* esrc, const int32_t* edst, int64_t N, int64_t E, int mean,
              const float* g_dh, float* g_src, float* g_dst, float* g_e, float* slab, int* grid, int policy, hipStream_t st,
diff --git a/caster-dta_amd/csrc/gvp_kernels.hip b/caster-dta_amd/csrc/gvp_kernels.hip
--- a/caster-dta_amd/csrc/gvp_kernels.hip
+++ b/caster-dta_amd/csrc/gvp_kernels.hip
@@ -928,6 +928,27 @@
                          const float* g_up2, int64_t N, int32_t with_head, float* g_dh, float* g_h,
                          float* zero_out, float* grad_params, float* workspace, cgvp_segment* segs, int32_t* nsegs,
                          void* stream) {
+  return quad::node_bwd_entry(dims, layout, image, layer, h, dh, mask0, mask1, rng, h_out, g_out, g_up0, g_up1, g_up2, N,
+                              with_head, g_dh, g_h, zero_out, nullptr, grad_params, workspace, segs, nsegs, stream);
+}
+
+int cgvp_conv_bwd(const cgvp_dims* dims, const cgvp_layout* layout, const float* image, int32_t layer,
+                  const float* h, const float* e_emb, const int32_t* rowptr, const int32_t* esrc,
+                  const int32_t* edst, int64_t N, int64_t E, int32_t aggr_mean, const float* g_dh, float* g_src,
+                  int32_t g_src_zeroed, float* g_dst, float* g_e, float* grad_params, float* workspace,
+                  cgvp_segment* segs, int32_t* nsegs, void* stream) {
+  if (quad::deterministic_env()) return CGVP_ERR_NONDETERMINISTIC;
+  return quad::conv_bwd_entry(dims, layout, image, layer, h, e_emb, rowptr, esrc, edst, N, E, aggr_mean, g_dh, g_src,
+                              g_src_zeroed, g_dst, g_e, grad_params, workspace, segs, nsegs, stream, nullptr);
+}
+}
+
+int quad::node_bwd_entry(const cgvp_dims* dims, const cgvp_layout* layout, const float* image, int32_t layer,
+                         const float* h, const float* dh, const float* mask0, const float* mask1, const cgvp_rng* rng,
+                         const float* h_out, const float* g_out, const float* g_up0, const float* g_up1,
+                         const float* g_up2, int64_t N, int32_t with_head, float* g_dh, float* g_h, float* zero_out,
+                         float* zero_out2, float* grad_params, float* workspace, cgvp_segment* segs, int32_t* nsegs,
+                         void* stream) {
   if (int rc = check_dims(dims)) return rc;
   if (int rc = check_rng(rng)) return rc;
   if (N < 0 || !layout || !image || !grad_params || !workspace) return CGVP_ERR_BAD_ARG;
@@ -936,7 +957,7 @@
   if (N == 0) return 0;
   if (!h || !dh || !g_dh || (with_head && (!g_out || !h_out))) return CGVP_ERR_BAD_ARG;
   if (with_head && dims->layer_kind != CGVP_LAYER_GATED) return CGVP_ERR_UNSUPPORTED_DIMS;
-  const void* al[] = {h, dh, mask0, mask1, h_out, g_out, g_up0, g_up1, g_up2, g_dh, g_h, zero_out};
+  const void* al[] = {h, dh, mask0, mask1, h_out, g_out, g_up0, g_up1, g_up2, g_dh, g_h, zero_out, zero_out2};
   for (const void* q : al) if ((uintptr_t)q & 15) return CGVP_ERR_BAD_ARG;
   BwdLookup o;
   if (int rc = bwd_lookup(*layout, &o)) return rc;
@@ -948,7 +969,7 @@
     if (int rc = quad::node_head_bwd(image + o.head, image + o.headT, h_out, g_out, g_dh, head_slab,
                                      image + o.node0 + layer * o.layer_stride, image + o.nodeT0 + layer * o.layerT_stride,
                                      h, dh, mask0, mask1, rng_args(rng, 2 * layer), N, g_dh, g_h, zero_out, workspace, &grid,
-                                     policy_of(dims), st)) return rc;
+                                     policy_of(dims), st, zero_out2)) return rc;
     hgrid = grid;
   } else {
   if (with_head) {
@@ -957,7 +978,7 @@
   }
   if (int rc = quad::node_update_bwd(image + o.node0 + layer * o.layer_stride, image + o.nodeT0 + layer * o.layerT_stride,
                                      h, dh, mask0, mask1, rng_args(rng, 2 * layer), g_up0, g_up1, g_up2, N, g_dh, g_h, zero_out,
-                                     workspace, &grid, policy_of(dims), st)) return rc;
+                                     workspace, &grid, policy_of(dims), st, zero_out2)) return rc;
   }
   const int node_len = conv_ff1() + LFf1::size(0) - conv_ln0();
   cgvp_segment sg[2] = {{workspace, grid, o.blk.node, 0, node_len, layout->conv0 + layer * layout->conv_stride + conv_ln0()},
@@ -965,15 +986,38 @@
   return emit_segments(sg, with_head ? 2 : 1, segs, nsegs, grad_params, st);
 }
 
-int cgvp_conv_bwd(const cgvp_dims* dims, const cgvp_layout* layout, const float* image, int32_t layer,
-                  const float* h, const float* e_emb, const int32_t* rowptr, const int32_t* esrc,
-                  const int32_t* edst, int64_t N, int64_t E, int32_t aggr_mean, const float* g_dh, float* g_src,
-                  int32_t g_src_zeroed, float* g_dst, float* g_e, float* grad_params, float* workspace,
-                  cgvp_segment* segs, int32_t* nsegs, void* stream) {
-  if (quad::deterministic_env()) return CGVP_ERR_NONDETERMINISTIC;
-  return quad::conv_bwd_entry(dims, layout, image, layer, h, e_emb, rowptr, esrc, edst, N, E, aggr_mean, g_dh, g_src,
-                              g_src_zeroed, g_dst, g_e, grad_params, workspace, segs, nsegs, stream, nullptr);
-}
+int quad::policy_index(const cgvp_dims* dims) { return policy_of(dims); }
+
+int quad::node_conv_bwd_entry(const cgvp_dims* dims, const cgvp_layout* layout, const float* image, int32_t layer,
+                              const float* h, const float* dh, const float* mask0, const float* mask1,
+                              const cgvp_rng* rng, const float* g_up0, const float* g_up1, const float* g_up2,
+                              const float* e_emb, const int32_t* rowptr, const int32_t* esrc, const int32_t* edst,
+                              int64_t N, int64_t E, int32_t aggr_mean, float* g_dh, float* g_h, float* zero_out,
+                              float* g_src, float* g_dst, float* g_e, float* node_workspace, float* conv_workspace,
+                              cgvp_segment* segs, int32_t* nsegs, void* stream) {
+  if (int rc = check_dims(dims)) return rc;
+  if (int rc = check_rng(rng)) return rc;
+  if (N <= 0 || E <= 0 || !layout || !image || !node_workspace || !conv_workspace || !segs || !nsegs) return CGVP_ERR_BAD_ARG;
+  const int nc = num_convs_of(*layout);
+  if (layer < 0 || layer >= nc - 1) return CGVP_ERR_BAD_ARG;
+  if (!h || !dh || !g_dh || !g_src || !g_dst || !rowptr || !e_emb || !g_e || !esrc || !edst) return CGVP_ERR_BAD_ARG;
+  if (policy_of(dims) != POLICY_F32) return CGVP_ERR_UNSUPPORTED_DIMS;
+  const void* al[] = {h, dh, mask0, mask1, g_up0, g_up1, g_up2, g_dh, g_h, zero_out, e_emb, g_src, g_dst, g_e};
+  for (const void* q : al) if ((uintptr_t)q & 15) return CGVP_ERR_BAD_ARG;
+  BwdLookup o;
+  if (int rc = bwd_lookup(*layout, &o)) return rc;
+  int grid = 0;
+  if (int rc = quad::node_conv_bwd(layout->nt_edge, image + o.node0 + layer * o.layer_stride,
+                                   image + o.nodeT0 + layer * o.layerT_stride, h, dh, mask0, mask1,
+                                   rng_args(rng, 2 * layer), g_up0, g_up1, g_up2, g_dh, g_h, zero_out, node_workspace,
+                                   image + o.conv0 + layer * o.layer_stride, image + o.convT0 + layer * o.layerT_stride,
+                                   e_emb, rowptr, esrc, edst, N, E, aggr_mean ? 1 : 0, g_src, g_dst, g_e, conv_workspace,
+                                   &grid, (hipStream_t)stream)) return rc;
+  const int node_len = conv_ff1() + LFf1::size(0) - conv_ln0();
+  const int base = layout->conv0 + layer * layout->conv_stride;
+  const cgvp_segment sg[2] = {{node_workspace, grid, o.blk.node, 0, node_len, base + conv_ln0()},
+                              {conv_workspace, grid, o.blk.conv_total, 0, conv_ln0(), base}};
+  return emit_segments(sg, 2, segs, nsegs, nullptr, (hipStream_t)stream);
 }
 
 int quad::conv_bwd_entry(const cgvp_dims* dims, const cgvp_layout* layout, const float* image, int32_t layer,
diff --git a/caster-dta_amd/csrc/gvp_quad_bwd_kernels.hip b/caster-dta_amd/csrc/gvp_quad_bwd_kernels.hip
--- a/caster-dta_amd/csrc/gvp_quad_bwd_kernels.hip
+++ b/caster-dta_amd/csrc/gvp_quad_bwd_kernels.hip
@@ -1,4 +1,5 @@
 #include <hip/hip_runtime.h>
+#include <stddef.h>
 #include <stdint.h>
 #include <stdlib.h>
 
@@ -6,6 +7,7 @@
 
 #include "gvp_internal.h"
 #include "gvp_quad.h"
+#include "gvp_range.h"
 
 using namespace gq;
 
@@ -62,10 +64,10 @@
   for (int k = lane; k < BLK / 4; k += WAVE) reinterpret_cast<f4*>(gblk)[k] = f4{0.f, 0.f, 0.f, 0.f};
 }
 template <int BLK, int PW, int WPB_ = 8>
-__device__ __forceinline__ void write_slab_row(float* slab, const float* blocks, int row = blockIdx.x) {
+__device__ __forceinline__ void write_slab_row(float* slab, const float* blocks, int row = blockIdx.x, int tid = threadIdx.x) {
   __syncthreads();
   float* out = slab + (size_t)row * BLK;
-  for (int k = threadIdx.x; k < BLK; k += WAVE * WPB_) {
+  for (int k = tid; k < BLK; k += WAVE * WPB_) {
     float t = 0.f;
 #pragma unroll
     for (int ww = 0; ww < WPB_; ++ww) t += blocks[ww * PW + k];
@@ -134,9 +136,129 @@
   const float* h; const float* dh; const float* mask0; const float* mask1; gvp::RngArgs rng;
   const float* g_up0; const float* g_up1; const float* g_up2;
   int64_t N; float* g_dh; float* g_h; float* zero_rows; float* slab;
+  float* zero_rows2 = nullptr;
 };
 constexpr int node_bwd_lds_floats() { return BW_TPB + Image<0, 0>::ND_SIZE + Image<0, 0>::TN_SIZE + BW_WPB * (NODE_GB + TSCR_FLOATS); }
 static_assert(node_bwd_lds_floats() * 4 <= 160 * 1024, "node backward LDS plan exceeds the CU");
+
+template <typename ST, class Acc>
+__device__ __forceinline__ void node_bwd_tile(const NodeBArgs& a, const float* f_node, const float* t_node, float* gblk,
+                                              float* tscr, int lane, int64_t n, bool active) {
+  typedef Image<0, 0> IM;
+  const int g = lane >> 4;
+  const f4 zero = {0.f, 0.f, 0.f, 0.f};
+  const int zt[1] = {0};
+  const bool first = false;
+  {
+    f4 x0[1] = {zero};
+    float xv0[3][1] = {{0.f}, {0.f}, {0.f}};
+    f4 m0s = {1.f, 1.f, 1.f, 1.f}, m1s = {1.f, 1.f, 1.f, 1.f};
+    float m0v = 1.f, m1v = 1.f;
+    f4 gs[1] = {zero};
+    float gv[3][1] = {{0.f}, {0.f}, {0.f}};
+    if (active) {
+      const int64_t hr = n * ROW;
+      node_dropout(a.mask0, a.rng, 0, n, g, m0s, m0v);
+      node_dropout(a.mask1, a.rng, 1, n, g, m1s, m1v);
+      x0[0] = Io<ST>::ld4(a.h, hr + 4 * g) + Io<ST>::ld4(a.dh, hr + 4 * g) * m0s;
+#pragma unroll
+      for (int p = 0; p < 3; ++p) xv0[p][0] = Io<ST>::ld(a.h, hr + NS + 3 * g + p) + Io<ST>::ld(a.dh, hr + NS + 3 * g + p) * m0v;
+      const float* ups[3] = {a.g_up0, a.g_up1, a.g_up2};
+#pragma unroll
+      for (int u = 0; u < 3; ++u)
+        if (ups[u]) {
+          const float* r_ = ups[u] + n * ROW;
+          gs[0] += *reinterpret_cast<const f4*>(r_ + 4 * g);
+#pragma unroll
+          for (int p = 0; p < 3; ++p) gv[p][0] += r_[NS + 3 * g + p];
+        }
+    }
+    f4 y[1] = {x0[0]};
+    float yv[3][1] = {{xv0[0][0]}, {xv0[1][0]}, {xv0[2][0]}};
+    ln_quad<NS, NV>(f_node + IM::ND_LN0, lane, y, yv);
+    f4 hs[1][4], s2[1][1];
+    float hv[1][3][2], v2[1][3][1];
+    float bs0[1][4], bv0[1][3][1], bs1[1][16], bv1[1][3][2];
+    typename Ff0<ST>::Cache c0[1];
+    typename Ff1<ST>::Cache c1[1];
+#pragma unroll
+    for (int r = 0; r < 4; ++r) bs0[0][r] = y[0][r];
+#pragma unroll
+    for (int p = 0; p < 3; ++p) bv0[0][p][0] = yv[p][0];
+    Ff0<ST>::template forward<1, Io<ST>::BF>(f_node + IM::ND_FF0, lane, zt, bs0, bv0, hs, hv, c0);
+#pragma unroll
+    for (int t = 0; t < 4; ++t)
+#pragma unroll
+      for (int r = 0; r < 4; ++r) bs1[0][4 * t + r] = hs[0][t][r];
+#pragma unroll
+    for (int p = 0; p < 3; ++p) { bv1[0][p][0] = hv[0][p][0]; bv1[0][p][1] = hv[0][p][1]; }
+    Ff1<ST>::template forward<1, Io<ST>::BF>(f_node + IM::ND_FF1, lane, zt, bs1, bv1, s2, v2, c1);
+    f4 z[1] = {y[0] + s2[0][0] * m1s};
+    float zv[3][1];
+#pragma unroll
+    for (int p = 0; p < 3; ++p) zv[p][0] = yv[p][0] + v2[0][p][0] * m1v;
+
+    STAMP(2);
+    STAMP(3);
+    {
+      f4 dga[1], dbe[1];
+      ln_quad_bwd<NS, NV>(f_node + IM::ND_LN1, lane, z, zv, gs, gv, dga, dbe);
+      ln_param_grads<Acc, NS>(gblk + NB_LN1, first, lane, active, dga, dbe);
+    }
+    float d_hs[16], d_hv[3][2];
+    {
+      f4 d_so[1] = {gs[0] * m1s};
+      float d_vo[3][1] = {{gv[0][0] * m1v}, {gv[1][0] * m1v}, {gv[2][0] * m1v}};
+      typename Ff1<ST>::Grads gr1;
+      STAMP(4);
+      Ff1<ST>::template backward<Io<ST>::BF>(t_node + IM::TN_FF1, lane, c1[0], d_so, d_vo, d_hs, d_hv, gr1);
+      STAMP(5);
+      Ff1<ST>::template weight_grads<Acc, Io<ST>::BF>(gblk + NB_FF1, first, lane, 0, active, bs1[0], bv1[0], c1[0], gr1, tscr);
+    }
+    {
+      f4 d_so[4];
+#pragma unroll
+      for (int t = 0; t < 4; ++t) d_so[t] = f4{d_hs[4 * t], d_hs[4 * t + 1], d_hs[4 * t + 2], d_hs[4 * t + 3]};
+      float d_ys[4], d_yv[3][1];
+      typename Ff0<ST>::Grads gr0;
+      STAMP(6);
+      Ff0<ST>::template backward<Io<ST>::BF>(t_node + IM::TN_FF0, lane, c0[0], d_so, d_hv, d_ys, d_yv, gr0);
+      STAMP(7);
+      Ff0<ST>::template weight_grads<Acc, Io<ST>::BF>(gblk + NB_FF0, first, lane, 0, active, bs0[0], bv0[0], c0[0], gr0, tscr);
+#pragma unroll
+      for (int r = 0; r < 4; ++r) gs[0][r] += d_ys[r];
+#pragma unroll
+      for (int p = 0; p < 3; ++p) gv[p][0] += d_yv[p][0];
+    }
+    STAMP(8);
+    {
+      f4 dga[1], dbe[1];
+      ln_quad_bwd<NS, NV>(f_node + IM::ND_LN0, lane, x0, xv0, gs, gv, dga, dbe);
+      ln_param_grads<Acc, NS>(gblk + NB_LN0, first, lane, active, dga, dbe);
+    }
+    if (active) {
+      if (a.g_h) {
+        float* row = a.g_h + n * ROW;
+        *reinterpret_cast<f4*>(row + 4 * g) = gs[0];
+#pragma unroll
+        for (int p = 0; p < 3; ++p) row[NS + 3 * g + p] = gv[p][0];
+      }
+      float* row = a.g_dh + n * ROW;
+      *reinterpret_cast<f4*>(row + 4 * g) = gs[0] * m0s;
+#pragma unroll
+      for (int p = 0; p < 3; ++p) row[NS + 3 * g + p] = gv[p][0] * m0v;
+      float* zs[2] = {a.zero_rows, a.zero_rows2};
+#pragma unroll
+      for (int u = 0; u < 2; ++u)
+        if (zs[u]) {
+          float* z = zs[u] + n * ROW;
+          *reinterpret_cast<f4*>(z + 4 * g) = zero;
+#pragma unroll
+          for (int p = 0; p < 3; ++p) z[NS + 3 * g + p] = 0.f;
+        }
+    }
+  }
+}
 
 template <typename ST, bool ONE = false>
 __device__ __forceinline__ void node_bwd_body(const NodeBArgs& a, float* lds) {
@@ -155,118 +277,11 @@
   __syncthreads();
   STAMP(1);
 
-  const f4 zero = {0.f, 0.f, 0.f, 0.f};
-  const int zt[1] = {0};
-  const bool first = false;
   const int64_t ntiles = (a.N + TILE - 1) / TILE;
   for (int64_t tile = (int64_t)w * gridDim.x + blockIdx.x; tile < ntiles; tile += (int64_t)gridDim.x * BW_WPB) {
-    const int lane = opaque_lane(lane0), i = lane & 15, g = lane >> 4;
-    const int64_t n = tile * TILE + i;
-    const bool active = n < a.N;
-    f4 x0[1] = {zero};
-    float xv0[3][1] = {{0.f}, {0.f}, {0.f}};
-    f4 m0s = {1.f, 1.f, 1.f, 1.f}, m1s = {1.f, 1.f, 1.f, 1.f};
-    float m0v = 1.f, m1v = 1.f;
-    f4 gs[1] = {zero};
-    float gv[3][1] = {{0.f}, {0.f}, {0.f}};
-    if (active) {
-      const int64_t hr = n * ROW;
-      node_dropout(a.mask0, a.rng, 0, n, g, m0s, m0v);
-      node_dropout(a.mask1, a.rng, 1, n, g, m1s, m1v);
-      x0[0] = Io<ST>::ld4(a.h, hr + 4 * g) + Io<ST>::ld4(a.dh, hr + 4 * g) * m0s;
-#pragma unroll
-      for (int p = 0; p < 3; ++p) xv0[p][0] = Io<ST>::ld(a.h, hr + NS + 3 * g + p) + Io<ST>::ld(a.dh, hr + NS + 3 * g + p) * m0v;
-      const float* ups[3] = {a.g_up0, a.g_up1, a.g_up2};
-#pragma unroll
-      for (int u = 0; u < 3; ++u)
-        if (ups[u]) {
-          const float* r_ = ups[u] + n * ROW;
-          gs[0] += *reinterpret_cast<const f4*>(r_ + 4 * g);
-#pragma unroll
-          for (int p = 0; p < 3; ++p) gv[p][0] += r_[NS + 3 * g + p];
-        }
-    }
-    f4 y[1] = {x0[0]};
-    float yv[3][1] = {{xv0[0][0]}, {xv0[1][0]}, {xv0[2][0]}};
-    ln_quad<NS, NV>(f_node + IM::ND_LN0, lane, y, yv);
-    f4 hs[1][4], s2[1][1];
-    float hv[1][3][2], v2[1][3][1];
-    float bs0[1][4], bv0[1][3][1], bs1[1][16], bv1[1][3][2];
-    typename Ff0<ST>::Cache c0[1];
-    typename Ff1<ST>::Cache c1[1];
-#pragma unroll
-    for (int r = 0; r < 4; ++r) bs0[0][r] = y[0][r];
-#pragma unroll
-    for (int p = 0; p < 3; ++p) bv0[0][p][0] = yv[p][0];
-    Ff0<ST>::template forward<1, Io<ST>::BF>(f_node + IM::ND_FF0, lane, zt, bs0, bv0, hs, hv, c0);
-#pragma unroll
-    for (int t = 0; t < 4; ++t)
-#pragma unroll
-      for (int r = 0; r < 4; ++r) bs1[0][4 * t + r] = hs[0][t][r];
-#pragma unroll
-    for (int p = 0; p < 3; ++p) { bv1[0][p][0] = hv[0][p][0]; bv1[0][p][1] = hv[0][p][1]; }
-    Ff1<ST>::template forward<1, Io<ST>::BF>(f_node + IM::ND_FF1, lane, zt, bs1, bv1, s2, v2, c1);
-    f4 z[1] = {y[0] + s2[0][0] * m1s};
-    float zv[3][1];
-#pragma unroll
-    for (int p = 0; p < 3; ++p) zv[p][0] = yv[p][0] + v2[0][p][0] * m1v;
-
-    STAMP(2);
-    STAMP(3);
-    {
-      f4 dga[1], dbe[1];
-      ln_quad_bwd<NS, NV>(f_node + IM::ND_LN1, lane, z, zv, gs, gv, dga, dbe);
-      ln_param_grads<Acc, NS>(gblk + NB_LN1, first, lane, active, dga, dbe);
-    }
-    float d_hs[16], d_hv[3][2];
-    {
-      f4 d_so[1] = {gs[0] * m1s};
-      float d_vo[3][1] = {{gv[0][0] * m1v}, {gv[1][0] * m1v}, {gv[2][0] * m1v}};
-      typename Ff1<ST>::Grads gr1;
-      STAMP(4);
-      Ff1<ST>::template backward<Io<ST>::BF>(t_node + IM::TN_FF1, lane, c1[0], d_so, d_vo, d_hs, d_hv, gr1);
-      STAMP(5);
-      Ff1<ST>::template weight_grads<Acc, Io<ST>::BF>(gblk + NB_FF1, first, lane, 0, active, bs1[0], bv1[0], c1[0], gr1, tscr);
-    }
-    {
-      f4 d_so[4];
-#pragma unroll
-      for (int t = 0; t < 4; ++t) d_so[t] = f4{d_hs[4 * t], d_hs[4 * t + 1], d_hs[4 * t + 2], d_hs[4 * t + 3]};
-      float d_ys[4], d_yv[3][1];
-      typename Ff0<ST>::Grads gr0;
-      STAMP(6);
-      Ff0<ST>::template backward<Io<ST>::BF>(t_node + IM::TN_FF0, lane, c0[0], d_so, d_hv, d_ys, d_yv, gr0);
-      STAMP(7);
-      Ff0<ST>::template weight_grads<Acc, Io<ST>::BF>(gblk + NB_FF0, first, lane, 0, active, bs0[0], bv0[0], c0[0], gr0, tscr);
-#pragma unroll
-      for (int r = 0; r < 4; ++r) gs[0][r] += d_ys[r];
-#pragma unroll
-      for (int p = 0; p < 3; ++p) gv[p][0] += d_yv[p][0];
-    }
-    STAMP(8);
-    {
-      f4 dga[1], dbe[1];
-      ln_quad_bwd<NS, NV>(f_node + IM::ND_LN0, lane, x0, xv0, gs, gv, dga, dbe);
-      ln_param_grads<Acc, NS>(gblk + NB_LN0, first, lane, active, dga, dbe);
-    }
-    if (active) {
-      if (a.g_h) {
-        float* row = a.g_h + n * ROW;
-        *reinterpret_cast<f4*>(row + 4 * g) = gs[0];
-#pragma unroll
-        for (int p = 0; p < 3; ++p) row[NS + 3 * g + p] = gv[p][0];
-      }
-      float* row = a.g_dh + n * ROW;
-      *reinterpret_cast<f4*>(row + 4 * g) = gs[0] * m0s;
-#pragma unroll
-      for (int p = 0; p < 3; ++p) row[NS + 3 * g + p] = gv[p][0] * m0v;
-      if (a.zero_rows) {
-        float* z = a.zero_rows + n * ROW;
-        *reinterpret_cast<f4*>(z + 4 * g) = zero;
-#pragma unroll
-        for (int p = 0; p < 3; ++p) z[NS + 3 * g + p] = 0.f;
-      }
-    }
+    const int lane = opaque_lane(lane0);
+    const int64_t n = tile * TILE + (lane & 15);
+    node_bwd_tile<ST, Acc>(a, f_node, t_node, gblk, tscr, lane, n, n < a.N);
   }
   STAMP(9);
   write_slab_row<NODE_GB, NODE_GB>(a.slab, blocks);
@@ -628,9 +643,8 @@
   }
 }
 
-template <int NTE, typename ST, int TN, int C2_WPB, bool STORE = false>
-__global__ __launch_bounds__(WAVE * C2_WPB) __attribute__((amdgpu_waves_per_eu(C2_WPB / 4, C2_WPB / 4))) void conv_bwd2_kernel(ConvBArgs a) {
-  WALL_STAMP(2);
+template <int NTE, typename ST, int TN, int C2_WPB, bool STORE, bool FUSED>
+__device__ __forceinline__ void conv_bwd2_body(const ConvBArgs& a, float* lds, int32_t wg_lo, int32_t wg_hi) {
   typedef Image<0, NTE> IM;
   typedef ConvBImg<NTE> BI;
   typedef ConvBlk<NTE> B;
@@ -638,7 +652,6 @@
   constexpr int C2_TPB = SH::TPB, C2_GS_ROWS = SH::GS_ROWS, C2_SCR = SH::SCR;
   constexpr int PW = B::SIZE + C2_SCR;
   constexpr bool BF = Io<ST>::BF;
-  extern __shared__ __attribute__((aligned(16))) float lds[];
   float* img = lds + C2_TPB - BI::F0;
   float* imgT = lds + C2_TPB + BI::FSIZE - BI::T0;
   const int lane = threadIdx.x & 63, i = lane & 15, g = lane >> 4;
@@ -648,8 +661,10 @@
   float* tscr = gblk + B::SIZE;
   float* trow = tscr + TN * TSCR_FLOATS;
   int* tsrc = reinterpret_cast<int*>(trow + C2_GS_ROWS * ROW);
-  stage_slice<BI::FSIZE, C2_TPB>(lds + C2_TPB, a.img + BI::F0, threadIdx.x);
-  stage_slice<BI::TSIZE, C2_TPB>(lds + C2_TPB + BI::FSIZE, a.imgT + BI::T0, threadIdx.x);
+  if constexpr (!FUSED) {
+    stage_slice<BI::FSIZE, C2_TPB>(lds + C2_TPB, a.img + BI::F0, threadIdx.x);
+    stage_slice<BI::TSIZE, C2_TPB>(lds + C2_TPB + BI::FSIZE, a.imgT + BI::T0, threadIdx.x);
+  }
   for (int k = lane; k < B::SIZE / 4; k += WAVE) reinterpret_cast<f4*>(gblk)[k] = f4{0.f, 0.f, 0.f, 0.f};
 
   const f4 zero = {0.f, 0.f, 0.f, 0.f};
@@ -663,15 +678,17 @@
       if (a.rowptr[nd + 1] == a.rowptr[nd]) a.g_dst[n0 * ROW + k] = 0.f;
     }
   }
-  const int32_t E = a.rowptr[a.N];
-  const int32_t iters = (E + TN * TILE - 1) / (TN * TILE);
-  const int32_t ipw = (int32_t)((iters + waves - 1) / waves);
-  const int64_t it0 = wid * ipw;
-  const int32_t c_lo = (int32_t)(it0 < iters ? it0 : iters) * (TN * TILE);
-  int32_t c_hi = (int32_t)(it0 + ipw < iters ? it0 + ipw : iters) * (TN * TILE);
-  c_hi = c_hi < E ? c_hi : E;
+  const int32_t r_lo = FUSED ? wg_lo : 0;
+  const int32_t r_hi = FUSED ? wg_hi : a.rowptr[a.N];
+  const int64_t nw = FUSED ? C2_WPB : waves, wi = FUSED ? w : wid;
+  const int32_t iters = (r_hi - r_lo + TN * TILE - 1) / (TN * TILE);
+  const int32_t ipw = (int32_t)((iters + nw - 1) / nw);
+  const int64_t it0 = wi * ipw;
+  const int32_t c_lo = r_lo + (int32_t)(it0 < iters ? it0 : iters) * (TN * TILE);
+  int32_t c_hi = r_lo + (int32_t)(it0 + ipw < iters ? it0 + ipw : iters) * (TN * TILE);
+  c_hi = c_hi < r_hi ? c_hi : r_hi;
   int32_t lead_dst = -1;
-  if (c_lo > 0 && c_lo < c_hi) {
+  if (c_lo > r_lo && c_lo < c_hi) {
     const int32_t d0 = a.edst[c_lo], dm = a.edst[c_lo - 1];
     lead_dst = d0 == dm ? d0 : -1;
   }
@@ -701,7 +718,7 @@
     }
   }
   STAMP(0);
-  __syncthreads();
+  if constexpr (!FUSED) __syncthreads();
   STAMP(1);
 
   const int zt[TN] = {};
@@ -956,6 +973,100 @@
   Msg2<ST>::template wacc_flush<AccStoreOnce>(w2, gblk + B::M2, lane);
   write_slab_row<B::SIZE, PW, C2_WPB>(a.slab, blocks);
   STAMP(9);
+}
+template <int NTE, typename ST, int TN, int C2_WPB, bool STORE = false>
+__global__ __launch_bounds__(WAVE * C2_WPB) __attribute__((amdgpu_waves_per_eu(C2_WPB / 4, C2_WPB / 4))) void conv_bwd2_kernel(ConvBArgs a) {
+  WALL_STAMP(2);
+  extern __shared__ __attribute__((aligned(16))) float lds[];
+  conv_bwd2_body<NTE, ST, TN, C2_WPB, STORE, false>(a, lds, 0, 0);
+}
+
+template <int NTE>
+struct FusedPlan {
+  typedef C2Shape<1, 8> SH;
+  static constexpr int WPB = 8, TPB = SH::TPB;
+  static constexpr int PW = ConvBlk<NTE>::SIZE + SH::SCR;
+  static constexpr int CONV = SH::template lds_floats<NTE>();
+  static constexpr int NODE_IMG = Image<0, 0>::ND_SIZE + Image<0, 0>::TN_SIZE;
+  static constexpr int SLOT = NODE_GB + TSCR_FLOATS;
+  static constexpr int NSLOT = (WPB * PW) / SLOT < WPB ? (WPB * PW) / SLOT : WPB;
+  static constexpr int TOTAL = CONV + NODE_IMG;
+  static_assert(TPB == BW_TPB, "both phases index the trash words by thread");
+  static_assert(NSLOT >= 1 && NSLOT * SLOT <= WPB * PW, "the node slots alias the conv regions and nothing else");
+  static_assert(CONV % 4 == 0 && SLOT % 4 == 0 && PW % 4 == 0, "16-B aligned regions");
+  static_assert(TOTAL * 4 <= 160 * 1024, "fused node + conv backward LDS plan exceeds the CU");
+};
+
+struct FusedArgs { NodeBArgs nd; ConvBArgs a; };
+static_assert(sizeof(ConvBArgs) % 8 == 0 && offsetof(FusedArgs, a) % 8 == 0, "read back as 8-byte words");
+__device__ __forceinline__ ConvBArgs conv_args_again() {
+  typedef const __attribute__((address_space(4))) uint64_t* KernargWords;
+  struct Words { uint64_t w[sizeof(ConvBArgs) / 8]; } v;
+  KernargWords k = (KernargWords)__builtin_amdgcn_kernarg_segment_ptr();
+  asm volatile("" : "+s"(k));
+#pragma unroll
+  for (size_t j = 0; j < sizeof(ConvBArgs) / 8; ++j) v.w[j] = k[offsetof(FusedArgs, a) / 8 + j];
+  return __builtin_bit_cast(ConvBArgs, v);
+}
+
+template <int NTE, typename ST>
+__global__ __launch_bounds__(BW_TPB) __attribute__((amdgpu_waves_per_eu(2, 2))) void node_conv_bwd_kernel(FusedArgs args) {
+  const NodeBArgs& nd = args.nd;
+  const ConvBArgs& a = args.a;
+  WALL_STAMP(2);
+  typedef FusedPlan<NTE> P;
+  typedef ConvBImg<NTE> BI;
+  typedef Image<0, 0> IM;
+  extern __shared__ __attribute__((aligned(16))) float lds[];
+  float* blocks = lds + P::TPB + BI::FSIZE + BI::TSIZE;
+  float* f_node = lds + P::CONV;
+  float* t_node = f_node + IM::ND_SIZE;
+  const int lane0 = threadIdx.x & 63;
+  const int w = __builtin_amdgcn_readfirstlane(threadIdx.x >> 6);
+  const int32_t E = a.rowptr[a.N];
+  const int b = blockIdx.x, G = gridDim.x;
+  const int32_t s0 = gvp_range::nominal_start(E, G, b), s1 = gvp_range::nominal_start(E, G, b + 1);
+  const bool f0 = gvp_range::is_boundary(a.edst, E, (int64_t)s0 + lane0);
+  const bool f1 = gvp_range::is_boundary(a.edst, E, (int64_t)s1 + lane0);
+  stage_slice<BI::FSIZE, P::TPB>(lds + P::TPB, a.img + BI::F0, threadIdx.x);
+  stage_slice<BI::TSIZE, P::TPB>(lds + P::TPB + BI::FSIZE, a.imgT + BI::T0, threadIdx.x);
+  stage_slice<IM::ND_SIZE, P::TPB>(f_node, nd.img_node, threadIdx.x);
+  stage_slice<IM::TN_SIZE, P::TPB>(t_node, nd.imgT_node, threadIdx.x);
+  float* gblk = blocks + (w < P::NSLOT ? w : 0) * P::SLOT;
+  if (w < P::NSLOT) zero_block<NODE_GB>(gblk, lane0);
+  const unsigned long long m0 = __ballot(f0), m1 = __ballot(f1);
+  int32_t lo = m0 ? s0 + __builtin_ctzll(m0) : gvp_range::range_start(a.edst, E, s0 + gvp_range::WINDOW, lane0);
+  int32_t hi = m1 ? s1 + __builtin_ctzll(m1) : gvp_range::range_start(a.edst, E, s1 + gvp_range::WINDOW, lane0);
+  lo = __builtin_amdgcn_readfirstlane(lo < E ? lo : E);
+  hi = __builtin_amdgcn_readfirstlane(hi < E ? hi : E);
+  int64_t n_lo, n_hi;
+  gvp_range::owned_nodes(a.edst, E, a.N, b, lo, hi, &n_lo, &n_hi);
+  STAMP(0);
+  __syncthreads();
+  STAMP(1);
+  const int32_t ntiles = (int32_t)((n_hi - n_lo + TILE - 1) / TILE);
+  if (w < P::NSLOT) {
+    float* tscr = gblk + NODE_GB;
+    if (ntiles <= P::NSLOT) {
+      if (w < ntiles) {
+        const int lane = opaque_lane(lane0);
+        const int64_t n = n_lo + (int64_t)w * TILE + (lane & 15);
+        node_bwd_tile<ST, AccStoreOnce>(nd, f_node, t_node, gblk, tscr, lane, n, n < n_hi);
+      }
+    } else {
+      for (int32_t tile = w; tile < ntiles; tile += P::NSLOT) {
+        const int lane = opaque_lane(lane0);
+        const int64_t n = n_lo + (int64_t)tile * TILE + (lane & 15);
+        node_bwd_tile<ST, AccPriv>(nd, f_node, t_node, gblk, tscr, lane, n, n < n_hi);
+      }
+    }
+  }
+  __builtin_amdgcn_fence(__ATOMIC_RELEASE, "workgroup");
+  write_slab_row<NODE_GB, P::SLOT, P::NSLOT>(nd.slab, blocks, blockIdx.x, opaque_lane(threadIdx.x));
+  __syncthreads();
+  __builtin_amdgcn_fence(__ATOMIC_ACQUIRE, "workgroup");
+  const ConvBArgs ca = conv_args_again();
+  conv_bwd2_body<NTE, ST, 1, P::WPB, false, true>(ca, lds, lo, hi);
 }
 
 template <int NTE>
@@ -1340,8 +1451,8 @@
 int node_update_bwd(const float* img_node, const float* imgT_node, const float* h, const float* dh,
                     const float* mask0, const float* mask1, gvp::RngArgs rng, const float* g_up0, const float* g_up1,
                     const float* g_up2, int64_t N, float* g_dh, float* g_h, float* zero_rows, float* slab, int* grid,
-                    int policy, hipStream_t st) {
-  NodeBArgs a{img_node, imgT_node, h, dh, mask0, mask1, rng, g_up0, g_up1, g_up2, N, g_dh, g_h, zero_rows, slab};
+                    int policy, hipStream_t st, float* zero_rows2) {
+  NodeBArgs a{img_node, imgT_node, h, dh, mask0, mask1, rng, g_up0, g_up1, g_up2, N, g_dh, g_h, zero_rows, slab, zero_rows2};
   const int64_t tiles = (N + TILE - 1) / TILE;
   const int G = grid_for(tiles);
   *grid = G;
@@ -1357,9 +1468,9 @@
 int node_head_bwd(const float* img_head, const float* imgT_head, const float* h_out, const float* g_out, float* g_h_out,
                   float* head_slab, const float* img_node, const float* imgT_node, const float* h, const float* dh,
                   const float* mask0, const float* mask1, gvp::RngArgs rng, int64_t N, float* g_dh, float* g_h,
-                  float* zero_rows, float* slab, int* grid, int policy, hipStream_t st) {
+                  float* zero_rows, float* slab, int* grid, int policy, hipStream_t st, float* zero_rows2) {
   HeadBArgs hd{img_head, imgT_head, h_out, g_out, N, g_h_out, head_slab};
-  NodeBArgs a{img_node, imgT_node, h, dh, mask0, mask1, rng, g_h_out, nullptr, nullptr, N, g_dh, g_h, zero_rows, slab};
+  NodeBArgs a{img_node, imgT_node, h, dh, mask0, mask1, rng, g_h_out, nullptr, nullptr, N, g_dh, g_h, zero_rows, slab, zero_rows2};
   const int64_t tiles = (N + TILE - 1) / TILE;
   const int G = grid_for(tiles);
   *grid = G;
@@ -1392,13 +1503,19 @@
   return v;
 }
 
+inline int64_t conv_bwd2_units(int64_t E) { return ((E + TILE - 1) / TILE + 1) / 2; }
+template <int TN, int WPB_>
+int conv_bwd2_grid(int64_t E) {
+  const int64_t iters = (E + TN * TILE - 1) / (TN * TILE);
+  const int64_t wgs = (iters + WPB_ - 1) / WPB_;
+  const int cap = bwd_grid_cap(conv_bwd2_units(E));
+  return (int)(wgs < 1 ? 1 : (wgs > cap ? cap : wgs));
+}
+
 template <int NTE, int TN, int WPB_, bool STORE>
 int conv_bwd2_impl(ConvBArgs& a, int64_t E, int* grid, int policy, hipStream_t st) {
   typedef C2Shape<TN, WPB_> SH;
-  const int64_t iters = (E + TN * TILE - 1) / (TN * TILE);
-  const int64_t wgs = (iters + WPB_ - 1) / WPB_;
-  const int cap = bwd_grid_cap(((E + TILE - 1) / TILE + 1) / 2);
-  const int G = (int)(wgs < 1 ? 1 : (wgs > cap ? cap : wgs));
+  const int G = conv_bwd2_grid<TN, WPB_>(E);
   *grid = G;
   const size_t lds = (size_t)SH::template lds_floats<NTE>() * sizeof(float);
   return with_policy<NTE == 0>(policy, [&](auto tag) {
@@ -1442,6 +1559,33 @@
   return CGVP_ERR_UNSUPPORTED_DIMS;
 }
 
+constexpr int kFusedSlots = FusedPlan<0>::NSLOT < FusedPlan<1>::NSLOT ? FusedPlan<0>::NSLOT : FusedPlan<1>::NSLOT;
+bool fuse_node_conv(int policy, int64_t N, int64_t E) {
+  static const int mode = [] { const char* e = getenv("CGVP_FUSE_NODE_CONV"); return !e ? 0 : (e[0] == '0' ? -1 : (e[0] == '1' ? 1 : 0)); }();
+  if (mode < 0 || policy != POLICY_F32 || conv_bwd_version() != 3 || N <= 0 || E <= 0) return false;
+  if (mode > 0) return true;
+  const int64_t G = conv_bwd2_grid<1, 8>(E);
+  return conv_bwd2_units(E) <= G * 8 && (N + TILE - 1) / TILE <= G * kFusedSlots;
+}
+
+int node_conv_bwd(int nt_edge, const float* img_node, const float* imgT_node, const float* h, const float* dh,
+                  const float* mask0, const float* mask1, gvp::RngArgs rng, const float* g_up0, const float* g_up1,
+                  const float* g_up2, float* g_dh, float* g_h, float* zero_rows, float* node_slab, const float* img,
+                  const float* imgT, const float* e_emb, const int32_t* rowptr, const int32_t* esrc, const int32_t* edst,
+                  int64_t N, int64_t E, int mean, float* g_src, float* g_dst, float* g_e, float* conv_slab, int* grid,
+                  hipStream_t st) {
+  NodeBArgs nd{img_node, imgT_node, h, dh, mask0, mask1, rng, g_up0, g_up1, g_up2, N, g_dh, g_h, zero_rows, node_slab};
+  ConvBArgs a{img, imgT, h, e_emb, rowptr, esrc, edst, N, 1, mean, g_dh, g_src, g_dst, g_e, conv_slab, nullptr, nullptr};
+  const int G = conv_bwd2_grid<1, 8>(E);
+  *grid = G;
+  const FusedArgs args{nd, a};
+  if (nt_edge == 0)
+    return launch<node_conv_bwd_kernel<0, float>>(dim3(G), dim3(BW_TPB), (size_t)FusedPlan<0>::TOTAL * sizeof(float), st, args);
+  if (nt_edge == 1)
+    return launch<node_conv_bwd_kernel<1, float>>(dim3(G), dim3(BW_TPB), (size_t)FusedPlan<1>::TOTAL * sizeof(float), st, args);
+  return CGVP_ERR_UNSUPPORTED_DIMS;
+}
+
 template <int NTE>
 int edge_bwd_impl(EdgeBArgs& a, int* grid, int policy, hipStream_t st) {
   const int64_t tiles = (a.E + TILE - 1) / TILE;
diff --git a/caster-dta_amd/csrc/gvp_range.h b/caster-dta_amd/csrc/gvp_range.h
--- /dev/null
+++ b/caster-dta_amd/csrc/gvp_range.h
@@ -0,0 +1,46 @@
+#pragma once
+#include <stdint.h>
+
+#if defined(__HIPCC__)
+#define GVP_RANGE_HD __host__ __device__
+#else
+#define GVP_RANGE_HD
+#endif
+
+namespace gvp_range {
+
+constexpr int WINDOW = 64;
+
+GVP_RANGE_HD inline int32_t nominal_start(int32_t E, int G, int b) {
+  const int64_t S = ((int64_t)E + G - 1) / G;
+  const int64_t p = (int64_t)b * S;
+  return (int32_t)(p < E ? p : E);
+}
+
+GVP_RANGE_HD inline bool is_boundary(const int32_t* edst, int32_t E, int64_t p) {
+  return p >= E || p == 0 || edst[p] != edst[p - 1];
+}
+
+GVP_RANGE_HD inline int32_t range_start(const int32_t* edst, int32_t E, int32_t from, int lane) {
+  for (int64_t base = from;; base += WINDOW) {
+#if defined(__HIP_DEVICE_COMPILE__)
+    const unsigned long long hits = __ballot(is_boundary(edst, E, base + lane));
+    if (hits) {
+      const int64_t p = base + __builtin_ctzll(hits);
+      return (int32_t)(p < E ? p : E);
+    }
+#else
+    (void)lane;
+    for (int k = 0; k < WINDOW; ++k)
+      if (is_boundary(edst, E, base + k)) return (int32_t)(base + k < E ? base + k : E);
+#endif
+  }
+}
+
+GVP_RANGE_HD inline void owned_nodes(const int32_t* edst, int32_t E, int64_t N, int b, int32_t lo, int32_t hi,
+                                     int64_t* n_lo, int64_t* n_hi) {
+  *n_lo = b == 0 ? 0 : (lo < E ? (int64_t)edst[lo] : N);
+  *n_hi = hi < E ? (int64_t)edst[hi] : N;
+}
+
+}
diff --git a/caster-dta_amd/csrc/pass_api.hip b/caster-dta_amd/csrc/pass_api.hip
--- a/caster-dta_amd/csrc/pass_api.hip
+++ b/caster-dta_amd/csrc/pass_api.hip
@@ -361,28 +361,43 @@
       return rc;
   }
   const float *up0 = nullptr, *up1 = nullptr, *up2 = nullptr;
+  const bool fuse = !det && nc > 1 && quad::fuse_node_conv(quad::policy_index(dims), N, E);
   for (int l = nc - 1; l >= 0; --l) {
     const bool last = l == nc - 1;
     float* g_dh = buf(l, 0);
     float* g_h = drop ? buf(l, 1) : nullptr;
     float* g_src = buf(l, 2);
     float* g_dst = buf(l, 3);
+    float* zero_below = (fuse && l >= 1) ? buf(l - 1, 2) : nullptr;
     cgvp_rng rng{draw ? seed : nullptr, dropout_p, 2 * l};
     const float* m0 = (drop && masks) ? masks + (int64_t)(2 * l) * mstride : nullptr;
     const float* m1 = (drop && masks) ? masks + (int64_t)(2 * l + 1) * mstride : nullptr;
-    if (int rc = cgvp_node_update_bwd(dims, layout, image, l, row(l), row(nc + l), m0, m1, draw ? &rng : nullptr,
-                                      last ? row(2 * nc) : nullptr, last ? g_out : nullptr, up0, up1, up2, N, last ? 1 : 0,
-                                      g_dh, g_h, g_src, grad_params, region(), segs + nseg, &cnt, stream))
-      return rc;
-    nseg += cnt;
-    {
+    if (fuse && !last) {
+      float* node_region = region();
+      float* conv_region = region();
       Timed timed(1, stream);
-      if (int rc = quad::conv_bwd_entry(dims, layout, image, l, row(l), e_emb, rowptr, esrc, edst, N, E, aggr_mean, g_dh, g_src,
-                                        1, g_dst, g_e + (int64_t)l * bw.g_e_stride, grad_params, region(), segs + nseg, &cnt,
-                                        stream, det ? &db : nullptr))
+      if (int rc = quad::node_conv_bwd_entry(dims, layout, image, l, row(l), row(nc + l), m0, m1, draw ? &rng : nullptr, up0,
+                                             up1, up2, e_emb, rowptr, esrc, edst, N, E, aggr_mean, g_dh, g_h, zero_below,
+                                             g_src, g_dst, g_e + (int64_t)l * bw.g_e_stride, node_region, conv_region,
+                                             segs + nseg, &cnt, stream))
         return rc;
+      nseg += cnt;
+    } else {
+      if (int rc = quad::node_bwd_entry(dims, layout, image, l, row(l), row(nc + l), m0, m1, draw ? &rng : nullptr,
+                                        last ? row(2 * nc) : nullptr, last ? g_out : nullptr, up0, up1, up2, N,
+                                        last ? 1 : 0, g_dh, g_h, g_src, zero_below, grad_params, region(), segs + nseg,
+                                        &cnt, stream))
+        return rc;
+      nseg += cnt;
+      {
+        Timed timed(1, stream);
+        if (int rc = quad::conv_bwd_entry(dims, layout, image, l, row(l), e_emb, rowptr, esrc, edst, N, E, aggr_mean, g_dh, g_src,
+                                          1, g_dst, g_e + (int64_t)l * bw.g_e_stride, grad_params, region(), segs + nseg, &cnt,
+                                          stream, det ? &db : nullptr))
+          return rc;
+      }
+      nseg += cnt;
     }
-    nseg += cnt;
     up0 = g_h ? g_h : g_dh; up1 = g_src; up2 = g_dst;
   }
   if (int rc = cgvp_node_embed_bwd(dims, layout, image, batch->x_s, batch->x_v, batch->ntypes, N, up0, up1, up2, g_x_s, g_x_v,
```

After: 279,300 graph-pairs/sec. About the same (-0.0%).
